# KirillHit/snn_for_object_detection

Measured on AMD Instinct MI355X. Metric: event-frames/sec (BxT) SODa-3M GEN1 304x240 fwd+bwd, higher is better.
Workload: dtype f32 (16-bit split products)

## Files before the change

include/snn_hip.h:

```cpp
#ifndef SNN_HIP_H
#define SNN_HIP_H

#include <stddef.h>
#include <stdint.h>

#ifdef __cplusplus
extern "C" {
#endif

#define SNN_ABI_VERSION 20

enum {
    SNN_NEURON_NONE = 0,
    SNN_NEURON_LIF = 1,
    SNN_NEURON_LI = 2,
    SNN_NEURON_LI_TANH = 3,
    SNN_NEURON_SLI = 4,
    SNN_NEURON_SYNAPSE = 5
};

enum { SNN_PREC_FP32 = 0, SNN_PREC_BF16X3 = 1, SNN_PREC_BF16X6 = 3, SNN_PREC_FP16X3 = 4, SNN_PREC_BF16X1 = 5,
       SNN_PREC_BF16S = 6 };

enum { SNN_SCAN_WIDE_ADDRESSING = 1,
// ... 77 lines not shown
                            int precision);
int snn_conv2d_gather_plan(int mode, int64_t N, int H, int W, int Cin, int Ho, int Wo, int Cout, int KH, int KW, int stride,
                           int pad, int64_t ld_in, int64_t ld_out, int align_bits, int has_split_image, int has_addend,
                           int has_addend2, int frames_per_step, int precision, int phase, int* out);
int snn_conv2d_wgrad_plan(int64_t N, int H, int W, int Cin, int Ho, int Wo, int Cout, int KH, int KW, int stride, int pad,
                          int64_t ldx, int64_t lddy, int align_bits, int precision, int spikes, int num_cu, int* out);
int snn_conv1x1_spikes_supported(int64_t N, int H, int W, int Cin, int Cout, int64_t ld, int fwd_precision,
                                 int bwd_precision);
int snn_conv1x1_spikes_fwd(const float* vdec, int64_t ld, float v_th, const float* w, float* y, int64_t ldy, int64_t N, int H,
                           int W, int Cin, int Cout, void* stream);
int snn_conv1x1_spikes_wgrad(const float* vdec, int64_t ld, float v_th, const float* dy, int64_t lddy, float* dw, int64_t N,
                             int H, int W, int Cin, int Cout, int accumulate, float* workspace, int splitk, void* stream);

int snn_conv2d_spikes_supported(int64_t N, int H, int W, int Cin, int Ho, int Wo, int Cout, int KH, int KW, int stride,
                                int pad, int64_t ld, int fwd_precision, int bwd_precision);
int snn_conv2d_spikes_fwd(const float* vdec, int64_t ld, float v_th, const float* w, float* y, int64_t ldy, int64_t N, int H,
                          int W, int Cin, int Ho, int Wo, int Cout, int KH, int KW, int stride, int pad, double* bn_partial,
                          int frames_per_step, int* bn_layout, void* stream);
int snn_conv2d_spikes_wgrad(const float* vdec, int64_t ld, float v_th, const float* dy, int64_t lddy, float* dw, int64_t N,
                            int H, int W, int Cin, int Ho, int Wo, int Cout, int KH, int KW, int stride, int pad,
                            int accumulate, float* workspace, int splitk, void* stream);
int snn_conv3x3_halo_spikes(const float* vdec, int64_t ld, float v_th, const void* w_image, float* y, int64_t ldy, int64_t N,
                            int H, int W, int Cin, int Cout, double* bn_partial, int frames_per_step, int* bn_layout,
                            void* stream);

int snn_conv1x1_mask_supported(int64_t N, int H, int W, int Cin, int Cout, const uint32_t* mask, int64_t ld_mask,
                               const float* w, const float* y, int64_t ldy, const float* dy, int64_t lddy, const float* dw,
                               int fwd_precision, int bwd_precision);
int snn_conv1x1_mask_fwd(const uint32_t* mask, int64_t ld_mask, const float* w, float* y, int64_t ldy, int64_t N, int H, int W,
                         int Cin, int Cout, void* stream);
int snn_conv1x1_mask_wgrad(const uint32_t* mask, int64_t ld_mask, const float* dy, int64_t lddy, float* dw, int64_t N, int H,
                           int W, int Cin, int Cout, int accumulate, float* workspace, int splitk, void* stream);

size_t snn_bn_stats_partial_size(int T, int64_t M, int C);
int snn_bn_stats(const float* y, int64_t ldy, int T, int64_t M, int C, double* partial, void* stream);
int snn_bn_stats_finalize(const double* partial, int chunks, int rows_per_chunk, int T, int64_t M, int C,
                          const float* gamma, const float* bias, float eps, float momentum,
                          float* running_mean, float* running_var, int use_running,
                          float* mean, float* invstd, float* alpha, float* beta, void* stream);

int snn_bn_stats_reduce(const double* partial, int chunks, int rows_per_chunk, int T, int64_t M, int C, double* sums,
                        void* stream);
int snn_bn_stats_from_sums(const double* sums, int T, int64_t M_total, int C,
                           const float* gamma, const float* bias, float eps, float momentum,
                           float* running_mean, float* running_var,
                           float* mean, float* invstd, float* alpha, float* beta,
                           double* var_scratch, void* stream);

int snn_affine_neuron_fwd(int neuron, const float* y, int64_t ldy,
                          const float* alpha, const float* beta,
                          const float* v0, const float* i0,
                          float* out, int64_t ldo, const float* addend, int64_t ld_addend,
                          float* vT, float* iT, float* vdec,
                          int T, int64_t M, int C, const snn_neuron_params* p, int flags, void* stream);
int snn_affine_neuron_fwd_mask(int neuron, const float* y, int64_t ldy, const float* alpha, const float* beta,
                               const float* v0, const float* i0, float* out, int64_t ldo, const float* addend,
                               int64_t ld_addend, float* vT, float* iT, float* vdec, int T, int64_t M, int C,
                               const snn_neuron_params* p, int flags, void* stream, uint32_t* mask, int64_t ld_mask);

size_t snn_affine_neuron_bwd_sums_size(int T, int64_t M, int C);
int snn_affine_neuron_bwd_sums_from_state(int neuron, int T, int64_t M, int C, int64_t ldg, const snn_neuron_params* p,
                                          int flags);
int snn_affine_neuron_bwd_plan(int neuron, int T, int64_t M, int C, int64_t ldg, int64_t ldy, int with_sums,
                               const snn_neuron_params* p, int flags, int64_t* out);
int snn_affine_neuron_bwd(int neuron, const float* g_out, int64_t ldg, const float* state,
                          const float* y, int64_t ldy, const float* g_vT, const float* g_iT,
// ... 207 lines not shown
```

snn_for_object_detection_amd/_hip.py:

```python

import ctypes
import os
from ctypes import POINTER, Structure, c_char_p, c_double, c_float, c_int, c_int32, c_int64, c_size_t, c_void_p

_HERE = os.path.dirname(os.path.abspath(__file__))
LIB_PATH = os.environ.get("SNN_HIP_LIB") or os.path.join(_HERE, "libsnn_hip.so")

NEURON_NONE, NEURON_LIF, NEURON_LI, NEURON_LI_TANH, NEURON_SLI, NEURON_SYNAPSE = 0, 1, 2, 3, 4, 5
POOL_AVG, POOL_MAX, POOL_SUM = 0, 1, 2
ACT_RELU, ACT_SILU, ACT_TANH = 0, 1, 2
ABI_VERSION = 20
PREC_FP32, PREC_BF16X3, PREC_BF16X6, PREC_FP16X3, PREC_BF16X1, PREC_BF16S = 0, 1, 3, 4, 5, 6
SCAN_WIDE_ADDRESSING, SCAN_LAST_STEP_ONLY, SCAN_BF16_STORAGE, SCAN_SPIKES_FROM_VDEC, SCAN_SUMS_FROM_STATE = 1, 2, 4, 8, 16
SCAN_STATE_LOOKBACK = 32
SCAN_SPIKE_MASK = 32
SURR_SUPER, SURR_TRIANGLE, SURR_SIGMOID, SURR_ATAN = 0, 1, 2, 3
ACTIVITY_NONZERO_F32, ACTIVITY_NONZERO_BF16, ACTIVITY_ABOVE_F32, ACTIVITY_ABOVE_BF16, ACTIVITY_MASK = 0, 1, 2, 3, 4
LOSS_CLS_MODES = {"ce": 0, "focal": 1}
LOSS_BOX_MODES = {"l1": 0, "giou": 1, "diou": 2, "ciou": 3}


class NeuronParams(Structure):
    _fields_ = [("c_mem", c_float), ("c_syn", c_float), ("v_leak", c_float), ("v_th", c_float),
                ("v_reset", c_float), ("alpha", c_float), ("v_st", c_float), ("tau_sec", c_float),
# ... 17 lines not shown
    "snn_detect_assemble": (c_int, [_P, _P, _P, _P, _P, _P, _I, _I, _I, _F, _P, _P]),
    "snn_conv2d_fwd": (c_int, [_P, _L, _P, _P, _P, _L, _L, _I, _I, _I, _I, _I, _I, _I, _I, _I, _I, _P, _L, _P, _I, _P, _I,
                               _P]),
    "snn_weight_presplit": (c_int, [_P, _P, _L, _I, _P]),
    "snn_conv2d_fwd_bn_partial_size": (c_size_t, [_L, _I, _I, _I, _I]),
    "snn_conv2d_wgrad_bn_supported": (c_int, [_L, _I, _I, _I, _I, _I, _I, _I, _I, _I, _I]),
    "snn_conv2d_wgrad_bn": (c_int, [_P, _L, _P, _L, _P, _L, _P, _I, _I, _P, _L, _I, _I, _I, _I, _I, _I, _I, _I, _I, _I, _I,
                                    _P, _I, _P]),
    "snn_conv3x3_s2_dgrad_supported": (c_int, [_L, _I, _I, _I, _I, _I, _I]),
    "snn_conv3x3_s2_dgrad_plan": (c_int, [_L, _I, _I, _I, _I, _I, _I, _P]),
    "snn_conv3x3_halo_plan": (c_int, [_L, _I, _I, _I, _I, _I, _P]),
    "snn_conv2d_wgrad_halo_plan": (c_int, [_L, _I, _I, _I, _I, _I, _I, _I, _I, _P]),
    "snn_conv_first_plan": (c_int, [_L, _I, _I, _I, _I, _I, _I, _I, _I, _I, _I, _P]),
    "snn_conv3x3_s2_dgrad": (c_int, [_P, _L, _P, _P, _L, _L, _I, _I, _I, _I, _I, _I, _P, _L, _P, _L, _I, _P]),
    "snn_conv3x3_halo_supported": (c_int, [_L, _I, _I, _I, _I]),
    "snn_conv3x3_halo_bn_chunks": (c_int64, [_I, _I, _I]),
    "snn_weight_frag_image_bytes": (c_size_t, [_I, _I]),
    "snn_weight_frag_image_batched": (c_int, [_P, _P, _P, _I, _I, _I, _I, _P]),
    "snn_conv3x3_halo": (c_int, [_P, _L, _P, _P, _L, _L, _I, _I, _I, _I, _P, _L, _P, _L, _P, _I, _P, _I, _P]),
    "snn_conv2d_dgrad": (c_int, [_P, _L, _P, _P, _P, _L, _L, _I, _I, _I, _I, _I, _I, _I, _I, _I, _I, _P, _L, _P, _L,
                                 _I, _P]),
    "snn_conv2d_wgrad": (c_int, [_P, _L, _P, _L, _P, _L, _I, _I, _I, _I, _I, _I, _I, _I, _I, _I, _I, _P, _I, _I,
                                 _P]),
    "snn_conv2d_wgrad_splitk": (c_int, [_L, _I, _I, _I, _I, _I, _I, _I, _I, _I, _I, _I]),
    "snn_conv2d_wgrad_kernel": (c_int, [_L, _I, _I, _I, _I, _I, _I, _I, _I, _I, _I, _I]),
    "snn_conv2d_gather_plan": (c_int, [_I, _L, _I, _I, _I, _I, _I, _I, _I, _I, _I, _I, _L, _L, _I, _I, _I, _I, _I, _I, _I, _P]),
    "snn_conv2d_wgrad_plan": (c_int, [_L, _I, _I, _I, _I, _I, _I, _I, _I, _I, _I, _L, _L, _I, _I, _I, _I, _P]),
    "snn_conv1x1_spikes_supported": (c_int, [_L, _I, _I, _I, _I, _L, _I, _I]),
    "snn_conv1x1_spikes_fwd": (c_int, [_P, _L, _F, _P, _P, _L, _L, _I, _I, _I, _I, _P]),
    "snn_conv1x1_spikes_wgrad": (c_int, [_P, _L, _F, _P, _L, _P, _L, _I, _I, _I, _I, _I, _P, _I, _P]),
    "snn_conv1x1_mask_supported": (c_int, [_L, _I, _I, _I, _I, _P, _L, _P, _P, _L, _P, _L, _P, _I, _I]),
    "snn_conv1x1_mask_fwd": (c_int, [_P, _L, _P, _P, _L, _L, _I, _I, _I, _I, _P]),
    "snn_conv1x1_mask_wgrad": (c_int, [_P, _L, _P, _L, _P, _L, _I, _I, _I, _I, _I, _P, _I, _P]),
    "snn_conv2d_spikes_supported": (c_int, [_L, _I, _I, _I, _I, _I, _I, _I, _I, _I, _I, _L, _I, _I]),
    "snn_conv2d_spikes_fwd": (c_int, [_P, _L, _F, _P, _P, _L, _L, _I, _I, _I, _I, _I, _I, _I, _I, _I, _I, _P, _I, _P, _P]),
    "snn_conv2d_spikes_wgrad": (c_int, [_P, _L, _F, _P, _L, _P, _L, _I, _I, _I, _I, _I, _I, _I, _I, _I, _I, _I, _P, _I, _P]),
    "snn_conv3x3_halo_spikes": (c_int, [_P, _L, _F, _P, _P, _L, _L, _I, _I, _I, _I, _P, _I, _P, _P]),
    "snn_bn_stats_partial_size": (c_size_t, [_I, _L, _I]),
    "snn_bn_stats": (c_int, [_P, _L, _I, _L, _I, _P, _P]),
    "snn_bn_stats_finalize": (c_int, [_P, _I, _I, _I, _L, _I, _P, _P, _F, _F, _P, _P, _I, _P, _P, _P, _P, _P]),
    "snn_bn_stats_reduce": (c_int, [_P, _I, _I, _I, _L, _I, _P, _P]),
    "snn_bn_stats_from_sums": (c_int, [_P, _I, _L, _I, _P, _P, _F, _F, _P, _P, _P, _P, _P, _P, _P, _P]),
    "snn_bn_bwd_reduce": (c_int, [_P, _I, _L, _I, _P, _P]),
    "snn_bn_bwd_coef": (c_int, [_P, _P, _P, _I, _L, _I, _P, _P, _P, _P, _P, _P, _P, _P, _I, _P]),
    "snn_affine_neuron_fwd": (c_int, [_I, _P, _L, _P, _P, _P, _P, _P, _L, _P, _L, _P, _P, _P, _I, _L, _I,
                                      POINTER(NeuronParams), _I, _P]),
    "snn_affine_neuron_fwd_mask": (c_int, [_I, _P, _L, _P, _P, _P, _P, _P, _L, _P, _L, _P, _P, _P, _I, _L, _I,
                                           POINTER(NeuronParams), _I, _P, _P, _L]),
    "snn_lif_ckpt_interval": (c_int, []),
    "snn_lif_fwd_ckpt": (c_int, [_P, _L, _P, _P, _P, _P, _P, _L, _P, _L, _P, _P, _P, _I, _L, _I,
                                 POINTER(NeuronParams), _P]),
    "snn_lif_bwd_ckpt": (c_int, [_P, _L, _P, _P, _L, _P, _P, _P, _P, _I, _P, _P, _P, _P, _I, _L, _I,
                                 POINTER(NeuronParams), _P]),
    "snn_affine_neuron_bwd_sums_size": (c_size_t, [_I, _L, _I]),
    "snn_affine_neuron_bwd": (c_int, [_I, _P, _L, _P, _P, _L, _P, _P, _P, _P, _I, _P, _P, _P, _P, _I, _L, _I,
                                      POINTER(NeuronParams), _I, _P]),
    "snn_bn_bwd_finalize": (c_int, [_P, _I, _L, _I, _P, _P, _P, _P, _P, _P, _P, _P, _I, _P]),
    "snn_bn_bwd_finalize_from_state": (c_int, [_P, _I, _L, _I, _P, _P, _P, _P, _P, _P, _L, _P, _P, _P, _P, _P, _I, _P]),
    "snn_bn_bwd_reduce_from_state": (c_int, [_P, _I, _L, _I, _P, _P, _P, _P, _P, _P, _L, _P, _P]),
    "snn_affine_neuron_bwd_sums_from_state": (c_int, [_I, _I, _L, _I, _L, POINTER(NeuronParams), _I]),
    "snn_affine_neuron_bwd_plan": (c_int, [_I, _I, _L, _I, _L, _L, _I, POINTER(NeuronParams), _I, _P]),
    "snn_lif_tau_param": (c_int, [_P, _P, _I, _I, _P, _P, _P]),
    "snn_lif_tau_fwd": (c_int, [_I, _P, _L, _P, _P, _P, _P, _P, _L, _P, _L, _P, _P, _P, _I, _L, _I,
                                POINTER(NeuronParams), _P, _P, _I, _P]),
    "snn_lif_tau_bwd_partial_size": (c_size_t, [_I, _L, _I, _I]),
    "snn_lif_tau_bwd_plan": (c_int, [_I, _I, _L, _I, _L, _L, _I, _I, POINTER(NeuronParams), _I, _P]),
# ... 105 lines not shown
```

snn_for_object_detection_amd/csrc/conv_common.h:

```cpp
#pragma once
#include "snn_common.h"

namespace {

constexpr int kThreads = 256;
#define SNN_CONV_MIN_WAVES 3

typedef __bf16 bf16x8 __attribute__((ext_vector_type(8)));
typedef __bf16 bf16x4 __attribute__((ext_vector_type(4)));
typedef __bf16 bf16x2 __attribute__((ext_vector_type(2)));
typedef float f32x2 __attribute__((ext_vector_type(2)));
typedef unsigned u32x4 __attribute__((ext_vector_type(4)));
typedef unsigned u32x2 __attribute__((ext_vector_type(2)));
typedef _Float16 f16x8 __attribute__((ext_vector_type(8)));
typedef _Float16 f16x2 __attribute__((ext_vector_type(2)));
constexpr float kF16WeightScale = 256.0f;
constexpr float kF16ActScale = 16.0f;
constexpr float kF16Unscale = 1.0f / (kF16WeightScale * kF16ActScale);

__device__ __forceinline__ int div_magic(int n, int d, unsigned magic) { return d == 1 ? n : (int)__umulhi((unsigned)n, magic); }

enum : unsigned {
    kAlignIn16 = 1u, kAlignIn8 = 2u, kAlignW16 = 4u, kAlignOut16 = 8u, kAlignOut8 = 16u, kAlignAdd16 = 32u, kAlignAdd8 = 64u,
    kAlignAdd2_16 = 128u, kAlignAdd2_8 = 256u, kAlignSplit16 = 512u, kAlignAll = 1023u
};

static int check_conv_shape(const char* name, int64_t N, int H, int W, int Cin, int Ho, int Wo, int Cout, int KH,
                            int KW, int stride, int pad) {
    SNN_REQUIRE(N > 0 && H > 0 && W > 0 && Cin > 0 && Cout > 0 && KH > 0 && KW > 0 && stride > 0 && pad >= 0,
                "%s: bad shape", name);
    SNN_REQUIRE(Ho == (H + 2 * pad - KH) / stride + 1 && Wo == (W + 2 * pad - KW) / stride + 1 && Ho > 0 && Wo > 0,
                "%s: output size %dx%d does not match input %dx%d k=%dx%d s=%d p=%d", name, Ho, Wo, H, W, KH, KW,
                stride, pad);
    return 0;
}

static bool spikes_shape_ok(int64_t N, int H, int W, int Cin, int Ho, int Wo, int Cout, int KH, int KW, int stride, int pad,
                            int64_t ld) {
    return N > 0 && H > 0 && W > 0 && Cin > 0 && Cout > 0 && KH >= 1 && KW >= 1 && KH <= 5 && KW <= 5 && stride >= 1 &&
           Ho == (H + 2 * pad - KH) / stride + 1 && Wo == (W + 2 * pad - KW) / stride + 1 && Ho > 0 && Wo > 0 &&
           Cin % 32 == 0 && Cout % 4 == 0 && ld % 4 == 0 && ld >= Cin && N * (int64_t)H * W < 0x7fffffffLL &&
           N * (int64_t)Ho * Wo < 0x7fffffffLL && (int64_t)H * W * ld * 16 < 0x7fffffffLL;
}

}

struct FirstGeom {
    int64_t ldx, ldy;
    int rows;
    int H, W, Ho, Wo, Cout, stride, pad;
    int group_rows, group_blocks;
    double* bn_partial;
    const float* bn_y;
    int64_t bn_ldy;
    const float* bn_coef;
    int bn_tc;
    int bn_fps;
    int rs;
};

struct FirstPlan {
    int ok;
    int rs, LW, cgs, PP;
    int blocks;
    int group_rows, group_blocks;
    int max_rows, last_stage_rows;
    size_t lds;
};
FirstPlan snn_first_layer_plan(int64_t N, int H, int W, int Ho, int Wo, int Cout, int stride, int pad,
                               int frames_per_step, bool wgrad, int num_cu);
bool snn_first_layer_shape(int Cin, int Cout, int KH, int KW);
int snn_first_layer_blocks(int64_t rows, int num_cu);
int snn_launch_first(bool wgrad, bool bnapply, bool sb, int blocks, size_t lds, const float* x, const float* w,
                     const float* dy, float* out, const FirstGeom& fg, void* stream, const char* name);

bool snn_wgrad_mask_ok(int64_t N, int H, int W, int Cin, int Cout, const uint32_t* mask, int64_t ld_mask, const float* dy,
                       int64_t lddy, const float* dw);
```

snn_for_object_detection_amd/csrc/conv_gather.hip:

```cpp
#include <stdlib.h>
#include <type_traits>
#include "conv_common.h"

#if defined(SNN_STAMP) || defined(SNN_CLOCK)
__device__ unsigned long long g_stamps[2048 * 8];
__device__ unsigned long long g_stamps2[2048 * 4];
extern "C" int snn_debug_stamps(unsigned long long* out, int n) {
    return (int)hipMemcpyFromSymbol(out, HIP_SYMBOL(g_stamps), sizeof(unsigned long long) * n);
}
extern "C" int snn_debug_stamps2(unsigned long long* out, int n) {
    return (int)hipMemcpyFromSymbol(out, HIP_SYMBOL(g_stamps2), sizeof(unsigned long long) * n);
}
#endif
#ifdef SNN_STAMP
#define STAMP(i) do { unsigned long long t_ = __builtin_readcyclecounter(); st_acc[i] += t_ - st_last; st_last = t_; } while (0)
#else
#define STAMP(i) do {} while (0)
#endif

namespace {

constexpr int BM = 128;
constexpr int BK = 32;
constexpr int LDK = BK + 4;
// ... 23 lines not shown

template <int WM, int WN, int TN>
__device__ __forceinline__ void stat_flush(double (&s)[TN], double (&q)[TN], double* red, double* __restrict__ partial,
                                           int64_t step, int64_t chunk, int64_t chunks, int n0, int OC, int tid) {
    const int lane = tid & 63, wave = tid >> 6;
#pragma unroll
    for (int j = 0; j < TN; ++j) {
        s[j] += __shfl_xor(s[j], 32, 64);
        q[j] += __shfl_xor(q[j], 32, 64);
        if (lane < 32) {
            red[((wave * TN + j) * 32 + lane) * 2 + 0] = s[j];
            red[((wave * TN + j) * 32 + lane) * 2 + 1] = q[j];
        }
    }
    __syncthreads();
    if (tid < WN * TN * 32) {
        const int wn = tid / (TN * 32), jr = tid % (TN * 32);
        double ss = 0.0, qq = 0.0;
#pragma unroll
        for (int wm = 0; wm < WM; ++wm) {
            const double* src = red + (((wm * WN + wn) * TN) * 32 + jr) * 2;
            ss += src[0];
            qq += src[1];
        }
        if (n0 + tid < OC) {
            double* dst = partial + snn_bn_partial_index(step, chunk, n0 + tid, chunks, OC);
            dst[0] = ss;
            dst[1] = qq;
        }
    }
    __syncthreads();
}

template <int BN, int WM, int WN, bool DGRAD, bool VEC, int SPLIT, bool FAST, bool PRESPLIT = false, bool SB = false,
          bool XSP = false, bool XM = false>
__global__ __launch_bounds__(kThreads, (FAST && SPLIT) ? (PRESPLIT ? 3 : (SB ? (DGRAD ? 4 : SNN_GATHER_SB_WAVES) : 2)) : SNN_CONV_MIN_WAVES) void k_conv_gather(const float* __restrict__ in, const float* __restrict__ wk,
                                                          float* __restrict__ out, ConvGeom g,
                                                          const float* __restrict__ addend, int64_t ld_add,
                                                          const float* __restrict__ addend2, int64_t ld_add2) {
    constexpr int TM = BM / WM / 32;
    constexpr int TN = BN / WN / 32;
    constexpr int BROWS = BN / 32;
    static_assert(WM * WN == 4, "4 waves");
    static_assert(!SB || (FAST && SPLIT == 5 && !PRESPLIT), "bf16 storage: the pipelined one-product kernel");
    static_assert(!XSP || (FAST && SPLIT == 4 && !DGRAD && !PRESPLIT && !SB), "spikes from potentials: fp16 x 3 forward");
    static_assert(!XM || XSP, "spike bit mask: an instance of the spikes-from-potentials kernel");
    constexpr int ES = SB ? 2 : 4;
    constexpr int NPIECE = SPLIT == 3 ? 3 : (SPLIT == 5 ? 1 : 2);
    constexpr int A_BYTES = SPLIT ? NPIECE * BM * LDB * 2 : BM * LDK * 4;
    constexpr int B_BYTES = SPLIT ? NPIECE * BN * LDB * 2 : BN * LDK * 4;
    constexpr int STAGE_BYTES = 4 * 32 * (TN * 32 + 4) * 4;
    constexpr int SMEM_BYTES = A_BYTES + B_BYTES > STAGE_BYTES ? A_BYTES + B_BYTES : STAGE_BYTES;
    __shared__ __attribute__((aligned(16))) unsigned char smem[SMEM_BYTES];
    float* As = reinterpret_cast<float*>(smem);
    float* Bs = reinterpret_cast<float*>(smem + A_BYTES);
    __bf16* Ah = reinterpret_cast<__bf16*>(smem);
    __bf16* Al = Ah + BM * LDB;
    __bf16* Am = Al + BM * LDB;
    __bf16* Bh = reinterpret_cast<__bf16*>(smem + A_BYTES);
    __bf16* Bl = Bh + BN * LDB;
    __bf16* Bm = Bl + BN * LDB;

    const int tid = threadIdx.x;
#if defined(SNN_STAMP) || defined(SNN_CLOCK)
    const unsigned long long st_kernel_begin = __builtin_amdgcn_s_memtime();
    const unsigned long long st_real_begin = __builtin_amdgcn_s_memrealtime();
#endif
    const int lane_id = tid & 63, wave = tid >> 6;
    const int wm = wave / WN, wn = wave % WN;
    const int r = lane_id & 31, h = lane_id >> 5;

    const int bid_xcd = blockIdx.x & 7, bid_q = blockIdx.x >> 3;
    const int bid_n = bid_q % g.ntiles;
    const int64_t bid_m = (int64_t)bid_xcd * g.mtiles_per_xcd + bid_q / g.ntiles;
    if (bid_m >= g.mtiles) return;
    const int64_t m0 = bid_m * BM;
    const int n0 = bid_n * BN;

    const int lrr = tid >> 3;
// ... 13 lines not shown
        const int oy = (int)(t - img * oh_);
        a_base[j] = (int)(img * (unsigned)(g.IH * g.IW));
        if (!DGRAD) {
            a_y0[j] = oy * g.stride - g.pad;
            a_x0[j] = ox * g.stride - g.pad;
        } else if (g.stride == 1) {
            a_y0[j] = oy + g.pad;
            a_x0[j] = ox + g.pad;
        } else {
            a_y0[j] = (int)((unsigned)(oy * g.stride + g.ph + g.pad - g.kh0) / (unsigned)g.stride);
            a_x0[j] = (int)((unsigned)(ox * g.stride + g.pw + g.pad - g.kw0) / (unsigned)g.stride);
        }
    }

    auto decode_k = [&](int kk, int& dy, int& dx, int& c, int& wcol) {
        int tap = div_magic(kk, g.IC, g.magic_ic);
        c = kk - tap * g.IC;
        if (!DGRAD) {
            int kh = div_magic(tap, g.KW, g.magic_kw), kw = tap - kh * g.KW;
            dy = kh;
            dx = kw;
            wcol = kk;
        } else {
            int jh = div_magic(tap, g.nkw, g.magic_kw), jw = tap - jh * g.nkw;
            dy = -jh;
            dx = -jw;
            wcol = ((g.kh0 + g.stride * jh) * g.KW + (g.kw0 + g.stride * jw)) * g.IC + c;
        }
    };

    using AReg = typename std::conditional<SB, u32x2, typename std::conditional<XM, unsigned, f32x4>::type>::type;
    AReg ra[4];
    f32x4 rb[BROWS];

    __amdgpu_buffer_rsrc_t rs_a, rs_b;
    int a_rel[4];
    unsigned a_mask[4];
    unsigned b_rel[BROWS];
    [[maybe_unused]] int xm_rel[TM];
    if constexpr (XM) {
        rs_a = __builtin_amdgcn_make_buffer_rsrc(const_cast<float*>(in), 0, (int)(g.Mtot * g.ldi * 4), 0x00020000);
        rs_b = __builtin_amdgcn_make_buffer_rsrc(const_cast<float*>(wk), 0, g.OC * g.KtotFull * 4, 0x00020000);
#pragma unroll
        for (int i = 0; i < TM; ++i) {
            const int64_t m = m0 + (wm * TM + i) * 32 + r;
            xm_rel[i] = m < g.Mtot ? (int)(m * g.ldi * 4) : -1;
        }
#pragma unroll
        for (int j = 0; j < BROWS; ++j) {
            const int n = n0 + lr + 32 * j;
            b_rel[j] = n < g.OC ? (unsigned)(n * g.KtotFull + kq) * 4u : 0x80000000u;
        }
    } else if (FAST) {
        const int ow_ = DGRAD ? g.OWc : g.OW, oh_ = DGRAD ? g.OHc : g.OH;
        const int64_t img0 = (unsigned)m0 / (unsigned)(oh_ * ow_);
        const int64_t ipix = (int64_t)g.IH * g.IW;
        const int64_t bytes = ((((int64_t)g.nimg - img0) * ipix - 1) * g.ldi + g.IC) * ES;
        rs_a = __builtin_amdgcn_make_buffer_rsrc(const_cast<char*>(reinterpret_cast<const char*>(in) + img0 * ipix * g.ldi * ES), 0,
                                                 bytes > 0xffffffffLL ? (int)0xffffffffu : (int)(unsigned)bytes,
                                                 0x00020000);
        rs_b = __builtin_amdgcn_make_buffer_rsrc(const_cast<float*>(wk), 0, g.OC * g.KtotFull * 4, 0x00020000);
        const int tw_n = DGRAD ? g.nkw : g.KW;
#pragma unroll
        for (int j = 0; j < 4; ++j) {
            const int relpix = (a_base[j] - (int)(img0 * ipix)) + a_y0[j] * g.IW + a_x0[j];
            a_rel[j] = (relpix * (int)g.ldi + kq) * ES;
            const int nth = DGRAD ? g.nkh : g.KH;
            unsigned xm = 0, mask = 0;
#pragma unroll
            for (int tw = 0; tw < 6; ++tw) {
                const int ix = DGRAD ? a_x0[j] - tw : a_x0[j] + tw;
                xm |= (tw < tw_n && (unsigned)ix < (unsigned)g.IW) ? 1u << tw : 0u;
            }
#pragma unroll
            for (int th = 0; th < 6; ++th) {
                const int iy = DGRAD ? a_y0[j] - th : a_y0[j] + th;
                mask |= (th < nth && (unsigned)iy < (unsigned)g.IH) ? xm << (th * tw_n) : 0u;
            }
            a_mask[j] = a_ok[j] ? mask : 0u;
        }
#pragma unroll
        for (int j = 0; j < BROWS; ++j) {
            const int n = n0 + lr + 32 * j;
            b_rel[j] = n < g.OC ? (unsigned)(n * g.KtotFull + kq) * 4u : 0x80000000u;
        }
    }
    const unsigned fast_tw_n = DGRAD ? g.nkw : g.KW;
    const unsigned fast_tw_one = fast_tw_n == 1 ? 1u : 0u;
    auto load_tiles_fast = [&](int k0n, AReg (&ra)[4], f32x4 (&rb)[BROWS], int which = 3) {
        const bool kin = k0n < g.Ktot;
        const int tap = (int)__umulhi((unsigned)k0n, g.magic_ic);
        const int c0 = k0n - tap * g.IC;
        const int th = (int)(__umulhi((unsigned)tap, g.magic_kw) + (unsigned)tap * fast_tw_one);
        const int tw = tap - th * (int)fast_tw_n;
        int toff, wcol0;
        if (!DGRAD) {
            toff = ((th * g.IW + tw) * (int)g.ldi + c0) * ES;
            wcol0 = k0n;
        } else {
            toff = (c0 - (th * g.IW + tw) * (int)g.ldi) * ES;
            wcol0 = ((g.kh0 + g.stride * th) * g.KW + (g.kw0 + g.stride * tw)) * g.IC + c0;
        }
        const int tbit = kin ? tap : 31;
        if constexpr (XM) {
            if (which & 1) {
#pragma unroll
                for (int i = 0; i < TM; ++i)
                    ra[i] = (unsigned)__builtin_amdgcn_raw_buffer_load_b32(rs_a, (kin && xm_rel[i] >= 0) ? xm_rel[i] + (k0n >> 5) * 4 : -1, 0, 0);
            }
        } else if (which & 1) {
#pragma unroll
            for (int j = 0; j < 4; ++j) {
                const int voff = ((a_mask[j] >> tbit) & 1u) ? a_rel[j] + toff : -1;
                if constexpr (SB) ra[j] = __builtin_bit_cast(u32x2, __builtin_amdgcn_raw_buffer_load_b64(rs_a, voff, 0, 0));
                else ra[j] = __builtin_bit_cast(f32x4, __builtin_amdgcn_raw_buffer_load_b128(rs_a, voff, 0, 0));
            }
        }
        if (which & 2) {
            const unsigned wb = (unsigned)wcol0 * 4u;
#pragma unroll
            for (int j = 0; j < BROWS; ++j)
                rb[j] = __builtin_bit_cast(f32x4, __builtin_amdgcn_raw_buffer_load_b128(rs_b, (int)(b_rel[j] + wb), 0, 0));
        }
    };

    auto load_tiles = [&](int k0) {
        if (FAST) {
            load_tiles_fast(k0, ra, rb);
            return;
        }
        if constexpr (!SB && !XM) {
        const int kk = k0 + kq;
        if (VEC) {
            const bool kin = kk < g.Ktot;
            int dy, dx, c, wcol;
            decode_k(kin ? kk : g.Ktot - 4, dy, dx, c, wcol);
            const f32x4 zero = {0.f, 0.f, 0.f, 0.f};
#pragma unroll
            for (int j = 0; j < 4; ++j) {
                const int iy = a_y0[j] + dy, ix = a_x0[j] + dx;
                const bool ok = kin & a_ok[j] & ((unsigned)iy < (unsigned)g.IH) & ((unsigned)ix < (unsigned)g.IW);
                const int iyc = min(max(iy, 0), g.IH - 1), ixc = min(max(ix, 0), g.IW - 1);
                f32x4 v = *reinterpret_cast<const f32x4*>(in + (int64_t)(a_base[j] + iyc * g.IW + ixc) * g.ldi + c);
                ra[j] = ok ? v : zero;
            }
#pragma unroll
            for (int j = 0; j < BROWS; ++j) {
                const int n = n0 + lr + 32 * j;
                const int nc = min(n, g.OC - 1);
                f32x4 v = *reinterpret_cast<const f32x4*>(wk + (int64_t)nc * g.KtotFull + wcol);
                rb[j] = (kin & (n < g.OC)) ? v : zero;
            }
        } else {
#pragma unroll
            for (int e = 0; e < 4; ++e) {
                const int ke = kk + e;
                const bool kin = ke < g.Ktot;
                int dy, dx, c, wcol;
                decode_k(kin ? ke : 0, dy, dx, c, wcol);
#pragma unroll
                for (int j = 0; j < 4; ++j) {
// ... 75 lines not shown
            if constexpr (SPLIT == 4) {
                u32x2 hi, lo;
#pragma unroll
                for (int e = 0; e < 4; e += 2) {
                    const float a = v[e] * scale, b = v[e + 1] * scale;
                    const f16x2 ph = __builtin_convertvector(f32x2{a, b}, f16x2);
                    const f16x2 pl = __builtin_convertvector(f32x2{a - (float)ph[0], b - (float)ph[1]}, f16x2);
                    hi[e >> 1] = __builtin_bit_cast(unsigned, ph);
                    lo[e >> 1] = __builtin_bit_cast(unsigned, pl);
                }
                out[0] = __builtin_bit_cast(bf16x4, hi);
                out[1] = __builtin_bit_cast(bf16x4, lo);
                return;
            }
#pragma unroll
            for (int e = 0; e < 4; e += 2) {
                f32x2 rest = {v[e], v[e + 1]};
                bf16x2 p = __builtin_convertvector(rest, bf16x2);
                unsigned bits = __builtin_bit_cast(unsigned, p);
                out[0][e] = p[0]; out[0][e + 1] = p[1];
                rest[0] -= __builtin_bit_cast(float, bits << 16);
                rest[1] -= __builtin_bit_cast(float, bits & 0xffff0000u);
                if (SPLIT == 3) {
                    p = __builtin_convertvector(rest, bf16x2);
                    bits = __builtin_bit_cast(unsigned, p);
                    out[2][e] = p[0]; out[2][e + 1] = p[1];
                    rest[0] -= __builtin_bit_cast(float, bits << 16);
                    rest[1] -= __builtin_bit_cast(float, bits & 0xffff0000u);
                }
                p = __builtin_convertvector(rest, bf16x2);
                out[1][e] = p[0]; out[1][e + 1] = p[1];
            }
        };
        auto convert_a = [&](const AReg& v, bf16x4* out) {
            if constexpr (SB) out[0] = __builtin_bit_cast(bf16x4, v);
            else if constexpr (XM) return;
            else if constexpr (XSP) {
                u32x2 hi;
#pragma unroll
                for (int e = 0; e < 4; e += 2)
                    hi[e >> 1] = (v[e] > g.x_th ? 0x4C00u : 0u) | (v[e + 1] > g.x_th ? 0x4C000000u : 0u);
                out[0] = __builtin_bit_cast(bf16x4, hi);
            } else convert(v, out, kF16ActScale);
        };
        auto convert_b = [&](const f32x4& v, bf16x4* out) {
            if constexpr (PRESPLIT) {
                static_assert(!PRESPLIT || SPLIT == 2 || SPLIT == 4, "pre-split weights: two-piece modes only");
                out[0] = __builtin_bit_cast(bf16x4, f32x2{v[0], v[1]});
                out[1] = __builtin_bit_cast(bf16x4, f32x2{v[2], v[3]});
            } else {
                convert(v, out, kF16WeightScale);
            }
        };
        [[maybe_unused]] unsigned xm_cur[TM];
        auto xm_expand = [&](unsigned word, int sel) {
            const unsigned b = (word >> (8 * sel)) & 0xffu;
            u32x4 d;
#pragma unroll
            for (int q = 0; q < 4; ++q) {
                const unsigned v = (b >> (2 * q)) & 3u;
                d[q] = ((v | (v << 15)) & 0x00010001u) * 0x4C00u;
            }
            return __builtin_bit_cast(bf16x8, d);
        };
        auto write_tiles = [&]() {
#pragma unroll
            for (int j = 0; j < (XM ? 0 : 4); ++j) {
// ... 36 lines not shown
                for (int j = 0; j < TN; ++j) {
                    if constexpr (SPLIT == 5) {
                        acc[i][j] = __builtin_amdgcn_mfma_f32_32x32x16_bf16(ah[i], bh[j], acc[i][j], 0, 0, 0);
                        continue;
                    }
                    if constexpr (SPLIT == 4 && XSP) {
                        const f16x8 xah = __builtin_bit_cast(f16x8, ah[i]);
                        const f16x8 xbh = __builtin_bit_cast(f16x8, bh[j]), xbl = __builtin_bit_cast(f16x8, bl[j]);
                        acc[i][j] = __builtin_amdgcn_mfma_f32_32x32x16_f16(xah, xbl, acc[i][j], 0, 0, 0);
                        acc[i][j] = __builtin_amdgcn_mfma_f32_32x32x16_f16(xah, xbh, acc[i][j], 0, 0, 0);
                        continue;
                    }
                    if constexpr (SPLIT == 4) {
                        const f16x8 xah = __builtin_bit_cast(f16x8, ah[i]), xal = __builtin_bit_cast(f16x8, al[i]);
                        const f16x8 xbh = __builtin_bit_cast(f16x8, bh[j]), xbl = __builtin_bit_cast(f16x8, bl[j]);
                        acc[i][j] = __builtin_amdgcn_mfma_f32_32x32x16_f16(xal, xbh, acc[i][j], 0, 0, 0);
                        acc[i][j] = __builtin_amdgcn_mfma_f32_32x32x16_f16(xah, xbl, acc[i][j], 0, 0, 0);
                        acc[i][j] = __builtin_amdgcn_mfma_f32_32x32x16_f16(xah, xbh, acc[i][j], 0, 0, 0);
                        continue;
                    }
                    acc[i][j] = __builtin_amdgcn_mfma_f32_32x32x16_bf16(al[i], bh[j], acc[i][j], 0, 0, 0);
                    acc[i][j] = __builtin_amdgcn_mfma_f32_32x32x16_bf16(ah[i], bl[j], acc[i][j], 0, 0, 0);
                    if (SPLIT == 3) {
                        acc[i][j] = __builtin_amdgcn_mfma_f32_32x32x16_bf16(am[i], bm[j], acc[i][j], 0, 0, 0);
                        acc[i][j] = __builtin_amdgcn_mfma_f32_32x32x16_bf16(am[i], bh[j], acc[i][j], 0, 0, 0);
                        acc[i][j] = __builtin_amdgcn_mfma_f32_32x32x16_bf16(ah[i], bm[j], acc[i][j], 0, 0, 0);
                    }
                    acc[i][j] = __builtin_amdgcn_mfma_f32_32x32x16_bf16(ah[i], bh[j], acc[i][j], 0, 0, 0);
                }
        };
        constexpr int NM = TM * TN * (XSP ? 2 : NPROD);
        constexpr int NREAD = XM ? TN * NP : (XSP ? TM + TN * NP : (TM + TN) * NP);
        constexpr int CONV_OPS = SPLIT == 3 ? 24 : (SPLIT == 5 ? 2 : 14);
        constexpr int VPG_A = ((XM ? TM * 18 : (XSP ? 4 * 8 : 4 * CONV_OPS)) + NM - 1) / NM;
        constexpr int VPG_B = PRESPLIT ? 1 : (BROWS * CONV_OPS + NM - 1) / NM;
        if (g.Ktot > 0) {
            AReg ra0[4];
            f32x4 rb0[BROWS];
            load_tiles_fast(0, ra0, rb0);
            load_tiles_fast(BK, ra, rb);
            if constexpr (XM) {
#pragma unroll
                for (int i = 0; i < TM; ++i) xm_cur[i] = ra0[i];
            }
#pragma unroll
            for (int j = 0; j < 4; ++j) convert_a(ra0[j], pa[j]);
#pragma unroll
            for (int j = 0; j < BROWS; ++j) convert_b(rb0[j], pb[j]);
            write_tiles();
        }
        __syncthreads();
#ifdef SNN_STAMP
        unsigned long long st_acc[8] = {0, 0, 0, 0, 0, 0, 0, 0};
        unsigned long long st_last = __builtin_readcyclecounter();
        const unsigned long long st_begin = st_last;
#endif
#pragma unroll 1
        for (int k0 = 0; k0 < g.Ktot; k0 += BK) {
            mfma_group(0);
#pragma unroll
            for (int j = 0; j < 4; ++j) convert_a(ra[j], pa[j]);
            __builtin_amdgcn_sched_group_barrier(0x100, NREAD, 0);
#pragma unroll
            for (int m = 0; m < NM; ++m) {
                __builtin_amdgcn_sched_group_barrier(0x008, 1, 0);
                __builtin_amdgcn_sched_group_barrier(0x002, VPG_A, 0);
            }
            __builtin_amdgcn_sched_barrier(0);
            STAMP(0);
            mfma_group(1);
#pragma unroll
            for (int j = 0; j < BROWS; ++j) convert_b(rb[j], pb[j]);
            __builtin_amdgcn_sched_group_barrier(0x100, NREAD, 0);
#pragma unroll
            for (int m = 0; m < NM; ++m) {
                __builtin_amdgcn_sched_group_barrier(0x008, 1, 0);
                __builtin_amdgcn_sched_group_barrier(0x002, VPG_B, 0);
            }
            __builtin_amdgcn_sched_barrier(0);
            STAMP(1);
            if constexpr (XM) {
#pragma unroll
                for (int i = 0; i < TM; ++i) xm_cur[i] = ra[i];
            }
            load_tiles_fast(k0 + 2 * BK, ra, rb);
            STAMP(2);
            __syncthreads();
            STAMP(3);
            write_tiles();
            STAMP(4);
            __syncthreads();
            STAMP(5);
        }
#ifdef SNN_STAMP
        if (tid == 0 && bid_n == 0 && blockIdx.x < 2048) {
            st_acc[6] = __builtin_readcyclecounter() - st_begin;
            st_acc[7] = st_begin;
            for (int i = 0; i < 8; ++i) g_stamps[blockIdx.x * 8 + i] = st_acc[i];
        }
#endif
    } else {
        if (g.Ktot > 0) {
            load_tiles(0);
            store_tiles();
        }
        __syncthreads();

    #pragma unroll 1
        for (int k0 = 0; k0 < g.Ktot; k0 += BK) {
            load_tiles(k0 + BK);
            __builtin_amdgcn_sched_barrier(0);
            if (SPLIT) {
    #pragma unroll
                for (int ks = 0; ks < BK / 16; ++ks) {
                    bf16x8 ah[TM], am[TM], al[TM], bh[TN], bm[TN], bl[TN];
    #pragma unroll
                    for (int i = 0; i < TM; ++i) {
                        const int off = ((wm * TM + i) * 32 + r) * LDB + ks * 16 + 8 * h;
// ... 208 lines not shown
    p.mtiles = (int)gm;
    p.mtiles_per_xcd = (int)snn_ceil_div(gm, 8);
    p.ntiles = (int)snn_ceil_div(g.OC, p.bn);
    p.blocks = (int64_t)p.mtiles_per_xcd * 8 * p.ntiles;
    if (p.blocks > 0x7fffffffLL) {
        p.why = kGatherGridTooLarge;
        return p;
    }
    p.ok = 1;
    return p;
}

static unsigned gather_align_bits(const void* in, const void* wk, const void* wk_split, const void* out, const void* addend,
                                  int64_t ld_add, const void* addend2, int64_t ld_add2) {
    unsigned a = 0;
    if (aligned(16, {in})) a |= kAlignIn16;
    if (aligned(8, {in})) a |= kAlignIn8;
    if (aligned(16, {wk})) a |= kAlignW16;
    if (aligned(16, {out})) a |= kAlignOut16;
    if (aligned(8, {out})) a |= kAlignOut8;
    if (addend && ld_add % 4 == 0 && aligned(16, {addend})) a |= kAlignAdd16;
    if (addend && ld_add % 4 == 0 && aligned(8, {addend})) a |= kAlignAdd8;
    if (addend2 && ld_add2 % 4 == 0 && aligned(16, {addend2})) a |= kAlignAdd2_16;
    if (addend2 && ld_add2 % 4 == 0 && aligned(8, {addend2})) a |= kAlignAdd2_8;
    if (wk_split && aligned(16, {wk_split})) a |= kAlignSplit16;
    return a;
}

constexpr int gather_wm(int bn) { return bn == 32 ? 4 : 2; }
constexpr int gather_wn(int bn) { return bn == 32 ? 1 : 2; }

static int launch_gather(bool dgrad, int split, bool sb, bool xsp, const float* in, const float* wk, const void* wk_split,
                         float* out, const ConvGeom& g, const float* addend, int64_t ld_add, const float* addend2,
                         int64_t ld_add2, hipStream_t st, const char* name, bool xm = false) {
    unsigned align = gather_align_bits(in, wk, wk_split, out, addend, ld_add, addend2, ld_add2);
    if (xm) align = (align & ~(kAlignIn16 | kAlignIn8)) | (aligned(4, {in}) ? kAlignIn16 : 0u);
    const GatherPlan p = gather_plan(g, dgrad, split, sb, xsp, align, wk_split != nullptr, addend != nullptr,
                                     addend2 != nullptr, xm);
    SNN_REQUIRE(p.why != kGatherTooManyPixels, "%s: too many pixels", name);
    SNN_REQUIRE(p.why != kGatherNotFastSB, "%s: bf16 storage covers the pipelined implicit GEMM only (channels a multiple of 32, pixel "
                "stride a multiple of 4, 8-byte aligned tensors): %d channels, stride %lld", name, g.IC, (long long)g.ldi);
    SNN_REQUIRE(p.why != kGatherNotFastXSP, "%s: covers the pipelined implicit GEMM only (input channels a multiple of 32, pixel stride a "
                "multiple of 4, 16-byte aligned tensors): %d channels, stride %lld", name, g.IC, (long long)g.ldi);
    SNN_REQUIRE(p.why != kGatherGridTooLarge, "%s: grid too large", name);
    ConvGeom gg = g;
    gg.out_vec = p.out_vec;
    gg.mtiles = p.mtiles;
    gg.mtiles_per_xcd = p.mtiles_per_xcd;
    gg.ntiles = p.ntiles;
    const dim3 grid((unsigned)p.blocks);
    const float* wsrc = p.loader == kLoadFastPresplit ? static_cast<const float*>(wk_split) : wk;
    dispatch(
        [&](auto BN, auto L, auto DGRAD, auto SPLIT) {
            constexpr int l = L(), s = SPLIT();
            constexpr bool vec = l != kLoadScalar, fast = l >= kLoadFast, pre = l == kLoadFastPresplit, sbl = l == kLoadSB,
                           xml = l == kLoadXM, xspl = l == kLoadXSP || xml;
            constexpr int ksplit = fast ? s : (vec ? (s == 4 ? 3 : (s == 5 ? 2 : s)) : 0);
            if constexpr ((DGRAD() ? s != 3 && s != 4 : s != 2) && (!sbl || s == 5) && (!xspl || (!DGRAD() && s == 4)) &&
                          (!pre || s == 2 || s == 4)) {
                hipLaunchKernelGGL((k_conv_gather<BN(), gather_wm(BN()), gather_wn(BN()), DGRAD(), vec, ksplit, fast, pre, sbl, xspl, xml>),
                                   grid, dim3(kThreads), 0, st, in, wsrc, out, gg, addend, ld_add, addend2, ld_add2);
                return true;
            }
            return false;
        },
        OneOf<32, 64, 128>{p.bn}, OneOf<0, 1, 2, 3, 4, 5, 6>{p.loader}, Flag{dgrad}, OneOf<0, 2, 3, 4, 5>{split});
    SNN_CHECK_LAUNCH(name);
    return 0;
}

}

namespace {
template <bool F16>
__global__ void k_weight_presplit(const f32x4* __restrict__ w, u32x4* __restrict__ out, int64_t groups) {
    for (int64_t i = (int64_t)blockIdx.x * blockDim.x + threadIdx.x; i < groups; i += (int64_t)gridDim.x * blockDim.x) {
        const f32x4 v = w[i];
        u32x4 o;
#pragma unroll
        for (int e = 0; e < 4; e += 2) {
            if (F16) {
                const float a = v[e] * kF16WeightScale, b = v[e + 1] * kF16WeightScale;
                const f16x2 ph = __builtin_convertvector(f32x2{a, b}, f16x2);
                const f16x2 pl = __builtin_convertvector(f32x2{a - (float)ph[0], b - (float)ph[1]}, f16x2);
                o[e >> 1] = __builtin_bit_cast(unsigned, ph);
                o[2 + (e >> 1)] = __builtin_bit_cast(unsigned, pl);
            } else {
                f32x2 rest = {v[e], v[e + 1]};
                const bf16x2 ph = __builtin_convertvector(rest, bf16x2);
                const unsigned bits = __builtin_bit_cast(unsigned, ph);
                rest[0] -= __builtin_bit_cast(float, bits << 16);
                rest[1] -= __builtin_bit_cast(float, bits & 0xffff0000u);
                const bf16x2 pl = __builtin_convertvector(rest, bf16x2);
                o[e >> 1] = bits;
                o[2 + (e >> 1)] = __builtin_bit_cast(unsigned, pl);
            }
        }
        out[i] = o;
    }
// ... 264 lines not shown
    if (!(N > 0 && H > 0 && W > 0 && Cin > 0 && Cout > 0 && Cin % 32 == 0 && ld_mask >= Cin / 32 && ldy >= Cout &&
          N * (int64_t)H * W < 0x7fffffffLL && (int64_t)Cin * Cin < 0xffffffffLL && mask && w && y))
        return false;
    const ConvGeom g = gather_fwd_geom(N, H, W, Cin, H, W, Cout, 1, 1, 1, 0, ld_mask, ldy);
    unsigned align = gather_align_bits(mask, w, nullptr, y, nullptr, 0, nullptr, 0) & ~(kAlignIn16 | kAlignIn8);
    if (aligned(4, {mask})) align |= kAlignIn16;
    const GatherPlan p = gather_plan(g, false, 4, false, true, align, false, false, false, true);
    return p.ok && p.loader == kLoadXM;
}
}

extern "C" int snn_conv1x1_mask_supported(int64_t N, int H, int W, int Cin, int Cout, const uint32_t* mask, int64_t ld_mask,
                                          const float* w, const float* y, int64_t ldy, const float* dy, int64_t lddy,
                                          const float* dw, int fwd_precision, int bwd_precision) {
    if (fwd_precision != SNN_PREC_FP16X3 || bwd_precision != SNN_PREC_BF16X3 || !mask) return 0;
    if (!(N > 0 && H > 0 && W > 0 && Cin > 0 && Cout > 0 && Cin % 32 == 0 && ld_mask >= Cin / 32 && aligned(4, {mask}) &&
          N * (int64_t)H * W * ld_mask * 4 < 0x7fffffffLL))
        return 0;
    if ((w || y) && !mask_fwd_ok(N, H, W, Cin, Cout, mask, ld_mask, w, y, ldy)) return 0;
    if ((dy || dw) && !snn_wgrad_mask_ok(N, H, W, Cin, Cout, mask, ld_mask, dy, lddy, dw)) return 0;
    return 1;
}

extern "C" int snn_conv1x1_mask_fwd(const uint32_t* mask, int64_t ld_mask, const float* w, float* y, int64_t ldy, int64_t N,
                                    int H, int W, int Cin, int Cout, void* stream) {
    SNN_REQUIRE(mask && w && y, "snn_conv1x1_mask_fwd: null pointer");
    if (check_conv_shape("snn_conv1x1_mask_fwd", N, H, W, Cin, H, W, Cout, 1, 1, 1, 0)) return 1;
    SNN_REQUIRE(mask_fwd_ok(N, H, W, Cin, Cout, mask, ld_mask, w, y, ldy),
                "snn_conv1x1_mask_fwd: call not covered (ask snn_conv1x1_mask_supported)");
    const ConvGeom g = gather_fwd_geom(N, H, W, Cin, H, W, Cout, 1, 1, 1, 0, ld_mask, ldy);
    return launch_gather(false, 4, false, true, reinterpret_cast<const float*>(mask), w, nullptr, y, g, nullptr, 0, nullptr, 0,
                         (hipStream_t)stream, "snn_conv1x1_mask_fwd", true);
}
```

snn_for_object_detection_amd/csrc/conv_wgrad.hip:

```cpp
#include <stdlib.h>
#include <type_traits>
#include "conv_common.h"

namespace {

constexpr int WB_K = 32;

struct WgradGeom {
    int64_t Mtot;
    int H, W, Cin, Ho, Wo, Cout, KH, KW, stride, pad;
    int64_t ldx, lddy;
    int Ktot;
    int64_t pix_per_split;
    int tiles_m, tiles_n, splitk;
    int nimg;
    float x_th;
};

template <int TM, int TN, int WM, int WN, bool VEC>
__global__ __launch_bounds__(kThreads, SNN_CONV_MIN_WAVES) void k_conv_wgrad(const float* __restrict__ x, const float* __restrict__ dy,
                                                         float* __restrict__ ws, WgradGeom g) {
    static_assert(WM * WN == 4, "4 waves");
    constexpr int BMc = 32 * TM * WM, BNk = 32 * TN * WN;
    constexpr int DG = BMc / 4, XG = BNk / 4;
    constexpr int DP = kThreads / DG, XP = kThreads / XG;
    constexpr int DJ = WB_K / DP, XJ = WB_K / XP;
    static_assert(DJ >= 1 && XJ >= 1, "tile too narrow");
    __shared__ __attribute__((aligned(16))) float Ds[WB_K * BMc];
    __shared__ __attribute__((aligned(16))) float Xs[WB_K * BNk];
    __shared__ int Pinfo[2][WB_K][4];

    const int tid = threadIdx.x;
    const int lane_id = tid & 63, wave = tid >> 6;
    const int wm = wave / WN, wn = wave % WN;
    const int r = lane_id & 31, h = lane_id >> 5;

    const int tiles = g.tiles_m * g.tiles_n;
    int L = blockIdx.x, z, tile;
    if (g.splitk % 8 == 0) {
        z = (L % 8) + 8 * (L / (8 * tiles));
        tile = (L / 8) % tiles;
    } else {
        z = L / tiles;
        tile = L % tiles;
    }
    const int co0 = (tile % g.tiles_m) * BMc;
    const int kc0 = (tile / g.tiles_m) * BNk;
    const int64_t p_lo = (int64_t)z * g.pix_per_split;
    int64_t p_hi = p_lo + g.pix_per_split;
    if (p_hi > g.Mtot) p_hi = g.Mtot;
// ... 115 lines not shown
        for (int ks = 0; ks < WB_K / 2; ++ks) {
            float a[TM], b[TN];
#pragma unroll
            for (int i = 0; i < TM; ++i) a[i] = Ds[(ks * 2 + h) * BMc + (wm * TM + i) * 32 + r];
#pragma unroll
            for (int j = 0; j < TN; ++j) b[j] = Xs[(ks * 2 + h) * BNk + (wn * TN + j) * 32 + r];
#pragma unroll
            for (int i = 0; i < TM; ++i)
#pragma unroll
                for (int j = 0; j < TN; ++j)
                    acc[i][j] = __builtin_amdgcn_mfma_f32_32x32x2f32(a[i], b[j], acc[i][j], 0, 0, 0);
        }
        __syncthreads();
        store_tiles();
        __syncthreads();
        slot ^= 1;
    }

    float* slab = ws + (int64_t)z * g.Cout * (int64_t)g.Ktot;
#pragma unroll
    for (int i = 0; i < TM; ++i)
#pragma unroll
        for (int j = 0; j < TN; ++j) {
            const int kc = kc0 + (wn * TN + j) * 32 + r;
            if (kc >= g.Ktot) continue;
#pragma unroll
            for (int e = 0; e < 16; ++e) {
                const int co = co0 + (wm * TM + i) * 32 + (e & 3) + 8 * (e >> 2) + 4 * h;
                if (co < g.Cout) slab[(int64_t)co * g.Ktot + kc] = acc[i][j][e];
            }
        }
}

template <int TM, int TN, int WM, int WN, int WBK, bool ONE, bool SB = false, bool XSP = false, bool XM = false>
__global__ __launch_bounds__(kThreads, 2) void k_conv_wgrad_pipe(const float* __restrict__ x,
                                                                 const float* __restrict__ dy,
                                                                 float* __restrict__ ws, WgradGeom g) {
    static_assert(WM * WN == 4, "4 waves");
    constexpr int BMc = 32 * TM * WM, BNk = 32 * TN * WN;
    constexpr int DG = BMc / 4, XG = BNk / 4;
    static_assert(WBK == 32 || WBK == 64, "stage length");
    static_assert(!SB || ONE, "bf16 storage: one product");
    static_assert(!XSP || (!ONE && !SB), "spikes from potentials: the bf16 x 3 kernel");
    static_assert(!XM || XSP, "spike bit mask: an instance of the spikes-from-potentials kernel");
    constexpr int XW = ((BNk / 32) * WBK + kThreads - 1) / kThreads;
    constexpr int ES = SB ? 2 : 4;
    constexpr int LDW = WBK + 8;
    constexpr int NQ = WBK / 4;
    constexpr int GPP = kThreads / NQ;
    constexpr int DQ = (DG + GPP - 1) / GPP, XQ = (XG + GPP - 1) / GPP;
    __shared__ __attribute__((aligned(16))) __bf16 Dh[BMc * LDW];
    __shared__ __attribute__((aligned(16))) __bf16 Dl[ONE ? 8 : BMc * LDW];
    __shared__ __attribute__((aligned(16))) __bf16 Xh[XM ? 8 : BNk * LDW];
    __shared__ __attribute__((aligned(16))) __bf16 Xl[(ONE || XSP) ? 8 : BNk * LDW];
    __shared__ __attribute__((aligned(16))) unsigned Xw[XM ? XW * kThreads : 4];
    __shared__ __attribute__((aligned(16))) int Pinfo[2][WBK][4];

    const int tid = threadIdx.x;
    const int lane_id = tid & 63, wave = tid >> 6;
    const int wm = wave / WN, wn = wave % WN;
    const int r = lane_id & 31, h = lane_id >> 5;

    const int tiles = g.tiles_m * g.tiles_n;
    int L = blockIdx.x, z, tile;
    if (g.splitk % 8 == 0) {
        z = (L % 8) + 8 * (L / (8 * tiles));
        tile = (L / 8) % tiles;
    } else {
        z = L / tiles;
        tile = L % tiles;
    }
    const int co0 = (tile % g.tiles_m) * BMc;
    const int kc0 = (tile / g.tiles_m) * BNk;
    const unsigned p_lo = (unsigned)((int64_t)z * g.pix_per_split);
    unsigned p_hi = p_lo + (unsigned)g.pix_per_split;
    if (p_hi > (unsigned)g.Mtot) p_hi = (unsigned)g.Mtot;
    if (p_lo >= p_hi) p_hi = p_lo;
// ... 2 lines not shown
    const unsigned img_lo = p_lo / opix;
    __amdgpu_buffer_rsrc_t rs_d, rs_x;
    {
        const int64_t dbytes = p_hi > p_lo ? (((int64_t)(p_hi - p_lo) - 1) * g.lddy + g.Cout) * ES : 0;
        rs_d = __builtin_amdgcn_make_buffer_rsrc(
            const_cast<char*>(reinterpret_cast<const char*>(dy) + (int64_t)p_lo * g.lddy * ES), 0, (int)dbytes, 0x00020000);
        const int64_t xbytes = ((((int64_t)g.nimg - img_lo) * ipix - 1) * g.ldx + g.Cin) * ES;
        rs_x = __builtin_amdgcn_make_buffer_rsrc(
            const_cast<char*>(reinterpret_cast<const char*>(x) + (int64_t)img_lo * ipix * g.ldx * ES), 0,
                                                 xbytes > 0x7fffffffLL ? 0x7fffffff : (xbytes < 0 ? 0 : (int)xbytes), 0x00020000);
    }

    const int quad = (tid >> 2) % NQ, grp0 = (tid & 3) + 4 * (tid / (4 * NQ));
    int d_off[DQ];
    int x_tapoff[XQ];
    int x_kh[XQ], x_kw[XQ], x_cq[XQ], d_cq[DQ];
    bool x_ok[XQ];
#pragma unroll
    for (int q = 0; q < DQ; ++q) {
        d_cq[q] = (grp0 + GPP * q) * 4;
        const bool ok = (grp0 + GPP * q) < DG && (co0 + d_cq[q]) < g.Cout;
        d_off[q] = ok ? ((quad * 4) * (int)g.lddy + co0 + d_cq[q]) * ES : -1;
    }
#pragma unroll
    for (int q = 0; q < XQ; ++q) {
        x_cq[q] = (grp0 + GPP * q) * 4;
        const int kc = kc0 + x_cq[q];
        x_ok[q] = (grp0 + GPP * q) < XG && kc < g.Ktot;
        const int kcc = x_ok[q] ? kc : 0;
        const int tap = kcc / g.Cin, ci = kcc - tap * g.Cin;
        x_kh[q] = tap / g.KW;
        x_kw[q] = tap - x_kh[q] * g.KW;
        x_tapoff[q] = ((x_kh[q] * g.W + x_kw[q]) * (int)g.ldx + ci) * ES;
    }

    int d_img = 0, d_oy = 0, d_ox = 0;
    unsigned d_p = p_lo + tid;
    if (tid < WBK) {
        const unsigned pp = d_p < (unsigned)g.Mtot ? d_p : 0u;
        const unsigned t = pp / (unsigned)g.Wo;
        d_ox = (int)(pp - t * (unsigned)g.Wo);
        const unsigned im = t / (unsigned)g.Ho;
        d_oy = (int)(t - im * (unsigned)g.Ho);
        d_img = (int)(im - img_lo);
    }
    auto decode = [&](int slot) {
        if constexpr (XM) return;
        if (tid < WBK) {
            const int y0 = d_oy * g.stride - g.pad, x0 = d_ox * g.stride - g.pad;
            int4 info;
            info.x = ((d_img * (int)ipix + y0 * g.W + x0) * (int)g.ldx) * ES;
            info.y = y0;
            info.z = x0;
            info.w = d_p < p_hi ? 1 : 0;
            *reinterpret_cast<int4*>(&Pinfo[slot][tid][0]) = info;
            d_p += WBK;
            d_ox += WBK;
            while (d_ox >= g.Wo) {
                d_ox -= g.Wo;
                if (++d_oy == g.Ho) {
                    d_oy = 0;
                    ++d_img;
                }
            }
        }
    };

    using OReg = typename std::conditional<SB, u32x2, f32x4>::type;
    OReg rd[DQ][4], rx[XQ][4];
    [[maybe_unused]] unsigned rxw[XW] = {}, pxw[XW] = {};
    [[maybe_unused]] const int xm_pl = tid % WBK;
    [[maybe_unused]] const int xm_word = kc0 / 32 + tid / WBK;
    [[maybe_unused]] bool xm_ok[XW];
#pragma unroll
    for (int k = 0; k < XW; ++k)
        xm_ok[k] = tid / WBK + k * (kThreads / WBK) < BNk / 32 && (xm_word + k * (kThreads / WBK)) * 32 < g.Cin;
    if constexpr (XM)
        rs_x = __builtin_amdgcn_make_buffer_rsrc(const_cast<float*>(x), 0, (int)(g.Mtot * g.ldx * 4), 0x00020000);
    auto load_tiles = [&](unsigned p0, int slot) {
        const int dstage = (int)(p0 - p_lo) * (int)g.lddy * ES;
        auto fetch = [&](__amdgpu_buffer_rsrc_t rs, int voff) -> OReg {
            if constexpr (SB) return __builtin_bit_cast(u32x2, __builtin_amdgcn_raw_buffer_load_b64(rs, voff, 0, 0));
            else return __builtin_bit_cast(f32x4, __builtin_amdgcn_raw_buffer_load_b128(rs, voff, 0, 0));
        };
        if constexpr (XM) {
            const unsigned p = p0 + (unsigned)xm_pl;
#pragma unroll
            for (int k = 0; k < XW; ++k)
                rxw[k] = (unsigned)__builtin_amdgcn_raw_buffer_load_b32(
                    rs_x, (xm_ok[k] && p < p_hi) ? (int)((p * (unsigned)g.ldx + (unsigned)(xm_word + k * (kThreads / WBK))) * 4u) : -1, 0, 0);
        }
#pragma unroll
        for (int e = 0; e < 4; ++e) {
            const int4 info = XM ? int4{0, 0, 0, 0} : *reinterpret_cast<const int4*>(&Pinfo[slot][quad * 4 + e][0]);
#pragma unroll
            for (int q = 0; q < DQ; ++q) {
                const int voff = d_off[q] < 0 ? -1 : d_off[q] + e * (int)g.lddy * ES + dstage;
                rd[q][e] = fetch(rs_d, voff);
            }
#pragma unroll
            for (int q = 0; q < (XM ? 0 : XQ); ++q) {
                const int iy = info.y + x_kh[q], ix = info.z + x_kw[q];
                const bool ok = (info.w != 0) & x_ok[q] & ((unsigned)iy < (unsigned)g.H) & ((unsigned)ix < (unsigned)g.W);
                const int voff = ok ? info.x + x_tapoff[q] : -1;
                rx[q][e] = fetch(rs_x, voff);
            }
        }
    };
    bf16x4 pd[DQ][4][2], px[XQ][4][2];
    auto convert_quad = [&](const OReg (&v)[4], bf16x4 (&out)[4][2]) {
        if constexpr (SB) {
#pragma unroll
            for (int c = 0; c < 4; ++c) {
                const unsigned a0 = v[0][c >> 1], a1 = v[1][c >> 1], a2 = v[2][c >> 1], a3 = v[3][c >> 1];
                u32x2 o;
                if (c & 1) o = u32x2{(a0 >> 16) | (a1 & 0xffff0000u), (a2 >> 16) | (a3 & 0xffff0000u)};
                else o = u32x2{(a0 & 0xffffu) | (a1 << 16), (a2 & 0xffffu) | (a3 << 16)};
                out[c][0] = __builtin_bit_cast(bf16x4, o);
            }
        } else {
#pragma unroll
        for (int c = 0; c < 4; ++c)
#pragma unroll
            for (int e = 0; e < 4; e += 2) {
                f32x2 rest = {v[e][c], v[e + 1][c]};
                bf16x2 pp = __builtin_convertvector(rest, bf16x2);
                const unsigned bits = __builtin_bit_cast(unsigned, pp);
                out[c][0][e] = pp[0]; out[c][0][e + 1] = pp[1];
                if constexpr (!ONE) {
                    rest[0] -= __builtin_bit_cast(float, bits << 16);
                    rest[1] -= __builtin_bit_cast(float, bits & 0xffff0000u);
                    pp = __builtin_convertvector(rest, bf16x2);
                    out[c][1][e] = pp[0]; out[c][1][e + 1] = pp[1];
                }
            }
        }
    };
    auto convert_spikes = [&](const OReg (&v)[4], bf16x4 (&out)[4][2]) {
        if constexpr (XSP) {
#pragma unroll
            for (int c = 0; c < 4; ++c) {
                u32x2 o;
// ... 46 lines not shown
            if constexpr (!ONE) al[i] = *reinterpret_cast<const bf16x8*>(&Dl[off]);
        }
#pragma unroll
        for (int j = 0; j < TN; ++j) {
            if constexpr (XM) {
                const u32x4 w0 = *reinterpret_cast<const u32x4*>(&Xw[(wn * TN + j) * WBK + ks * 16 + 8 * h]);
                const u32x4 w1 = *reinterpret_cast<const u32x4*>(&Xw[(wn * TN + j) * WBK + ks * 16 + 8 * h + 4]);
                u32x4 d;
                d[0] = (((w0[0] >> r) & 1u) | (((w0[1] >> r) & 1u) << 16)) * 0x3F80u;
                d[1] = (((w0[2] >> r) & 1u) | (((w0[3] >> r) & 1u) << 16)) * 0x3F80u;
                d[2] = (((w1[0] >> r) & 1u) | (((w1[1] >> r) & 1u) << 16)) * 0x3F80u;
                d[3] = (((w1[2] >> r) & 1u) | (((w1[3] >> r) & 1u) << 16)) * 0x3F80u;
                bh[j] = __builtin_bit_cast(bf16x8, d);
                continue;
            }
            const int off = ((wn * TN + j) * 32 + r) * LDW + ks * 16 + 8 * h;
            bh[j] = *reinterpret_cast<const bf16x8*>(&Xh[off]);
            if constexpr (!ONE && !XSP) bl[j] = *reinterpret_cast<const bf16x8*>(&Xl[off]);
        }
#pragma unroll
        for (int i = 0; i < TM; ++i)
#pragma unroll
            for (int j = 0; j < TN; ++j) {
                if constexpr (!ONE) {
                    acc[i][j] = __builtin_amdgcn_mfma_f32_32x32x16_bf16(al[i], bh[j], acc[i][j], 0, 0, 0);
                    if constexpr (!XSP) acc[i][j] = __builtin_amdgcn_mfma_f32_32x32x16_bf16(ah[i], bl[j], acc[i][j], 0, 0, 0);
                }
                acc[i][j] = __builtin_amdgcn_mfma_f32_32x32x16_bf16(ah[i], bh[j], acc[i][j], 0, 0, 0);
            }
    };
    constexpr int NM = TM * TN * (ONE ? 1 : (XSP ? 2 : 3));
    constexpr int NREAD = XM ? 2 * TM + 2 * TN : (XSP ? 2 * TM + TN : (TM + TN) * (ONE ? 1 : 2));
    constexpr int CQ_OPS = SB ? 12 : 56;
    constexpr int VPG_D = (DQ * CQ_OPS + NM - 1) / NM, VPG_X = XM ? (TN * 20 + NM - 1) / NM : (XQ * (XSP ? 24 : CQ_OPS) + NM - 1) / NM;

    decode(0);
    __syncthreads();
    load_tiles(p_lo, 0);
    decode(1);
    __syncthreads();
#pragma unroll
    for (int q = 0; q < DQ; ++q) convert_quad(rd[q], pd[q]);
#pragma unroll
    for (int k = 0; k < XW; ++k) pxw[k] = rxw[k];
#pragma unroll
    for (int q = 0; q < XQ; ++q) {
        if constexpr (XM) continue;
        else if constexpr (XSP) convert_spikes(rx[q], px[q]);
        else convert_quad(rx[q], px[q]);
    }
    write_tiles();
    load_tiles(p_lo + WBK, 1);
    decode(0);
    __syncthreads();

    int slot = 0;
#pragma unroll 1
    for (unsigned p0 = p_lo; p0 < p_hi; p0 += WBK) {
        mfma_group(0);
#pragma unroll
        for (int q = 0; q < DQ; ++q) convert_quad(rd[q], pd[q]);
        __builtin_amdgcn_sched_group_barrier(0x100, NREAD, 0);
#pragma unroll
        for (int m = 0; m < NM; ++m) {
            __builtin_amdgcn_sched_group_barrier(0x008, 1, 0);
            __builtin_amdgcn_sched_group_barrier(0x002, VPG_D, 0);
        }
        __builtin_amdgcn_sched_barrier(0);
        mfma_group(1);
#pragma unroll
        for (int k = 0; k < XW; ++k) pxw[k] = rxw[k];
#pragma unroll
        for (int q = 0; q < XQ; ++q) {
            if constexpr (XM) continue;
            else if constexpr (XSP) convert_spikes(rx[q], px[q]);
            else convert_quad(rx[q], px[q]);
        }
        __builtin_amdgcn_sched_group_barrier(0x100, NREAD, 0);
#pragma unroll
        for (int m = 0; m < NM; ++m) {
            __builtin_amdgcn_sched_group_barrier(0x008, 1, 0);
            __builtin_amdgcn_sched_group_barrier(0x002, VPG_X, 0);
        }
        __builtin_amdgcn_sched_barrier(0);
#pragma unroll
        for (int ks = 2; ks < WBK / 16; ++ks) mfma_group(ks);
        load_tiles(p0 + 2 * WBK, slot);
        __syncthreads();
        write_tiles();
        decode(slot ^ 1);
        __syncthreads();
        slot ^= 1;
    }

    float* slab = ws + (int64_t)z * g.Cout * (int64_t)g.Ktot;
#pragma unroll
    for (int i = 0; i < TM; ++i)
#pragma unroll
        for (int j = 0; j < TN; ++j) {
            const int kcol = kc0 + (wn * TN + j) * 32 + r;
            if (kcol >= g.Ktot) continue;
#pragma unroll
            for (int e = 0; e < 16; ++e) {
                const int co = co0 + (wm * TM + i) * 32 + (e & 3) + 8 * (e >> 2) + 4 * h;
                if (co < g.Cout) slab[(int64_t)co * g.Ktot + kcol] = acc[i][j][e];
            }
        }
}

// ... 306 lines not shown
    p.pix_per_split = snn_ceil_div(snn_ceil_div(M, p.splitk), p.wbk) * p.wbk;
    const int64_t span_pix = p.pix_per_split * (int64_t)stride * stride + 3 * (int64_t)H * W;
    static const bool no_pipe = snn_tuning_env("SNN_WGRAD_NO_PIPE") != nullptr;
    const bool pipe = vec && bwd_split && !no_pipe && M < 0x7fffffffLL && span_pix * ldx * 4 < 0x7fffffffLL &&
                      p.pix_per_split * lddy * 4 < 0x7fffffffLL && (int64_t)H * W * ldx * 4 < 0x7fffffffLL &&
                      (!xm || (Cin % 32 == 0 && ldx * 32 >= Cin && M * ldx * 4 < 0x7fffffffLL));
    p.one = precision == SNN_PREC_BF16X1 || sbf;
    p.kernel = pipe ? kWgradPipe : (vec ? kWgradVec : kWgradScalar);
    if (sbf && !pipe) {
        p.why = kWgradNotPipeSB;
        return p;
    }
    if (xsp && !(pipe && !p.one)) {
        p.why = kWgradNotPipeXSP;
        return p;
    }
    p.tiles_m = (int)snn_ceil_div(Cout, p.t.bm);
    p.tiles_n = (int)snn_ceil_div(Ktot, p.t.bn);
    if ((int64_t)p.tiles_m * p.tiles_n * p.splitk > 0x7fffffff) {
        p.why = kWgradGridTooLarge;
        return p;
    }
    const int64_t owners = snn_ceil_div(M, p.pix_per_split);
    p.last_pix = M - (owners - 1) * p.pix_per_split;
    p.empty_splits = (int)(p.splitk - owners);
    p.ok = 1;
    return p;
}
}

static int wgrad_common(const float* x, int64_t ldx, const float* dy, int64_t lddy, float* dw, int64_t N,
                        int H, int W, int Cin, int Ho, int Wo, int Cout, int KH, int KW, int stride, int pad,
                        int accumulate, float* workspace, int splitk, int precision, void* stream, bool xsp, float x_th,
                        bool xm = false) {
    SNN_REQUIRE(x && dy && dw && workspace, "snn_conv2d_wgrad: null pointer");
    SNN_REQUIRE(precision == SNN_PREC_FP32 || precision == SNN_PREC_BF16X3 || precision == SNN_PREC_BF16X1 ||
                    precision == SNN_PREC_BF16S,
                "snn_conv2d_wgrad: precision must be SNN_PREC_FP32, _BF16X3, _BF16X1 or _BF16S (got %d)", precision);
    const bool sbf = precision == SNN_PREC_BF16S;
    if (check_conv_shape("snn_conv2d_wgrad", N, H, W, Cin, Ho, Wo, Cout, KH, KW, stride, pad)) return 1;
    SNN_REQUIRE((xm || ldx >= Cin) && lddy >= Cout, "snn_conv2d_wgrad: pixel stride smaller than channel count");
    SNN_REQUIRE(splitk >= 1 && splitk <= 32768, "snn_conv2d_wgrad: bad splitk %d", splitk);
    SNN_REQUIRE(N * (int64_t)H * W < 0x7fffffffLL, "snn_conv2d_wgrad: more than 2^31 input pixels");
    WgradGeom g;
    g.Mtot = N * Ho * (int64_t)Wo;
    g.H = H; g.W = W; g.Cin = Cin; g.Ho = Ho; g.Wo = Wo; g.Cout = Cout;
    g.KH = KH; g.KW = KW; g.stride = stride; g.pad = pad;
    g.ldx = ldx; g.lddy = lddy;
    g.Ktot = KH * KW * Cin;
    g.x_th = x_th;
    unsigned align = wgrad_align_bits(x, dy) | (aligned(16, {dw, workspace}) ? kAlignDw16 : 0u);
    if (xm) align = (align & ~(kAlignIn16 | kAlignIn8)) | (aligned(4, {x}) ? kAlignIn16 : 0u);
    WgradPlan p = wgrad_plan(N, H, W, Cin, Ho, Wo, Cout, KH, KW, stride, pad, ldx, lddy, align, precision, xsp, 0, splitk, !xm, xm);
    if (p.kernel == kWgradFirst) {
        const FirstPlan& fp = p.fp;
        FirstGeom fg = {ldx, lddy, (int)(N * Ho), H, W, Ho, Wo, Cout, stride, pad, fp.group_rows, splitk, nullptr,
                        nullptr, 0, nullptr, 0, 1, fp.rs};
        if (const int rc = snn_launch_first(true, false, sbf, splitk, fp.lds, x, nullptr, dy, workspace, fg, stream, "snn_conv2d_wgrad"))
            return rc;
        return wgrad_reduce_slabs(workspace, dw, (int64_t)Cout * g.Ktot, splitk, accumulate, (hipStream_t)stream);
    }
    if (p.kernel == kWgradHalo) {
        const SnnWgradHaloPlan& hp = p.hp;
        SNN_REQUIRE(p.why != kWgradHaloSplitk, "snn_conv2d_wgrad: splitk %d, expected %d (snn_conv2d_wgrad_splitk)", splitk,
                    hp.slabs);
        const int rc = snn_wgrad_halo_launch(hp, x, ldx, dy, lddy, workspace, N, H, W, Cin, Ho, Wo, Cout, stride,
                                             xsp ? 2 : ((precision == SNN_PREC_BF16X1 || sbf) ? 1 : 3), sbf,
                                             (hipStream_t)stream, x_th);
        if (rc == 0)
            return wgrad_reduce_slabs(workspace, dw, (int64_t)Cout * g.Ktot, hp.slabs, accumulate, (hipStream_t)stream);
        if (rc > 0) return rc;
        p = wgrad_plan(N, H, W, Cin, Ho, Wo, Cout, KH, KW, stride, pad, ldx, lddy, align, precision, xsp, 0, splitk, false);
    }
    SNN_REQUIRE(p.why != kWgradNotPipeSB, "snn_conv2d_wgrad: bf16 storage covers the event-frame layer and the pipelined kernels only "
                "(channels and strides multiples of 4, 8-byte aligned tensors, < 2 GiB per pixel split)");
    SNN_REQUIRE(p.why != kWgradNotPipeXSP, "snn_conv1x1_spikes_wgrad: covers the pipelined bf16 x 3 kernel only (channels and "
                "strides multiples of 4, 16-byte aligned tensors, < 2 GiB per pixel split)");
    SNN_REQUIRE(p.why != kWgradGridTooLarge, "snn_conv2d_wgrad: grid too large");
    g.pix_per_split = p.pix_per_split;
    g.nimg = (int)N;
    g.tiles_m = p.tiles_m;
    g.tiles_n = p.tiles_n;
    g.splitk = splitk;
    dim3 grid((unsigned)((int64_t)g.tiles_m * g.tiles_n * splitk));
    hipStream_t st = (hipStream_t)stream;
    dispatch(
        [&](auto ID, auto KERNEL, auto WBK, auto ONE, auto SB, auto XSP, auto XM) {
            constexpr WgradShape t = kWgradShapes[ID()];
            if constexpr (KERNEL() != kWgradPipe) {
                hipLaunchKernelGGL((k_conv_wgrad<t.tm, t.tn, t.wm, t.wn, KERNEL() == kWgradVec>), grid, dim3(kThreads), 0, st, x, dy,
                                   workspace, g);
            } else if constexpr ((!SB() || ONE()) && (!XSP() || (!ONE() && !SB())) && (!XM() || XSP())) {
                hipLaunchKernelGGL((k_conv_wgrad_pipe<t.tm, t.tn, t.wm, t.wn, WBK(), ONE(), SB(), XSP(), XM()>), grid, dim3(kThreads), 0,
                                   st, x, dy, workspace, g);
            }
            return true;
        },
        OneOf<0, 1, 2, 3, 4, 5>{p.t.id}, OneOf<0, 1, 2>{p.kernel}, OneOf<32, 64>{p.wbk}, Flag{p.one}, Flag{sbf}, Flag{xsp}, Flag{xm});
    SNN_CHECK_LAUNCH("snn_conv2d_wgrad");
    return wgrad_reduce_slabs(workspace, dw, (int64_t)Cout * g.Ktot, splitk, accumulate, st);
}

extern "C" int snn_conv2d_wgrad_splitk(int64_t N, int H, int W, int Cin, int Ho, int Wo, int Cout, int KH, int KW,
                                       int stride, int pad, int precision) {
    if (N <= 0 || Ho <= 0 || Wo <= 0 || Cin <= 0 || Cout <= 0 || KH <= 0 || KW <= 0) return 1;
    return wgrad_plan(N, H, W, Cin, Ho, Wo, Cout, KH, KW, stride, pad, Cin, Cout, kAlignAll, precision, false, 0, 0).splitk;
}

extern "C" int snn_conv2d_wgrad_kernel(int64_t N, int H, int W, int Cin, int Ho, int Wo, int Cout, int KH, int KW, int stride,
                                       int pad, int precision) {
    if (N <= 0 || Ho <= 0 || Wo <= 0 || Cin <= 0 || Cout <= 0 || KH <= 0 || KW <= 0) return 0;
    if (snn_first_layer_shape(Cin, Cout, KH, KW)) return 2;
    const int k = wgrad_plan(N, H, W, Cin, Ho, Wo, Cout, KH, KW, stride, pad, Cin, Cout, kAlignAll, precision, false, 0, 0).kernel;
    return k == kWgradHalo ? 1 : (k == kWgradFirst ? 2 : 0);
}

extern "C" int snn_conv2d_wgrad_bn_supported(int64_t N, int H, int W, int Cin, int Ho, int Wo, int Cout, int KH, int KW,
                                             int stride, int pad) {
    if (Cin != 2 || KH != 3 || KW != 3) return 0;
    return snn_first_layer_plan(N, H, W, Ho, Wo, Cout, stride, pad, 0, true, 0).ok;
}

extern "C" int snn_conv2d_wgrad_bn(const float* x, int64_t ldx, const float* gx, int64_t ldgx, const float* y, int64_t ldy,
                                   const float* coef, int T, int frames_per_step, float* dw, int64_t N, int H, int W,
                                   int Cin, int Ho, int Wo, int Cout, int KH, int KW, int stride, int pad, int accumulate,
                                   float* workspace, int splitk, void* stream) {
    SNN_REQUIRE(x && gx && y && coef && dw && workspace, "snn_conv2d_wgrad_bn: null pointer");
    if (check_conv_shape("snn_conv2d_wgrad_bn", N, H, W, Cin, Ho, Wo, Cout, KH, KW, stride, pad)) return 1;
    SNN_REQUIRE(frames_per_step > 0 && T > 0 && (int64_t)T * frames_per_step == N,
                "snn_conv2d_wgrad_bn: %lld frames are not %d timesteps of %d", (long long)N, T, frames_per_step);
    SNN_REQUIRE(ldx >= Cin && ldgx >= Cout && ldy >= Cout, "snn_conv2d_wgrad_bn: pixel stride smaller than channel count");
// ... 48 lines not shown
                        SNN_PREC_BF16X3, stream, true, v_th);
}

extern "C" int snn_conv1x1_spikes_wgrad(const float* vdec, int64_t ld, float v_th, const float* dy, int64_t lddy, float* dw,
                                        int64_t N, int H, int W, int Cin, int Cout, int accumulate, float* workspace,
                                        int splitk, void* stream) {
    return snn_conv2d_spikes_wgrad(vdec, ld, v_th, dy, lddy, dw, N, H, W, Cin, H, W, Cout, 1, 1, 1, 0, accumulate, workspace,
                                   splitk, stream);
}

bool snn_wgrad_mask_ok(int64_t N, int H, int W, int Cin, int Cout, const uint32_t* mask, int64_t ld_mask, const float* dy,
                       int64_t lddy, const float* dw) {
    if (!(N > 0 && H > 0 && W > 0 && Cin > 0 && Cout > 0 && mask && dy && dw && Cin % 32 == 0 && Cout % 4 == 0 &&
          ld_mask >= Cin / 32 && lddy >= Cout && lddy % 4 == 0 && aligned(4, {mask, dw}) && aligned(16, {dy}) &&
          (int64_t)Cin * Cout < (1LL << 26)))
        return false;
    const int64_t M = N * H * (int64_t)W;
    if (!(M < 0x7fffffffLL - 64 && (M + 64 + 3 * (int64_t)H * W) * ld_mask * 4 < 0x7fffffffLL && (M + 64) * lddy * 4 < 0x7fffffffLL))
        return false;
    const unsigned align = kAlignIn16 | kAlignDy16 | kAlignDy8 | (aligned(16, {dw}) ? kAlignDw16 : 0u);
    const WgradPlan p = wgrad_plan(N, H, W, Cin, H, W, Cout, 1, 1, 1, 0, ld_mask, lddy, align, SNN_PREC_BF16X3, true, 0, 0, false, true);
    return p.ok && p.kernel == kWgradPipe;
}

extern "C" int snn_conv1x1_mask_wgrad(const uint32_t* mask, int64_t ld_mask, const float* dy, int64_t lddy, float* dw, int64_t N,
                                      int H, int W, int Cin, int Cout, int accumulate, float* workspace, int splitk,
                                      void* stream) {
    SNN_REQUIRE(mask && dy && dw && workspace, "snn_conv1x1_mask_wgrad: null pointer");
    SNN_REQUIRE(snn_wgrad_mask_ok(N, H, W, Cin, Cout, mask, ld_mask, dy, lddy, dw),
                "snn_conv1x1_mask_wgrad: call not covered (ask snn_conv1x1_mask_supported)");
    return wgrad_common(reinterpret_cast<const float*>(mask), ld_mask, dy, lddy, dw, N, H, W, Cin, H, W, Cout, 1, 1, 1, 0,
                        accumulate, workspace, splitk, SNN_PREC_BF16X3, stream, true, 0.0f, true);
}
```

snn_for_object_detection_amd/functional.py:

```python

import collections
import ctypes
import os
from typing import List, NamedTuple, Optional, Sequence, Tuple

import torch
from torch.autograd import Function

from . import _hip
from ._hip import NeuronParams

_F32 = torch.float32
DEFAULT_DT = 0.001


SURROGATES = {"super": _hip.SURR_SUPER, "triangle": _hip.SURR_TRIANGLE, "sigmoid": _hip.SURR_SIGMOID,
              "atan": _hip.SURR_ATAN}


def _surrogate_code(surrogate: str) -> int:
    if surrogate not in SURROGATES:
        raise ValueError(f"unknown surrogate {surrogate!r}: one of {sorted(SURROGATES)}")
    return SURROGATES[surrogate]

# ... 509 lines not shown
        self.buf = buf
        self.written = False

    def claim(self) -> int:
        acc = 1 if self.written else 0
        self.written = True
        return acc


_NBT_BATCH = None


def begin_counter_batch() -> None:
    global _NBT_BATCH
    _NBT_BATCH = []


def flush_counter_batch() -> None:
    global _NBT_BATCH
    pending, _NBT_BATCH = _NBT_BATCH, None
    if pending:
        by_inc = {}
        for t, inc in pending:
            by_inc.setdefault(inc, []).append(t)
        for inc, tensors in by_inc.items():
            torch._foreach_add_(tensors, inc)


FUSE_OUTER_ADDEND = not os.environ.get("SNN_NO_OUTER_ADDEND")
USE_SIBLING_FUSION = not os.environ.get("SNN_NO_SIBLING_FUSION")
USE_SPIKES_FROM_VDEC = not os.environ.get("SNN_NO_SPIKES_FROM_VDEC")
USE_SPIKE_MASK = not os.environ.get("SNN_NO_SPIKE_MASK")
SPIKE_MASK_MIN_BYTES = 4 << 20


class GradAccumulator:

    __slots__ = ("deposits", "result", "fused", "outer", "exclusive", "grad_in_slot")

    def __init__(self):
        self.deposits = {}
        self.result = None
        self.fused = {}
        self.outer = None
        self.exclusive = set()
        self.grad_in_slot = False

    def deposit(self, key, g: torch.Tensor, exclusive: bool = False) -> None:
        if self.result is None and g is not None:
            self.deposits[key] = g
            if exclusive:
                self.exclusive.add(key)

    def set_result(self, dx: torch.Tensor) -> None:
        self.result = dx


def _acc_of(x):
    return getattr(x, "_snn_acc", None)


def _same_tensor(a: torch.Tensor, b: torch.Tensor) -> bool:
    return (a.data_ptr() == b.data_ptr() and tuple(a.shape) == tuple(b.shape) and a.stride() == b.stride())


def _slot_of(param) -> Optional[GradSlot]:
# ... 119 lines not shown
class PendingBnApply(NamedTuple):
    gx: torch.Tensor
    y: torch.Tensor
    coef: torch.Tensor
    dims: Tuple[int, int, int, int, int]


_PENDING_APPLY = {}
USE_DEFERRED_BN_APPLY = not os.environ.get("SNN_NO_DEFERRED_BN_APPLY")


def reset_backward_state() -> None:
    _PENDING_APPLY.clear()


def _apply_pending(pend: PendingBnApply) -> None:
    T, B, C, H, W = pend.dims
    _hip.call("snn_bn_bwd_apply_bf16" if pend.gx.dtype == _BF16 else "snn_bn_bwd_apply", pend.gx.data_ptr(), pend.y.data_ptr(), cl_stride(pend.y), pend.coef[0].data_ptr(),
              pend.coef[1].data_ptr(), pend.coef[2].data_ptr(), pend.gx.data_ptr(), C, T, B * H * W, C, 0, _stream())


def _wgrad_bn_ok(x: torch.Tensor, weight: torch.Tensor, stride: int, pad: int) -> bool:
    if not (USE_DEFERRED_BN_APPLY and weight.requires_grad and x.dim() == 5) or x.requires_grad:
        return False
    T, B, Cin, H, W = x.shape
    Cout, _, KH, KW = weight.shape
    Ho, Wo = (H + 2 * pad - KH) // stride + 1, (W + 2 * pad - KW) // stride + 1
    return bool(_hip.query("snn_conv2d_wgrad_bn_supported", T * B, H, W, Cin, Ho, Wo, Cout, KH, KW, stride, pad))


class _Conv2d(Function):

    @staticmethod
    def forward(ctx, x, weight, stride: int, pad: int, slot=None, dest=None, acc=None, prec=None, bn_out=None, x_th=None):
        _require_device(x, "conv2d input", bf16_ok=True)
        _require_device(weight, "conv2d weight")
        T, B, Cin, H, W = _dims5(x)
        Cout, Cin_w, KH, KW = weight.shape
        sb = x.dtype == _BF16 or (_activation_storage == "bf16" and Cin == 2 and (KH, KW) == (3, 3))
        fwd_prec, bwd_prec = _conv_precs(prec, sb)
        if Cin_w != Cin:
            raise RuntimeError(f"conv2d: input has {Cin} channels, weight expects {Cin_w}")
        Ho = (H + 2 * pad - KH) // stride + 1
        Wo = (W + 2 * pad - KW) // stride + 1
        x = _raw_to_cl(x)
        w = weight.detach()
        w_ohwi = w if is_channels_last(w) else _raw_dense_cl(w)
        x, x_th = _spikes_fwd_operand(x, x_th, lambda: not sb and _spikes_fwd_ok(
            _hip.query("snn_conv2d_spikes_supported", T * B, H, W, Cin, Ho, Wo, Cout, KH, KW, stride, pad, cl_stride(x),
                       fwd_prec, bwd_prec),
            _halo_ok(T * B, H, W, Cin, Cout, KH, KW, stride, pad), x.data_ptr(), w_ohwi.data_ptr()))
        if _ACTIVITY is not None:
            _ACTIVITY.count_conv((weight,), x, x_th, None, Cout, KH, KW, stride)
        y = _out_tensor(dest, T, B, Cout, Ho, Wo, x, _BF16 if sb else None)
        partial = layout = None
        if bn_out is not None:
            n_part = _hip.query("snn_conv2d_fwd_bn_partial_size", T * B, B, Ho, Wo, Cout)
            partial = torch.empty((n_part,), device=x.device, dtype=torch.float64)
            layout = (ctypes.c_int * 2)()
        w16 = None
        if fwd_prec == _hip.PREC_FP16X3 and USE_PRESPLIT_WEIGHTS and w_ohwi is w:
            w16 = _ptr(_kept_view(weight, "_snn_w16"))
        halo = (_halo_ok(T * B, H, W, Cin, Cout, KH, KW, stride, pad)
                and _halo_operand_ok(x.data_ptr(), cl_stride(x), x.dtype == _BF16))
        if halo and fwd_prec in (_hip.PREC_FP16X3, _hip.PREC_BF16S):
            img_prec = _hip.PREC_BF16X3 if sb else _hip.PREC_FP16X3
            img = _kept_view(weight, "_snn_wfrag", img_prec) if w_ohwi is w else None
            if img is None:
                img = _frag_image(w_ohwi, Cout, Cin, 0, img_prec)
            if x_th is not None:
                _hip.call("snn_conv3x3_halo_spikes", x.data_ptr(), cl_stride(x), x_th, img.data_ptr(), y.data_ptr(),
                          cl_stride(y), T * B, H, W, Cin, Cout, _ptr(partial), B, layout, _stream())
            else:
                _hip.call("snn_conv3x3_halo", x.data_ptr(), cl_stride(x), img.data_ptr(), y.data_ptr(), cl_stride(y), T * B,
                          H, W, Cin, Cout, None, 0, None, 0, _ptr(partial), B, layout, fwd_prec, _stream())
        elif x_th is not None:
            _hip.call("snn_conv2d_spikes_fwd", x.data_ptr(), cl_stride(x), x_th, w_ohwi.data_ptr(), y.data_ptr(), cl_stride(y),
                      T * B, H, W, Cin, Ho, Wo, Cout, KH, KW, stride, pad, _ptr(partial), B, layout, _stream())
        else:
            _hip.call("snn_conv2d_fwd", x.data_ptr(), cl_stride(x), w_ohwi.data_ptr(), w16, y.data_ptr(), cl_stride(y),
                      T * B, H, W, Cin, Ho, Wo, Cout, KH, KW, stride, pad, None, 0, _ptr(partial), B, layout, fwd_prec,
                      _stream())
        if layout is not None and layout[0] > 0:
            bn_out.append(BnPartial(partial, int(layout[0]), int(layout[1]), y.data_ptr(), (T, B * Ho * Wo, Cout)))
        ctx.prec = bwd_prec
        ctx.x_th = x_th
        ctx.save_for_backward(x, w_ohwi)
        ctx.weight = weight
        ctx.geom = (T, B, Cin, H, W, Cout, KH, KW, Ho, Wo, stride, pad)
        ctx.slot = slot
        ctx.acc = acc
        return y

    @staticmethod
    def backward(ctx, gy):
        x, w_ohwi = ctx.saved_tensors
        T, B, Cin, H, W, Cout, KH, KW, Ho, Wo, stride, pad = ctx.geom
        gy = _raw_to_cl(gy)
        ldg, ldx = cl_stride(gy), cl_stride(x)
        st = _stream()
        dx = dw = None
        pend = _PENDING_APPLY.pop(gy.data_ptr(), None)
        if pend is not None:
            fused = (not ctx.needs_input_grad[0] and ctx.needs_input_grad[1] and ctx.slot is not None
                     and pend.gx.dtype == _F32 and pend.dims == (T, B, Cout, Ho, Wo) and cl_stride(pend.y) % 4 == 0
                     and _hip.query("snn_conv2d_wgrad_bn_supported", T * B, H, W, Cin, Ho, Wo, Cout, KH, KW, stride, pad))
            if fused:
                splitk = _hip.query("snn_conv2d_wgrad_splitk", T * B, H, W, Cin, Ho, Wo, Cout, KH, KW, stride, pad, ctx.prec)
                with _WgradLaunch(x.device, True, splitk, Cout, KH * KW * Cin,
                                   hold=(x, pend.gx, pend.y, pend.coef)) as (stream, ws, _):
                    _hip.call("snn_conv2d_wgrad_bn", x.data_ptr(), ldx, pend.gx.data_ptr(), Cout, pend.y.data_ptr(),
                              cl_stride(pend.y), pend.coef.data_ptr(), T, B, ctx.slot.buf.data_ptr(), T * B, H, W, Cin, Ho,
                              Wo, Cout, KH, KW, stride, pad, ctx.slot.claim(), ws.data_ptr(), splitk, stream)
                return None, None, None, None, None, None, None, None, None, None
            _apply_pending(pend)
        if ctx.needs_input_grad[0]:
            wt = _kept_view(ctx.weight, "_snn_wt")
            wt16 = wt_img = None
            if wt is not None:
                wt_img = _kept_view(ctx.weight, "_snn_wtfrag")
                if ctx.prec == _hip.PREC_BF16X3 and USE_PRESPLIT_WEIGHTS and USE_PRESPLIT_DGRAD:
                    wt16 = _ptr(_kept_view(ctx.weight, "_snn_wt16"))
            else:
                wt = torch.empty((Cin, KH, KW, Cout), device=x.device, dtype=_F32)
                _hip.call("snn_weight_transpose", w_ohwi.data_ptr(), wt.data_ptr(), Cout, KH, KW, Cin, st)
            dx = _dgrad_accumulate(ctx.acc, gy, ldg, wt, x, ctx.geom, st, ctx.prec, wt_split=wt16, wt_image=wt_img)
        if ctx.needs_input_grad[1]:
            splitk = _hip.query("snn_conv2d_wgrad_splitk", T * B, H, W, Cin, Ho, Wo, Cout, KH, KW, stride, pad, ctx.prec)
            xw, ldxw, x_th = _spikes_wgrad_operand(x, ldx, ctx.x_th, gy, ldg)
            slot = ctx.slot
            with _WgradLaunch(x.device, slot is not None, splitk, Cout, KH * KW * Cin,
                              hold=(x, xw, gy)) as (stream, ws, _):
                if slot is not None:
                    dst, accumulate = slot.buf, slot.claim()
                else:
                    dst, accumulate = torch.empty((Cout, KH, KW, Cin), device=x.device, dtype=_F32), 0
                if x_th is not None:
                    _hip.call("snn_conv2d_spikes_wgrad", xw.data_ptr(), ldxw, x_th, gy.data_ptr(), ldg, dst.data_ptr(),
                              T * B, H, W, Cin, Ho, Wo, Cout, KH, KW, stride, pad, accumulate, ws.data_ptr(), splitk,
                              stream)
                else:
                    _hip.call("snn_conv2d_wgrad", xw.data_ptr(), ldxw, gy.data_ptr(), ldg, dst.data_ptr(), T * B, H, W,
                              Cin, Ho, Wo, Cout, KH, KW, stride, pad, accumulate, ws.data_ptr(), splitk, ctx.prec,
                              stream)
            if slot is None:
                dw = dst.permute(0, 3, 1, 2)
        return dx, dw, None, None, None, None, None, None, None, None


def _small_gemm(a: torch.Tensor, trans_a: bool, b: torch.Tensor, trans_b: bool, c: torch.Tensor, accumulate: int,
                ct: Optional[torch.Tensor] = None, ct_col: int = 0) -> None:
    m, n = c.shape
    k = a.shape[0] if trans_a else a.shape[1]
    ct_ptr, ldct = (None, 0) if ct is None else (ct.data_ptr() + 4 * ct_col, ct.shape[1])
    _hip.call("snn_small_gemm", a.data_ptr(), a.shape[1], int(trans_a), b.data_ptr(), b.shape[1], int(trans_b),
              c.data_ptr(), n, m, n, k, int(accumulate), ct_ptr, ldct, _stream())


class _SplitChannels(Function):

    @staticmethod
    def forward(ctx, x, widths):
        T, B, C, H, W = _dims5(x)
        if sum(widths) != C:
            raise RuntimeError(f"split_channels: widths {widths} do not add up to {C} channels")
        ctx.widths, ctx.like = tuple(widths), (T, B, H, W)
        ld, outs, off = cl_stride(x), [], 0
        for c in widths:
            t = _alias(x, x.storage_offset() + off, T, B, c, H, W, ld)
            t._snn_grad_in_slot = True
            outs.append(t)
            off += c
        return tuple(outs)

    @staticmethod
    def backward(ctx, *gs):
        T, B, H, W = ctx.like
        live = [g for g in gs if g is not None]
        if not live:
            return None, None
# ... 178 lines not shown
def sibling_conv1x1(x: torch.Tensor, w1: Optional[torch.Tensor], w2s: Sequence[torch.Tensor], dest: Optional[Dest] = None,
                    forward_precision: Optional[str] = None, backward_precision: Optional[str] = None) -> torch.Tensor:
    return _SiblingConv1x1.apply(x, w1, dest, _acc_of(x), _prec_codes(forward_precision, backward_precision),
                                 _slot_of(w1), tuple(_slot_of(w) for w in w2s), getattr(x, "_snn_spike_threshold", None),
                                 getattr(x, "_snn_spike_mask", None), *w2s)


def composed_conv1x1(x: torch.Tensor, w1: torch.Tensor, w2: torch.Tensor, dest: Optional[Dest] = None,
                     forward_precision: Optional[str] = None, backward_precision: Optional[str] = None) -> torch.Tensor:
    if x.dtype == _BF16 and (w1.shape[1] % 32 or w2.shape[0] % 32):
        y = to_bfloat16(composed_conv1x1(to_float32(x), w1, w2, None, forward_precision, backward_precision))
        return place(y, dest) if dest is not None else y
    seq, single = as_sequence(x)
    y = _SiblingConv1x1.apply(seq, w1, dest, _acc_of(seq), _prec_codes(forward_precision, backward_precision),
                              _slot_of(w1), (_slot_of(w2),), None, None, w2)
    return y[0] if single else y


class BnPartial(NamedTuple):
    partial: torch.Tensor
    chunks: int
    rows_per_chunk: int
    data_ptr: int
    dims: Tuple[int, int, int]


def conv2d(x: torch.Tensor, weight: torch.Tensor, stride: int = 1, padding: int = 0, dest: Optional[Dest] = None,
           forward_precision: Optional[str] = None, backward_precision: Optional[str] = None,
           bn_stats: bool = False) -> torch.Tensor:
    if x.dtype == _BF16 and (weight.shape[1] % 32 or weight.shape[0] % 32):
        y = to_bfloat16(conv2d(to_float32(x), weight, stride, padding, None, forward_precision, backward_precision, False))
        return place(y, dest) if dest is not None else y
    x_th = getattr(x, "_snn_spike_threshold", None)
    seq, single = as_sequence(x)
    bn_out = [] if bn_stats else None
    y = _Conv2d.apply(seq, weight, int(stride), int(padding), _slot_of(weight), dest, _acc_of(seq),
                      _prec_codes(forward_precision, backward_precision), bn_out, x_th)
    y = y[0] if single else y
    if bn_out:
        y._snn_bn_partial = bn_out[0]
    if bn_stats and not single and _slot_of(weight) is not None and _wgrad_bn_ok(seq, weight, int(stride), int(padding)):
        y._snn_defer_apply = True
    return y


class NeuronState(NamedTuple):
    v: torch.Tensor
    i: torch.Tensor


class SynapseState(NamedTuple):
    p: torch.Tensor


_SAVES_STEP = (_hip.NEURON_LIF, _hip.NEURON_SLI, _hip.NEURON_SYNAPSE)
SCAN_SEGMENT_T = 32
USE_CONV_BN_STATS = not os.environ.get("SNN_NO_CONV_BN_STATS")
USE_PRESPLIT_WEIGHTS = not os.environ.get("SNN_NO_PRESPLIT_WEIGHTS")
USE_PRESPLIT_DGRAD = bool(os.environ.get("SNN_PRESPLIT_DGRAD"))
SCAN_FLAGS = 0
USE_SUMS_FROM_STATE = not os.environ.get("SNN_NO_SUMS_FROM_STATE")

LIF_CHECKPOINT_BYTES: Optional[int] = None


def _bn_coefficients(y, ldy, dims, gamma, bias, use_running, eps, momentum, running_mean, running_var, sync_group,
                     bn_hint, st):
    T, M, C = dims
    dev = y.device
    mean, invstd, alpha, beta = (torch.empty((T, C), device=dev, dtype=_F32) for _ in range(4))
# ... 43 lines not shown
    else:
        _hip.call("snn_bn_bwd_reduce", sums.data_ptr(), T, M, C, raw_local.data_ptr(), st)
    raw = raw_local.clone()
    dist.all_reduce(raw, op=dist.ReduceOp.SUM, group=sync_group[0])
    param_sums = torch.empty((T, C, 2), device=y.device, dtype=torch.float64)
    _hip.call("snn_bn_bwd_coef", raw.data_ptr(), raw_local.data_ptr(), param_sums.data_ptr(), T, M * world,
              C, _ptr(gamma), mean.data_ptr(), invstd.data_ptr(), coef[0].data_ptr(), coef[1].data_ptr(),
              coef[2].data_ptr(), dg_ptr, db_ptr, acc_flag, st)


def _ptr_at(t: Optional[torch.Tensor], offset: int) -> Optional[int]:
    return None if t is None else t.data_ptr() + offset


class _NeuronCfg(NamedTuple):
    neuron: int
    has_bn: bool
    training: bool
    eps: float
    momentum: float
    running_mean: Optional[torch.Tensor]
    running_var: Optional[torch.Tensor]
    params: NeuronParams
    g_slot: Optional[GradSlot]
    b_slot: Optional[GradSlot]
    dest: Optional[Dest]
    sync_group: object
    bn_hint: object
    last_only: bool
    defer_apply: bool
    spikes_out: Optional[list]
    tau_slots: Tuple[Optional[GradSlot], Optional[GradSlot]]
    spike_mask: bool = False


def _bf16_scan_covers(neuron: int, channels: int) -> bool:
    return neuron in (_hip.NEURON_NONE, _hip.NEURON_LIF, _hip.NEURON_LI, _hip.NEURON_LI_TANH) and channels % 4 == 0


def _takes_checkpointed_pair(neuron: int, nbytes: int, params: NeuronParams, last_only: bool, sb: bool, tau: bool) -> bool:
    return (neuron == _hip.NEURON_LIF and LIF_CHECKPOINT_BYTES is not None and not last_only and not sb
            and nbytes >= LIF_CHECKPOINT_BYTES and default_gradient_rule(params) and not tau)


def _grad_pair(slots, needed, n: int, dev):
    if not any(needed):
        return None, None, 0, None, None
    if all(s_ is not None or not need for s_, need in zip(slots, needed)):
        acc = 1 if (slots[0] or slots[1]).written else 0
        for s_ in slots:
            if s_ is not None:
                s_.claim()
        pa, pb = (s_.buf.data_ptr() if (s_ is not None and need) else None for s_, need in zip(slots, needed))
        return pa, pb, acc, None, None
    fa, fb = (torch.empty((n,), device=dev, dtype=_F32) if need else None for need in needed)
    return _ptr(fa), _ptr(fb), 0, fa, fb


class _AffineNeuron(Function):

    @staticmethod
    def forward(ctx, y, gamma, bias, v0, i0, addend, cfg, w_mem=None, w_syn=None):
        neuron, has_bn, params, dest, sync_group, last_only = (cfg.neuron, cfg.has_bn, cfg.params, cfg.dest, cfg.sync_group,
                                                               cfg.last_only)
        _require_device(y, "norm/neuron input", bf16_ok=True)
        sb = y.dtype == _BF16
        tau = w_mem is not None
        if tau:
            _tau_refusal(neuron, sb)
            if last_only and (ctx.needs_input_grad[7] or ctx.needs_input_grad[8]):
                raise RuntimeError("last_only is not built for a LIF layer whose time constants are learned (tau=...)")
        if sb and not _bf16_scan_covers(neuron, y.shape[-3]):
            raise RuntimeError("bf16 storage: Norm + none / LIF / LI / LI+Tanh with a multiple of 4 channels only")
        if not default_gradient_rule(params):
            name = next((k for k, v in SURROGATES.items() if v == params.surrogate), params.surrogate)
            rule = f"surrogate={name!r}, detach_reset={bool(params.reset_detached)}"
            if neuron != _hip.NEURON_LIF:
                raise RuntimeError(f"a non-default gradient rule ({rule}) belongs to LIF layers")
            if sb:
                raise RuntimeError(f"bf16 storage has the default LIF gradient rule only, not ({rule}): keep this layer's "
                                   "tensors fp32 or its rule at surrogate='super', detach_reset=False")
        sb_flag = _hip.SCAN_BF16_STORAGE if sb else 0
        ctx.set_materialize_grads(False)
        y = _raw_to_cl(y)
        ldy = cl_stride(y)
        T, B, C, H, W = _dims5(y)
        if (C % 4 == 0 and (y.data_ptr() % (8 if sb else 16) or ldy % 4)
                and (has_bn or neuron in (_hip.NEURON_SLI, _hip.NEURON_SYNAPSE))):
            y = _raw_dense_cl(y)
            ldy = C
        M = B * H * W
        st = _stream()
        dev = y.device
        use_running = has_bn and not cfg.training
        if tau:
            learn = ctx.needs_input_grad[7] or ctx.needs_input_grad[8]
            nig = ctx.needs_input_grad
            sums_wanted = has_bn and ((nig[0] and not use_running) or (gamma is not None and nig[1]) or nig[2])
            if learn and sums_wanted and sync_group is None and SCAN_SEGMENT_T and T > SCAN_SEGMENT_T:
                raise RuntimeError(f"learnable time constants (tau=...): a Norm -> LIF sequence of {T} steps is longer than one "
                                   f"scan segment (SCAN_SEGMENT_T = {SCAN_SEGMENT_T}) and the segment look-back of the two "
                                   "gradient sums is not built")
        mean = invstd = alpha = beta = None
        if has_bn:
            mean, invstd, alpha, beta = _bn_coefficients(y, ldy, (T, M, C), gamma, bias, use_running, cfg.eps, cfg.momentum,
                                                         cfg.running_mean, cfg.running_var, sync_group, cfg.bn_hint, st)
        need_grad = any(ctx.needs_input_grad[:5]) or (tau and (ctx.needs_input_grad[7] or ctx.needs_input_grad[8]))
        c_mem = c_syn = None
        if tau:
            c_mem, c_syn = lif_time_constants(w_mem, w_syn, C)
        ckpt_pair = _takes_checkpointed_pair(neuron, T * M * C * 4, params, last_only, sb, tau)
        spikes_out = cfg.spikes_out
        no_out = (spikes_out is not None and USE_SPIKES_FROM_VDEC and neuron == _hip.NEURON_LIF and need_grad and has_bn
                  and addend is None and dest is None and not last_only and not sb and C % 4 == 0 and ldy % 4 == 0
                  and params.v_th >= 0.0 and not ckpt_pair)
        if last_only:
            if (neuron not in (_hip.NEURON_LIF, _hip.NEURON_LI, _hip.NEURON_LI_TANH) or addend is not None
                    or dest is not None):
                raise RuntimeError("last_only is for LIF / LI / LI+Tanh without shortcut or concat destination")
            out = _new_cl((B,), C, H, W, y)
        elif no_out:
            out = None
        else:
            out = _out_tensor(dest, T, B, C, H, W, y)
        has_state = neuron != _hip.NEURON_NONE
        vT = _new_cl((B,), C, H, W, y, _F32) if has_state else torch.empty(0, device=dev)
        iT = _new_cl((B,), C, H, W, y, _F32) if has_state else torch.empty(0, device=dev)
        vdec = None
        ckpt = False
        if neuron in _SAVES_STEP and need_grad:
            ckpt = ckpt_pair
            if ckpt:
                k = _hip.query("snn_lif_ckpt_interval")
                vdec = torch.empty(((T + k - 1) // k, 2, B, H, W, C), device=dev, dtype=_F32)
            else:
                vdec = torch.empty((T, B, H, W, C), device=dev, dtype=y.dtype)
        count_only = False
        if _ACTIVITY is not None and neuron == _hip.NEURON_LIF and (addend is not None or last_only):
            if ckpt:
                raise RuntimeError("activity.record: a LIF layer on the checkpointed scan (LIF_CHECKPOINT_BYTES) with a fused "
                                   "shortcut keeps neither spikes nor potentials to count")
            if vdec is None:
                vdec = torch.empty((T, B, H, W, C), device=dev, dtype=y.dtype)
                count_only = True
        if v0 is not None:
            v0 = _expand_state(v0, (B, C, H, W), dev)
        if i0 is not None:
            i0 = _expand_state(i0, (B, C, H, W), dev)
        ctx.addend_acc = None
        ad_ptr, ld_ad = None, 0
        if addend is not None:
            if neuron == _hip.NEURON_LI_TANH:
                raise RuntimeError("a fused shortcut is not supported after LI+Tanh (its backward reads the output)")
            ctx.addend_acc = _acc_of(addend)
            addend = _raw_to_cl(addend)
            if tuple(addend.shape) != (T, B, C, H, W):
                raise RuntimeError("Residual merge: branch outputs differ in shape")
            if addend.dtype != y.dtype:
                raise RuntimeError("Residual merge: shortcut and branch are stored in different types (fp32 / bf16)")
            ad_ptr, ld_ad = addend.data_ptr(), cl_stride(addend)
        mask = None
        if ckpt:
            _hip.call("snn_lif_fwd_ckpt", y.data_ptr(), ldy, _ptr(alpha), _ptr(beta), _ptr(v0), _ptr(i0),
                      out.data_ptr(), cl_stride(out), ad_ptr, ld_ad, _ptr(vT), _ptr(iT), vdec.data_ptr(), T, M, C,
                      params, st)
        else:
            head = (neuron, y.data_ptr(), ldy, _ptr(alpha), _ptr(beta), _ptr(v0), _ptr(i0),
                    _ptr(out), C if out is None else cl_stride(out), ad_ptr, ld_ad, _ptr(vT) if has_state else None,
                    _ptr(iT) if has_state else None, _ptr(vdec), T, M, C, params)
            fwd_flags = ((_hip.SCAN_LAST_STEP_ONLY if last_only else 0) | sb_flag
                         | (_hip.SCAN_SPIKES_FROM_VDEC if no_out else 0))
            if no_out and cfg.spike_mask and USE_SPIKE_MASK and not tau and C % 32 == 0 and T * M * C * 4 >= SPIKE_MASK_MIN_BYTES and all(
                    t is None or t.data_ptr() % 16 == 0 for t in (y, alpha, beta, v0, i0, vT, iT, vdec)):
                mask = torch.empty((T, B, H, W, C // 32), device=dev, dtype=torch.int32)
            if tau:
                _hip.call("snn_lif_tau_fwd", *head, c_mem.data_ptr(), c_syn.data_ptr(), fwd_flags, st)
            elif mask is not None:
                _hip.call("snn_affine_neuron_fwd_mask", *head, fwd_flags | _hip.SCAN_SPIKE_MASK, st, mask.data_ptr(), C // 32)
            else:
                _hip.call("snn_affine_neuron_fwd", *head, fwd_flags, st)
            if no_out:
                out = _alias(vdec, vdec.storage_offset(), T, B, C, H, W, C)
                spikes_out.append(float(params.v_th))
                if mask is not None:
                    spikes_out.append(mask)
        if _ACTIVITY is not None and neuron == _hip.NEURON_LIF:
            spikes = None if (no_out or addend is not None or last_only) else out
            _ACTIVITY.count_lif(params, mask, spikes, None if ckpt else vdec, float(params.v_th), (T, B, C, H, W))
            if count_only:
                vdec = None
        ctx.ckpt = ckpt
        ctx.sb = sb
        ctx.defer_apply = cfg.defer_apply
        ctx.last_only = last_only
        ctx.cfg = (neuron, has_bn, use_running, NeuronParams.from_buffer_copy(params), (T, B, C, H, W))
# ... 155 lines not shown

def affine_neuron_bwd_plan(neuron: int, T: int, M: int, C: int, ldg: int, ldy: int, with_sums: bool, flags: int = 0,
                           params: Optional[NeuronParams] = None) -> BwdPlan:
    out = (ctypes.c_int64 * 10)()
    _hip.call("snn_affine_neuron_bwd_plan", neuron, T, M, C, ldg, ldy, int(bool(with_sums)), params or neuron_params(),
              flags, ctypes.addressof(out))
    return BwdPlan(*out)


class TauBwdPlan(NamedTuple):
    scan: BwdPlan
    ordered: int
    lds_bytes: int


def lif_tau_bwd_plan(T: int, M: int, C: int, ldg: int, ldy: int, with_sums: bool, with_tau_sums: bool = True, flags: int = 0,
                     params: Optional[NeuronParams] = None, neuron: int = _hip.NEURON_LIF) -> TauBwdPlan:
    out = (ctypes.c_int64 * 12)()
    _hip.call("snn_lif_tau_bwd_plan", neuron, T, M, C, ldg, ldy, int(bool(with_sums)), int(bool(with_tau_sums)),
              params or neuron_params(), flags, ctypes.addressof(out))
    return TauBwdPlan(BwdPlan(*out[:10]), int(out[10]), int(out[11]))


def _expand_state(s: torch.Tensor, shape, dev) -> torch.Tensor:
    s = s.detach()
    if s.dim() == 0 or tuple(s.shape) != tuple(shape):
        s = s.to(device=dev, dtype=_F32).expand(shape)
    return _raw_dense_cl(s)


def affine_neuron(y: torch.Tensor, neuron: int, state: Optional[NeuronState] = None, bn=None,
                  params: Optional[NeuronParams] = None, dest: Optional[Dest] = None,
                  addend: Optional[torch.Tensor] = None, last_only: bool = False, spikes_ok: bool = False,
                  tau: Optional[Tuple[torch.Tensor, torch.Tensor]] = None, spike_mask_ok: bool = False):
    if y.dtype == _BF16 and not _bf16_scan_covers(neuron, y.shape[-3]):
        if tau is not None:
            _tau_refusal(neuron, True)
        out, new_state = affine_neuron(to_float32(y), neuron, state, bn, params, None,
                                       None if addend is None else to_float32(addend), last_only, False)
        out = out if (last_only and y.dim() == 5) else to_bfloat16(out)
        return (place(out, dest) if dest is not None else out), new_state
    bn_hint = getattr(y, "_snn_bn_partial", None)
    defer_apply = bool(getattr(y, "_snn_defer_apply", False))
    seq, single = as_sequence(y)
    if addend is not None:
        acc = _acc_of(addend)
        addend, _ = as_sequence(addend)
        if acc is not None:
            addend._snn_acc = acc
    params = params or neuron_params()
    has_bn = bn is not None
    gamma = bias = rm = rv = None
    training, eps, momentum = False, 1e-5, 0.1
    if has_bn:
        gamma, bias = bn.weight, bn.bias
        training = bn.training or (bn.running_mean is None and bn.running_var is None)
        rm, rv = bn.running_mean, bn.running_var
        eps = bn.eps
        if bn.momentum is None:
            raise RuntimeError("cumulative-average BatchNorm (momentum=None) is not supported")
        momentum = bn.momentum
        if training and seq.shape[1] * seq.shape[3] * seq.shape[4] <= 1:
            raise ValueError("Expected more than 1 value per channel when training, got input size "
                             f"{torch.Size((seq.shape[1], seq.shape[2], seq.shape[3], seq.shape[4]))}")
        if training and bn.num_batches_tracked is not None:
            if _NBT_BATCH is not None:
                _NBT_BATCH.append((bn.num_batches_tracked, int(seq.shape[0])))
            else:
                bn.num_batches_tracked.add_(seq.shape[0])
    v0 = i0 = None
    if state is not None:
        if neuron == _hip.NEURON_SYNAPSE:
            (v0,) = state
        else:
            v0, i0 = state
    sync_group = getattr(bn, "_snn_sync_group", None) if has_bn else None
    spikes_out = [] if (spikes_ok and not single and dest is None and addend is None) else None
    w_mem, w_syn = tau if tau is not None else (None, None)
    cfg = _NeuronCfg(neuron=neuron, has_bn=has_bn, training=training, eps=float(eps), momentum=float(momentum),
                     running_mean=rm, running_var=rv, params=params, g_slot=_slot_of(gamma), b_slot=_slot_of(bias), dest=dest,
                     sync_group=sync_group, bn_hint=bn_hint, last_only=bool(last_only) and not single,
                     defer_apply=defer_apply, spikes_out=spikes_out, tau_slots=(_slot_of(w_mem), _slot_of(w_syn)),
                     spike_mask=bool(spike_mask_ok))
    out, vT, iT = _AffineNeuron.apply(seq, gamma, bias, v0, i0, addend, cfg, w_mem, w_syn)
    if spikes_out:
        out._snn_spike_threshold = spikes_out[0]
        if len(spikes_out) > 1:
            out._snn_spike_mask = spikes_out[1]
    if neuron == _hip.NEURON_NONE:
        new_state = None
    elif neuron == _hip.NEURON_SYNAPSE:
        new_state = SynapseState(vT)
    else:
        new_state = NeuronState(vT, iT)
    if last_only and not single:
        return out, new_state
    return (out[0] if single else out), new_state


def _copy_cl(src: torch.Tensor, dst: torch.Tensor) -> None:
    if src.dtype != dst.dtype:
        raise RuntimeError("merge: operands are stored in different types (fp32 / bf16 storage mixed)")
    T, B, C, H, W = _dims5(src)
    _hip.call("snn_copy_channels_bf16" if src.dtype == _BF16 else "snn_copy_channels", src.data_ptr(), cl_stride(src),
              dst.data_ptr(), cl_stride(dst), T * B * H * W, C, _stream())


def _add_cl(a: torch.Tensor, b: torch.Tensor, dst: torch.Tensor) -> None:
    if not (a.dtype == b.dtype == dst.dtype):
        raise RuntimeError("merge: operands are stored in different types (fp32 / bf16 storage mixed)")
    T, B, C, H, W = _dims5(a)
    _hip.call("snn_add_bf16" if a.dtype == _BF16 else "snn_add", a.data_ptr(), cl_stride(a), b.data_ptr(), cl_stride(b),
              dst.data_ptr(), cl_stride(dst), T * B * H * W, C, _stream())


class _Concat(Function):

# ... 138 lines not shown
class _Place(Function):

    @staticmethod
    def forward(ctx, x, dest):
        ctx.acc = _acc_of(x)
        x = _raw_to_cl(x)
        T, B, C, H, W = _dims5(x)
        out = dest.tensor(T, B, C, H, W, x)
        _copy_cl(x, out)
        return out

    @staticmethod
    def backward(ctx, g):
        if ctx.acc is not None:
            ctx.acc[0].deposit(ctx.acc[1], g)
        return g, None


def place(x: torch.Tensor, dest: Dest) -> torch.Tensor:
    if dest.holds(x):
        return x
    return _Place.apply(x, dest)


def concat_channels(xs: List[torch.Tensor], dest: Optional[Dest] = None) -> torch.Tensor:
    if len(xs) == 1 and dest is None:
        return xs[0]
    seqs = [as_sequence(x) for x in xs]
    out = _Concat.apply(dest, *[s for s, _ in seqs])
    return out[0] if seqs[0][1] else out


def assemble_channels(promise: ConcatPromise, xs: List[torch.Tensor]) -> torch.Tensor:
    return _ConcatAssemble.apply(promise.buf, *xs)


def sum_tensors(xs: List[torch.Tensor], dest: Optional[Dest] = None) -> torch.Tensor:
    if len(xs) == 1:
        return xs[0] if dest is None else place(as_sequence(xs[0])[0], dest)
    seqs = [as_sequence(x) for x in xs]
    out = _Sum.apply(dest, *[s for s, _ in seqs])
    return out[0] if seqs[0][1] else out


class _GradReady(Function):

    @staticmethod
    def forward(ctx, x, fn):
        ctx.fn = fn
        acc = _acc_of(x)
        out = torch.empty(0, device=x.device, dtype=x.dtype)
        out.set_(x.untyped_storage(), x.storage_offset(), x.size(), x.stride())
        if acc is not None:
            out._snn_acc = acc
        return out

    @staticmethod
    def backward(ctx, g):
        ctx.fn()
        return g, None


def grad_ready_hook(x: torch.Tensor, fn) -> torch.Tensor:
    if fn is None or not x.requires_grad:
        return x
    return _GradReady.apply(x, fn)

# ... 560 lines not shown
```

snn_for_object_detection_amd/generator.py:

```python

import inspect
import os
from typing import Any, List, Optional, Tuple, Union

import torch
from torch import nn

from . import _hip
from . import functional as HF
from .anchors import AnchorGenerator
from .layer_gen import *
from .layer_gen import (ConvLSTM, Dense, HipBatchNorm2d, HipConv2d, HipReLU, HipSiLU, HipTanh, LayerGen,
                        LICell, LIFCell, Residual, Return, SLICell, StateStorage, Storage, SumPool2d, SynapseCell)

ListGen = List[Union[LayerGen, "ListGen"]]
ListState = List[Union[torch.Tensor, None, "ListState"]]


def _is_module_stateful(m: nn.Module) -> bool:
    return "state" in inspect.signature(m.forward).parameters


def _neuron_cell(layer: nn.Module) -> Optional[nn.Module]:
    cell = layer.module if isinstance(layer, StateStorage) else layer
# ... 136 lines not shown

    def _run_siblings(self, X: torch.Tensor, promise, pre_conv):
        specs = self._siblings
        convs = [branch[0] for branch in self.net]
        pendings = []
        for b, (_, _, nested) in enumerate(specs):
            if nested is None:
                pendings.append(None)
            else:
                nxt = self.net[b][nested]
                pendings.append(HF.ConcatPromise(nxt.out_channels,
                                                 parent=HF.Dest(promise, self._offsets[b], self._branch_channels[b])))
        first = convs[0]
        fp = (pre_conv.forward_precision if pre_conv is not None else None) or first.forward_precision
        bp = (pre_conv.backward_precision if pre_conv is not None else None) or first.backward_precision
        dest = HF.Dest(promise, specs[0][0], sum(c for _, c, _ in specs))
        whole = HF.sibling_conv1x1(X, pre_conv.weight if pre_conv is not None else None, [c.weight for c in convs],
                                   dest=dest, forward_precision=fp, backward_precision=bp)
        T, B, _, H, W = whole.shape
        for p in pendings:
            if p is not None:
                p.get(T, B, H, W, whole)
        return HF.split_channels(whole, [c for _, c, _ in specs]), pendings

    def _opens_with_1x1(self, in_channels: int) -> bool:
        if self.in_channels != in_channels or not len(self.net):
            return False
        for branch, plan in zip(self.net, self._plan):
            if not plan or plan[0] != ("layer", 0, 1) or not _is_plain_1x1(branch[0]):
                return False
        return True

    def forward(self, X: torch.Tensor, state: Optional[ListState] = None, dest=None, promise=None, pre_conv=None,
                last_only: bool = False):
        out = []
        out_state = []
        state = [None] * len(self.net) if state is None else state
        zero_copy = X.dim() == 5
        if not zero_copy:
            dest = promise = None
        if self.merge == "dense" and zero_copy and promise is None:
            promise = HF.ConcatPromise(self.out_channels, parent=dest)
        siblings = None
        spike_coded = getattr(X, "_snn_spike_threshold", None) is not None
        if (self._siblings is not None and zero_copy and HF.USE_SIBLING_FUSION and X.is_cuda
                and (X.dtype != torch.bfloat16 or all(c % 32 == 0 for c in (self.in_channels, *(s[1] for s in self._siblings))))):
            inputs, siblings = self._run_siblings(X, promise, pre_conv)
        elif spike_coded:
            raise RuntimeError("internal error: a tensor of saved potentials (spikes never written) reached a block that does "
                               "not open with the fused sibling convolution")
        else:
            inputs = HF.fanout(X, len(self.net))
        for b, (branch, flags, plan, branch_state) in enumerate(zip(self.net, self.branch_state, self._plan, state)):
            branch_state = [None] * len(branch) if branch_state is None else branch_state
            if self.merge == "dense":
                branch_dest = HF.Dest(promise, self._offsets[b], self._branch_channels[b]) if zero_copy else None
            elif self.merge == "forward":
                branch_dest = dest
            else:
                branch_dest = None
            fuse_here = self._fused_shortcut is not None and self._fused_shortcut[0] == b
            Y = inputs[b]
            pending = None
            if siblings is not None:
                pending = siblings[b]
            for k, (kind, idx, span) in enumerate(plan):
                if siblings is not None and k == 0:
                    continue
                last = k == len(plan) - 1
                step_dest = branch_dest if last else None
                step_promise, pending = pending, None
                if zero_copy and not last:
                    nkind, nidx, _ = plan[k + 1]
                    nxt = branch[nidx]
                    if nkind == "layer" and isinstance(nxt, BlockGen) and nxt._pass_offset is not None:
                        parent = branch_dest if (k + 1 == len(plan) - 1) else None
                        pending = HF.ConcatPromise(nxt.out_channels, parent=parent)
                        step_dest = HF.Dest(pending, nxt._pass_offset, nxt.in_channels)
                layer = branch[idx]
                if kind == "norm_neuron":
                    holder = branch[idx + 1]
                    cell = _neuron_cell(holder)
                    neuron = cell.kind
                    if span == 3:
                        neuron = _hip.NEURON_LI_TANH
                    old = branch_state[idx + 1]
                    direct = step_dest if neuron != _hip.NEURON_LI_TANH else None
                    shortcut = None
                    if fuse_here and last:
                        direct, shortcut = dest, inputs[self._fused_shortcut[1]]
                    only_last = (last_only and last and zero_copy and len(self.net) == 1 and direct is None
                                 and shortcut is None
                                 and neuron in (_hip.NEURON_LIF, _hip.NEURON_LI, _hip.NEURON_LI_TANH)
                                 and not (getattr(cell, "tau", None) is not None and torch.is_grad_enabled()
                                          and any(w.requires_grad for w in cell.tau))
                                 and not (isinstance(holder, StateStorage) and not self.training))
                    nxt_l = branch[plan[k + 1][1]] if (not last and plan[k + 1][0] == "layer") else None
                    to_siblings = (not last and plan[k + 1][0] == "conv_block"
                                   and branch[plan[k + 1][1] + 1]._siblings is not None and HF.USE_SIBLING_FUSION)
                    spikes_ok = (zero_copy and not last and self.training and neuron == _hip.NEURON_LIF
                                 and direct is None and shortcut is None and not isinstance(holder, StateStorage)
                                 and HF.USE_SPIKES_FROM_VDEC
                                 and (to_siblings
                                      or (isinstance(nxt_l, HipConv2d) and nxt_l.in_channels % 32 == 0
                                          and nxt_l.out_channels % 4 == 0 and nxt_l.kernel_size[0] <= 5
                                          and nxt_l.forward_precision is None and nxt_l.backward_precision is None)))
                    Y, new = HF.affine_neuron(Y, neuron, old, bn=layer, params=cell.params, dest=direct,
                                              addend=shortcut, last_only=only_last, spikes_ok=spikes_ok,
                                              tau=getattr(cell, "tau", None), spike_mask_ok=spikes_ok and to_siblings)
                    if isinstance(holder, StateStorage):
                        holder.record(old, Y, new)
                    branch_state[idx + 1] = new
                elif kind == "conv_block":
                    blk = branch[idx + 1]
                    Y, branch_state[idx + 1] = blk(Y, branch_state[idx + 1], dest=step_dest, promise=step_promise,
                                                   pre_conv=layer)
                elif isinstance(layer, BlockGen):
                    Y, branch_state[idx] = layer(Y, branch_state[idx], dest=step_dest, promise=step_promise,
                                                 last_only=last_only and last and len(self.net) == 1)
                elif isinstance(layer, HipConv2d) and pre_conv is not None and k == 0:
                    Y = HF.composed_conv1x1(Y, pre_conv.weight, layer.weight, dest=step_dest,
                                            forward_precision=pre_conv.forward_precision or layer.forward_precision,
                                            backward_precision=(pre_conv.backward_precision
                                                                or layer.backward_precision))
                elif isinstance(layer, HipConv2d):
                    feeds_bn = False
                    if not last and plan[k + 1][0] == "norm_neuron" and Y.is_cuda:
                        bn = branch[plan[k + 1][1]]
                        feeds_bn = bn.training or (bn.running_mean is None and bn.running_var is None)
                    Y = layer(Y, dest=step_dest, bn_stats=feeds_bn)
                elif isinstance(layer, (LIFCell, LICell, SLICell, SynapseCell)):
                    Y, branch_state[idx] = layer(Y, branch_state[idx], dest=step_dest)
                elif flags[idx]:
                    Y, branch_state[idx] = layer(Y, branch_state[idx])
                else:
                    Y = layer(Y)
                if step_dest is not None:
                    Y = HF.place(Y, step_dest)
            if branch_dest is not None and not plan:
                Y = HF.place(Y, branch_dest)
            out.append(Y)
            out_state.append(branch_state)
        if self.merge == "residual" and self._fused_shortcut is not None:
            merged = out[self._fused_shortcut[0]]
        elif self.merge == "residual":
            merged = HF.sum_tensors(out, dest=dest)
        elif self.merge == "dense":
            merged = HF.assemble_channels(promise, out) if zero_copy else HF.concat_channels(out)
        else:
            merged = out[0]
        return merged, out_state

# ... 176 lines not shown
```

snn_for_object_detection_amd/profiler.py:

```python

from collections import defaultdict
from typing import Dict

import torch


WGRAD_LABELS = ("k_conv_wgrad_pipe", "k_conv_wgrad_halo", "k_conv_first<wgrad>")


def _wgrad_label(n, h, w, cin, ho, wo, cout, kh, kw, stride, pad, prec) -> str:
    from . import _hip
    return WGRAD_LABELS[int(_hip.query("snn_conv2d_wgrad_kernel", n, h, w, cin, ho, wo, cout, kh, kw, stride, pad, prec))]


def _conv_label(name: str, a) -> str:
    if name == "snn_conv2d_wgrad":
        return _wgrad_label(a[5], a[6], a[7], a[8], a[9], a[10], a[11], a[12], a[13], a[14], a[15], a[19])
    dgrad = name == "snn_conv2d_dgrad"
    cin, cout = a[8], a[11]
    oc, ic = (cin, cout) if dgrad else (cout, cin)
    if not dgrad and cin == 2 and a[12] == 3 and a[13] == 3 and cout % 4 == 0 and (cout // 4) & (cout // 4 - 1) == 0 \
            and cout <= 256 and a[16] is None:
        return "k_conv_first<2, 3, false>"
    if oc <= 32:
# ... 13 lines not shown
        a = tuple(a[:3]) + tuple(a[4:])
        n, h, w, cin, ho, wo, cout, kh, kw = a[5], a[6], a[7], a[8], a[9], a[10], a[11], a[12], a[13]
        sb = a[21 if name == "snn_conv2d_fwd" else 20] == PREC_BF16S
        es = 2.0 if sb else 4.0
        es_in = 4.0 if (cin == 2 and name == "snn_conv2d_fwd") else es
        flops = 2.0 * n * ho * wo * cout * kh * kw * cin
        byts = es_in * n * h * w * cin + es * n * ho * wo * cout + 4.0 * cout * kh * kw * cin
        return _conv_label(name, a) + (", bf16s" if sb else ""), flops, byts
    if name == "snn_conv2d_wgrad":
        n, h, w, cin, ho, wo, cout, kh, kw = a[5], a[6], a[7], a[8], a[9], a[10], a[11], a[12], a[13]
        sb = a[19] == PREC_BF16S
        es = 2.0 if sb else 4.0
        flops = 2.0 * n * ho * wo * cout * kh * kw * cin
        byts = (4.0 if cin == 2 else es) * n * h * w * cin + es * n * ho * wo * cout + 4.0 * cout * kh * kw * cin
        return _conv_label(name, a) + (", bf16s" if sb else ""), flops, byts
    if name in ("snn_conv1x1_spikes_fwd", "snn_conv1x1_spikes_wgrad"):
        fwd = name.endswith("_fwd")
        n, h, w, cin, cout = (a[6], a[7], a[8], a[9], a[10])
        flops = 2.0 * n * h * w * cout * cin
        byts = 4.0 * (n * h * w * cin + n * h * w * cout + cout * cin)
        if not fwd:
            return WGRAD_LABELS[0], flops, byts
        tile = "32, 4, 1" if cout <= 32 else ("64, 2, 2" if cout <= 64 else "128, 2, 2")
        return f"k_conv_gather<{tile}, false, true>", flops, byts
    if name in ("snn_conv1x1_mask_fwd", "snn_conv1x1_mask_wgrad"):
        fwd = name.endswith("_fwd")
        n, h, w, cin, cout = (a[5], a[6], a[7], a[8], a[9])
        flops = 2.0 * n * h * w * cout * cin
        byts = n * h * w * cin / 8.0 + 4.0 * (n * h * w * cout + cout * cin)
        if not fwd:
            return WGRAD_LABELS[0] + ", mask, spikes", flops, byts
        tile = "32, 4, 1" if cout <= 32 else ("64, 2, 2" if cout <= 64 else "128, 2, 2")
        return f"k_conv_gather<{tile}, false, true>, mask, spikes", flops, byts
    if name in ("snn_conv2d_spikes_fwd", "snn_conv2d_spikes_wgrad"):
        fwd = name.endswith("_fwd")
        n, h, w, cin, ho, wo, cout, kh, kw, stride, pad = a[6:17]
        flops = 2.0 * n * ho * wo * cout * kh * kw * cin
        byts = 4.0 * (n * h * w * cin + n * ho * wo * cout + cout * kh * kw * cin)
        if not fwd:
            return _wgrad_label(n, h, w, cin, ho, wo, cout, kh, kw, stride, pad, 1) + ", spikes", flops, byts
        tile = "32, 4, 1" if cout <= 32 else ("64, 2, 2" if cout <= 64 else "128, 2, 2")
        return f"k_conv_gather<{tile}, false, true>", flops, byts
    if name == "snn_conv3x3_halo_spikes":
        n, h, w, cin, cout = a[6], a[7], a[8], a[9], a[10]
        flops = 2.0 * n * h * w * cout * 9 * cin
        byts = 4.0 * (n * h * w * cin + n * h * w * cout) + 4.0 * cout * 9 * cin
        return f"k_conv_halo3<{128 if cout % 128 == 0 else (64 if cout % 64 == 0 else 32)}, fwd, spikes>", flops, byts
    if name == "snn_conv3x3_halo":
        n, h, w, cin, cout, prec = a[5], a[6], a[7], a[8], a[9], a[17]
        es = 2.0 if prec == PREC_BF16S else 4.0
        flops = 2.0 * n * h * w * cout * 9 * cin
        byts = es * (n * h * w * cin + n * h * w * cout) + 4.0 * cout * 9 * cin
        kind = "fwd" if prec == 4 else ("dgrad" if prec == 1 else "bf16s")
        return f"k_conv_halo3<{128 if cout % 128 == 0 else (64 if cout % 64 == 0 else 32)}, {kind}>", flops, byts
    if name == "snn_conv3x3_s2_dgrad":
        n, h, w, cin, ho, wo, cout = a[5], a[6], a[7], a[8], a[9], a[10], a[11]
        sb = a[16] == PREC_BF16S
        flops = 2.0 * n * ho * wo * cout * 9 * cin
        byts = (2.0 if sb else 4.0) * (n * h * w * cin + n * ho * wo * cout) + 4.0 * cout * 9 * cin
        return "k_conv_s2dgrad3<dgrad>" + (", bf16s" if sb else ""), flops, byts
    if name == "snn_conv2d_wgrad_bn":
        n, h, w, cin, ho, wo, cout, kh, kw = a[10], a[11], a[12], a[13], a[14], a[15], a[16], a[17], a[18]
        flops = 2.0 * n * ho * wo * cout * kh * kw * cin
        byts = 4.0 * (n * h * w * cin + 2 * n * ho * wo * cout + cout * kh * kw * cin)
        return WGRAD_LABELS[2], flops, byts
    if name in ("snn_affine_neuron_fwd", "snn_affine_neuron_fwd_mask"):
# ... 105 lines not shown
```

Before: 7405.

## Fuse residual-chain spike masks into 1x1 conv gather instead of materializing sums

Adds a residual-chain path for 1x1 convolutions. Instead of materializing the residual-sum activations, the layer stores the base tensor plus per-layer spike bit masks. The gather kernel adds the mask bits to the base values while loading the A operand, and a matching wgrad path is added. This cuts the memory writes and reads of the full fp32 sum tensors between blocks, at the cost of extra mask loads, more register pressure (lower launch-bounds occupancy for XC>1) and fairly complex Python plumbing.

```diff
diff --git a/include/snn_hip.h b/include/snn_hip.h
--- a/include/snn_hip.h
+++ b/include/snn_hip.h
@@ -133,6 +133,18 @@
 int snn_conv1x1_mask_wgrad(const uint32_t* mask, int64_t ld_mask, const float* dy, int64_t lddy, float* dw, int64_t N, int H,
                            int W, int Cin, int Cout, int accumulate, float* workspace, int splitk, void* stream);
 
+int snn_conv1x1_chain_supported(int64_t N, int H, int W, int Cin, int Cout, const float* x, int64_t ldx, const int* groups,
+                                const uint32_t* const* masks, const int64_t* ld_masks, int n_masks, const float* w,
+                                const void* w_split, const float* y, int64_t ldy, const float* dy, int64_t lddy,
+                                const float* dw, int fwd_precision, int bwd_precision);
+int snn_conv1x1_chain_fwd(const float* x, int64_t ldx, const int* groups, const uint32_t* const* masks,
+                          const int64_t* ld_masks, int n_masks, const float* w, const void* w_split, float* y, int64_t ldy,
+                          int64_t N, int H, int W, int Cin, int Cout, double* bn_partial, int frames_per_step, int* bn_layout,
+                          void* stream);
+int snn_conv1x1_chain_wgrad(const float* x, int64_t ldx, const int* groups, const uint32_t* const* masks,
+                            const int64_t* ld_masks, int n_masks, const float* dy, int64_t lddy, float* dw, int64_t N, int H,
+                            int W, int Cin, int Cout, int accumulate, float* workspace, int splitk, void* stream);
+
 size_t snn_bn_stats_partial_size(int T, int64_t M, int C);
 int snn_bn_stats(const float* y, int64_t ldy, int T, int64_t M, int C, double* partial, void* stream);
 int snn_bn_stats_finalize(const double* partial, int chunks, int rows_per_chunk, int T, int64_t M, int C,
diff --git a/snn_for_object_detection_amd/_hip.py b/snn_for_object_detection_amd/_hip.py
--- a/snn_for_object_detection_amd/_hip.py
+++ b/snn_for_object_detection_amd/_hip.py
@@ -73,6 +73,9 @@
     "snn_conv1x1_mask_supported": (c_int, [_L, _I, _I, _I, _I, _P, _L, _P, _P, _L, _P, _L, _P, _I, _I]),
     "snn_conv1x1_mask_fwd": (c_int, [_P, _L, _P, _P, _L, _L, _I, _I, _I, _I, _P]),
     "snn_conv1x1_mask_wgrad": (c_int, [_P, _L, _P, _L, _P, _L, _I, _I, _I, _I, _I, _P, _I, _P]),
+    "snn_conv1x1_chain_supported": (c_int, [_L, _I, _I, _I, _I, _P, _L, _P, _P, _P, _I, _P, _P, _P, _L, _P, _L, _P, _I, _I]),
+    "snn_conv1x1_chain_fwd": (c_int, [_P, _L, _P, _P, _P, _I, _P, _P, _P, _L, _L, _I, _I, _I, _I, _P, _I, _P, _P]),
+    "snn_conv1x1_chain_wgrad": (c_int, [_P, _L, _P, _P, _P, _I, _P, _L, _P, _L, _I, _I, _I, _I, _I, _P, _I, _P]),
     "snn_conv2d_spikes_supported": (c_int, [_L, _I, _I, _I, _I, _I, _I, _I, _I, _I, _I, _L, _I, _I]),
     "snn_conv2d_spikes_fwd": (c_int, [_P, _L, _F, _P, _P, _L, _L, _I, _I, _I, _I, _I, _I, _I, _I, _I, _I, _P, _I, _P, _P]),
     "snn_conv2d_spikes_wgrad": (c_int, [_P, _L, _F, _P, _L, _P, _L, _I, _I, _I, _I, _I, _I, _I, _I, _I, _I, _I, _P, _I, _P]),
diff --git a/snn_for_object_detection_amd/csrc/conv_common.h b/snn_for_object_detection_amd/csrc/conv_common.h
--- a/snn_for_object_detection_amd/csrc/conv_common.h
+++ b/snn_for_object_detection_amd/csrc/conv_common.h
@@ -43,7 +43,50 @@
            N * (int64_t)Ho * Wo < 0x7fffffffLL && (int64_t)H * W * ld * 16 < 0x7fffffffLL;
 }
 
+constexpr int kChainMaxGroups = 32;
+constexpr int kChainMaxMasks = 4;
+constexpr int kChainMaxDepth = 4;
+struct GatherChain {
+    const uint32_t* mask[kChainMaxMasks];
+    int ld_mask[kChainMaxMasks];
+    unsigned grp[kChainMaxGroups];
+};
+
+static int chain_build(GatherChain& ch, int64_t pixels, int Cin, const int* groups, const uint32_t* const* masks,
+                       const int64_t* ld_masks, int n_masks) {
+    if (!(groups && masks && ld_masks && Cin > 0 && Cin % 32 == 0 && Cin / 32 <= kChainMaxGroups && n_masks >= 1 &&
+          n_masks <= kChainMaxMasks && pixels > 0))
+        return -1;
+    ch = GatherChain{};
+    for (int m = 0; m < n_masks; ++m) {
+        if (!(masks[m] && aligned(4, {masks[m]}) && ld_masks[m] >= 1 && pixels * ld_masks[m] * 4 < 0x7fffffffLL)) return -1;
+        ch.mask[m] = masks[m];
+        ch.ld_mask[m] = (int)ld_masks[m];
+    }
+    for (int m = n_masks; m < kChainMaxMasks; ++m) ch.mask[m] = masks[0];
+    int depth = 0;
+    for (int k = 0; k < Cin / 32; ++k) {
+        const int base = groups[4 * k], first = groups[4 * k + 1], count = groups[4 * k + 2], word = groups[4 * k + 3];
+        if (!(base >= 0 && base % 4 == 0 && base + 32 <= Cin && count >= 0 && count <= kChainMaxDepth)) return -1;
+        if (count == 0) {
+            if (base != 32 * k) return -1;
+            ch.grp[k] = (unsigned)base;
+            continue;
+        }
+        if (!(first >= 0 && first + count <= n_masks && word >= 0 && word < 64)) return -1;
+        for (int m = first; m < first + count; ++m)
+            if (word >= ld_masks[m]) return -1;
+        ch.grp[k] = (unsigned)base | ((unsigned)first << 16) | ((unsigned)count << 20) | ((unsigned)word << 23);
+        if (count > depth) depth = count;
+    }
+    return depth > 0 ? depth : -1;
 }
+
+}
+
+bool snn_wgrad_chain_ok(int64_t N, int H, int W, int Cin, int Cout, const float* x, int64_t ldx, const int* groups,
+                        const uint32_t* const* masks, const int64_t* ld_masks, int n_masks, const float* dy, int64_t lddy,
+                        const float* dw);
 
 struct FirstGeom {
     int64_t ldx, ldy;
diff --git a/snn_for_object_detection_amd/csrc/conv_gather.hip b/snn_for_object_detection_amd/csrc/conv_gather.hip
--- a/snn_for_object_detection_amd/csrc/conv_gather.hip
+++ b/snn_for_object_detection_amd/csrc/conv_gather.hip
@@ -79,12 +79,15 @@
     __syncthreads();
 }
 
+struct GatherNoChain {};
+
 template <int BN, int WM, int WN, bool DGRAD, bool VEC, int SPLIT, bool FAST, bool PRESPLIT = false, bool SB = false,
-          bool XSP = false, bool XM = false>
-__global__ __launch_bounds__(kThreads, (FAST && SPLIT) ? (PRESPLIT ? 3 : (SB ? (DGRAD ? 4 : SNN_GATHER_SB_WAVES) : 2)) : SNN_CONV_MIN_WAVES) void k_conv_gather(const float* __restrict__ in, const float* __restrict__ wk,
+          bool XSP = false, bool XM = false, int XC = 0>
+__global__ __launch_bounds__(kThreads, (FAST && SPLIT) ? (PRESPLIT ? (XC > 1 ? 2 : 3) : (SB ? (DGRAD ? 4 : SNN_GATHER_SB_WAVES) : 2)) : SNN_CONV_MIN_WAVES) void k_conv_gather(const float* __restrict__ in, const float* __restrict__ wk,
                                                           float* __restrict__ out, ConvGeom g,
                                                           const float* __restrict__ addend, int64_t ld_add,
-                                                          const float* __restrict__ addend2, int64_t ld_add2) {
+                                                          const float* __restrict__ addend2, int64_t ld_add2,
+                                                          typename std::conditional<(XC > 0), GatherChain, GatherNoChain>::type ch) {
     constexpr int TM = BM / WM / 32;
     constexpr int TN = BN / WN / 32;
     constexpr int BROWS = BN / 32;
@@ -92,6 +95,8 @@
     static_assert(!SB || (FAST && SPLIT == 5 && !PRESPLIT), "bf16 storage: the pipelined one-product kernel");
     static_assert(!XSP || (FAST && SPLIT == 4 && !DGRAD && !PRESPLIT && !SB), "spikes from potentials: fp16 x 3 forward");
     static_assert(!XM || XSP, "spike bit mask: an instance of the spikes-from-potentials kernel");
+    static_assert(XC == 0 || ((XC == 1 || XC == kChainMaxDepth) && FAST && SPLIT == 4 && !DGRAD && !SB && !XSP),
+                  "residual-chain K groups: the pipelined fp16 x 3 forward");
     constexpr int ES = SB ? 2 : 4;
     constexpr int NPIECE = SPLIT == 3 ? 3 : (SPLIT == 5 ? 1 : 2);
     constexpr int A_BYTES = SPLIT ? NPIECE * BM * LDB * 2 : BM * LDK * 4;
@@ -171,6 +176,8 @@
     using AReg = typename std::conditional<SB, u32x2, typename std::conditional<XM, unsigned, f32x4>::type>::type;
     AReg ra[4];
     f32x4 rb[BROWS];
+    struct ChainWords { unsigned w[4][XC > 0 ? XC : 1]; };
+    [[maybe_unused]] ChainWords rm;
 
     __amdgpu_buffer_rsrc_t rs_a, rs_b;
     int a_rel[4];
@@ -226,7 +233,7 @@
     }
     const unsigned fast_tw_n = DGRAD ? g.nkw : g.KW;
     const unsigned fast_tw_one = fast_tw_n == 1 ? 1u : 0u;
-    auto load_tiles_fast = [&](int k0n, AReg (&ra)[4], f32x4 (&rb)[BROWS], int which = 3) {
+    auto load_tiles_fast = [&](int k0n, AReg (&ra)[4], f32x4 (&rb)[BROWS], [[maybe_unused]] ChainWords& rm, int which = 3) {
         const bool kin = k0n < g.Ktot;
         const int tap = (int)__umulhi((unsigned)k0n, g.magic_ic);
         const int c0 = k0n - tap * g.IC;
@@ -241,6 +248,24 @@
             wcol0 = ((g.kh0 + g.stride * th) * g.KW + (g.kw0 + g.stride * tw)) * g.IC + c0;
         }
         const int tbit = kin ? tap : 31;
+        if constexpr (XC > 0) {
+            const unsigned d = ch.grp[kin ? (k0n >> 5) : 0];
+            const int cnt = kin ? (int)((d >> 20) & 7u) : 0, first = (int)((d >> 16) & 15u), word = (int)((d >> 23) & 63u);
+            toff = (int)(d & 0xffffu) * ES;
+            if (which & 1) {
+#pragma unroll
+                for (int q = 0; q < XC; ++q) {
+                    const int mi = first + q < kChainMaxMasks ? first + q : kChainMaxMasks - 1;
+                    const int ldm = ch.ld_mask[mi];
+                    const __amdgpu_buffer_rsrc_t rs_m = __builtin_amdgcn_make_buffer_rsrc(
+                        const_cast<uint32_t*>(ch.mask[mi]), 0, q < cnt ? (int)(g.Mtot * ldm * 4) : 0, 0x00020000);
+#pragma unroll
+                    for (int j = 0; j < 4; ++j)
+                        rm.w[j][q] = (unsigned)__builtin_amdgcn_raw_buffer_load_b32(
+                            rs_m, a_ok[j] ? (int)(((unsigned)m0 + lr + 32 * j) * (unsigned)ldm + (unsigned)word) * 4 : -1, 0, 0);
+                }
+            }
+        }
         if constexpr (XM) {
             if (which & 1) {
 #pragma unroll
@@ -265,7 +290,7 @@
 
     auto load_tiles = [&](int k0) {
         if (FAST) {
-            load_tiles_fast(k0, ra, rb);
+            load_tiles_fast(k0, ra, rb, rm);
             return;
         }
         if constexpr (!SB && !XM) {
@@ -407,7 +432,15 @@
                 out[1][e] = p[0]; out[1][e + 1] = p[1];
             }
         };
-        auto convert_a = [&](const AReg& v, bf16x4* out) {
+        auto convert_a = [&](const AReg& v, bf16x4* out, [[maybe_unused]] const unsigned* words = nullptr) {
+            if constexpr (XC > 0) {
+                f32x4 s = v;
+#pragma unroll
+                for (int q = 0; q < XC; ++q)
+#pragma unroll
+                    for (int e = 0; e < 4; ++e) s[e] += (float)((words[q] >> (kq + e)) & 1u);
+                convert(s, out, kF16ActScale);
+            } else
             if constexpr (SB) out[0] = __builtin_bit_cast(bf16x4, v);
             else if constexpr (XM) return;
             else if constexpr (XSP) {
@@ -510,19 +543,23 @@
         constexpr int NM = TM * TN * (XSP ? 2 : NPROD);
         constexpr int NREAD = XM ? TN * NP : (XSP ? TM + TN * NP : (TM + TN) * NP);
         constexpr int CONV_OPS = SPLIT == 3 ? 24 : (SPLIT == 5 ? 2 : 14);
-        constexpr int VPG_A = ((XM ? TM * 18 : (XSP ? 4 * 8 : 4 * CONV_OPS)) + NM - 1) / NM;
+        constexpr int VPG_A = ((XM ? TM * 18 : (XSP ? 4 * 8 : 4 * (CONV_OPS + 12 * XC))) + NM - 1) / NM;
         constexpr int VPG_B = PRESPLIT ? 1 : (BROWS * CONV_OPS + NM - 1) / NM;
         if (g.Ktot > 0) {
             AReg ra0[4];
             f32x4 rb0[BROWS];
-            load_tiles_fast(0, ra0, rb0);
-            load_tiles_fast(BK, ra, rb);
+            [[maybe_unused]] ChainWords rm0;
+            load_tiles_fast(0, ra0, rb0, rm0);
+            load_tiles_fast(BK, ra, rb, rm);
             if constexpr (XM) {
 #pragma unroll
                 for (int i = 0; i < TM; ++i) xm_cur[i] = ra0[i];
             }
 #pragma unroll
-            for (int j = 0; j < 4; ++j) convert_a(ra0[j], pa[j]);
+            for (int j = 0; j < 4; ++j) {
+                if constexpr (XC > 0) convert_a(ra0[j], pa[j], rm0.w[j]);
+                else convert_a(ra0[j], pa[j]);
+            }
 #pragma unroll
             for (int j = 0; j < BROWS; ++j) convert_b(rb0[j], pb[j]);
             write_tiles();
@@ -537,7 +574,10 @@
         for (int k0 = 0; k0 < g.Ktot; k0 += BK) {
             mfma_group(0);
 #pragma unroll
-            for (int j = 0; j < 4; ++j) convert_a(ra[j], pa[j]);
+            for (int j = 0; j < 4; ++j) {
+                if constexpr (XC > 0) convert_a(ra[j], pa[j], rm.w[j]);
+                else convert_a(ra[j], pa[j]);
+            }
             __builtin_amdgcn_sched_group_barrier(0x100, NREAD, 0);
 #pragma unroll
             for (int m = 0; m < NM; ++m) {
@@ -561,7 +601,7 @@
 #pragma unroll
                 for (int i = 0; i < TM; ++i) xm_cur[i] = ra[i];
             }
-            load_tiles_fast(k0 + 2 * BK, ra, rb);
+            load_tiles_fast(k0 + 2 * BK, ra, rb, rm);
             STAMP(2);
             __syncthreads();
             STAMP(3);
@@ -836,7 +876,8 @@
 
 static int launch_gather(bool dgrad, int split, bool sb, bool xsp, const float* in, const float* wk, const void* wk_split,
                          float* out, const ConvGeom& g, const float* addend, int64_t ld_add, const float* addend2,
-                         int64_t ld_add2, hipStream_t st, const char* name, bool xm = false) {
+                         int64_t ld_add2, hipStream_t st, const char* name, bool xm = false, const GatherChain* chain = nullptr,
+                         int xc = 0) {
     unsigned align = gather_align_bits(in, wk, wk_split, out, addend, ld_add, addend2, ld_add2);
     if (xm) align = (align & ~(kAlignIn16 | kAlignIn8)) | (aligned(4, {in}) ? kAlignIn16 : 0u);
     const GatherPlan p = gather_plan(g, dgrad, split, sb, xsp, align, wk_split != nullptr, addend != nullptr,
@@ -854,21 +895,33 @@
     gg.ntiles = p.ntiles;
     const dim3 grid((unsigned)p.blocks);
     const float* wsrc = p.loader == kLoadFastPresplit ? static_cast<const float*>(wk_split) : wk;
-    dispatch(
-        [&](auto BN, auto L, auto DGRAD, auto SPLIT) {
+    SNN_REQUIRE(!chain || ((p.loader == kLoadFast || p.loader == kLoadFastPresplit) && !dgrad && split == 4 && g.KtotFull == g.IC &&
+                           g.stride == 1 && g.pad == 0 && (xc == 1 || xc == kChainMaxDepth)),
+                "%s: residual-chain groups take the pipelined fp16 x 3 forward of a 1x1 convolution only", name);
+    const bool launched = dispatch(
+        [&](auto BN, auto L, auto DGRAD, auto SPLIT, auto XC) {
             constexpr int l = L(), s = SPLIT();
             constexpr bool vec = l != kLoadScalar, fast = l >= kLoadFast, pre = l == kLoadFastPresplit, sbl = l == kLoadSB,
                            xml = l == kLoadXM, xspl = l == kLoadXSP || xml;
             constexpr int ksplit = fast ? s : (vec ? (s == 4 ? 3 : (s == 5 ? 2 : s)) : 0);
-            if constexpr ((DGRAD() ? s != 3 && s != 4 : s != 2) && (!sbl || s == 5) && (!xspl || (!DGRAD() && s == 4)) &&
+            if constexpr (XC() > 0) {
+                if constexpr ((l == kLoadFast || l == kLoadFastPresplit) && !DGRAD() && s == 4) {
+                    hipLaunchKernelGGL((k_conv_gather<BN(), gather_wm(BN()), gather_wn(BN()), false, true, 4, true, pre, false, false, false, XC()>),
+                                       grid, dim3(kThreads), 0, st, in, wsrc, out, gg, addend, ld_add, addend2, ld_add2, *chain);
+                    return true;
+                }
+                return false;
+            } else if constexpr ((DGRAD() ? s != 3 && s != 4 : s != 2) && (!sbl || s == 5) && (!xspl || (!DGRAD() && s == 4)) &&
                           (!pre || s == 2 || s == 4)) {
                 hipLaunchKernelGGL((k_conv_gather<BN(), gather_wm(BN()), gather_wn(BN()), DGRAD(), vec, ksplit, fast, pre, sbl, xspl, xml>),
-                                   grid, dim3(kThreads), 0, st, in, wsrc, out, gg, addend, ld_add, addend2, ld_add2);
+                                   grid, dim3(kThreads), 0, st, in, wsrc, out, gg, addend, ld_add, addend2, ld_add2, GatherNoChain{});
                 return true;
             }
             return false;
         },
-        OneOf<32, 64, 128>{p.bn}, OneOf<0, 1, 2, 3, 4, 5, 6>{p.loader}, Flag{dgrad}, OneOf<0, 2, 3, 4, 5>{split});
+        OneOf<32, 64, 128>{p.bn}, OneOf<0, 1, 2, 3, 4, 5, 6>{p.loader}, Flag{dgrad}, OneOf<0, 2, 3, 4, 5>{split},
+        OneOf<0, 1, kChainMaxDepth>{chain ? xc : 0});
+    SNN_REQUIRE(launched || !chain, "%s: no kernel instance for these residual-chain groups", name);
     SNN_CHECK_LAUNCH(name);
     return 0;
 }
@@ -1199,3 +1252,62 @@
     return launch_gather(false, 4, false, true, reinterpret_cast<const float*>(mask), w, nullptr, y, g, nullptr, 0, nullptr, 0,
                          (hipStream_t)stream, "snn_conv1x1_mask_fwd", true);
 }
+
+namespace {
+static bool chain_fwd_ok(int64_t N, int H, int W, int Cin, int Cout, const float* x, int64_t ldx, const int* groups,
+                         const uint32_t* const* masks, const int64_t* ld_masks, int n_masks, const float* w,
+                         const void* w_split, const float* y, int64_t ldy, GatherChain* out_chain, int* out_depth) {
+    if (!(N > 0 && H > 0 && W > 0 && Cin > 0 && Cout > 0 && x && w && ldx >= Cin && ldy >= Cout &&
+          N * (int64_t)H * W < 0x7fffffffLL && (int64_t)Cin * Cin < 0xffffffffLL))
+        return false;
+    GatherChain ch;
+    const int depth = chain_build(ch, N * (int64_t)H * W, Cin, groups, masks, ld_masks, n_masks);
+    if (depth < 1) return false;
+    const ConvGeom g = gather_fwd_geom(N, H, W, Cin, H, W, Cout, 1, 1, 1, 0, ldx, ldy);
+    const unsigned align = gather_align_bits(x, w, w_split, y ? y : x, nullptr, 0, nullptr, 0);
+    const GatherPlan p = gather_plan(g, false, 4, false, false, align, w_split != nullptr, false, false);
+    if (!(p.ok && (p.loader == kLoadFast || p.loader == kLoadFastPresplit))) return false;
+    if (out_chain) *out_chain = ch;
+    if (out_depth) *out_depth = depth;
+    return true;
+}
+}
+
+extern "C" int snn_conv1x1_chain_supported(int64_t N, int H, int W, int Cin, int Cout, const float* x, int64_t ldx,
+                                           const int* groups, const uint32_t* const* masks, const int64_t* ld_masks,
+                                           int n_masks, const float* w, const void* w_split, const float* y, int64_t ldy,
+                                           const float* dy, int64_t lddy, const float* dw, int fwd_precision,
+                                           int bwd_precision) {
+    if (fwd_precision != SNN_PREC_FP16X3 || bwd_precision != SNN_PREC_BF16X3 || !x) return 0;
+    if (w && !chain_fwd_ok(N, H, W, Cin, Cout, x, ldx, groups, masks, ld_masks, n_masks, w, w_split, y, y ? ldy : Cout, nullptr,
+                           nullptr))
+        return 0;
+    if (!snn_wgrad_chain_ok(N, H, W, Cin, Cout, x, ldx, groups, masks, ld_masks, n_masks, dy, dy ? lddy : Cout, dw)) return 0;
+    return 1;
+}
+
+extern "C" int snn_conv1x1_chain_fwd(const float* x, int64_t ldx, const int* groups, const uint32_t* const* masks,
+                                     const int64_t* ld_masks, int n_masks, const float* w, const void* w_split, float* y,
+                                     int64_t ldy, int64_t N, int H, int W, int Cin, int Cout, double* bn_partial,
+                                     int frames_per_step, int* bn_layout, void* stream) {
+    SNN_REQUIRE(x && w && y, "snn_conv1x1_chain_fwd: null pointer");
+    if (check_conv_shape("snn_conv1x1_chain_fwd", N, H, W, Cin, H, W, Cout, 1, 1, 1, 0)) return 1;
+    GatherChain ch;
+    int depth = 0;
+    SNN_REQUIRE(chain_fwd_ok(N, H, W, Cin, Cout, x, ldx, groups, masks, ld_masks, n_masks, w, w_split, y, ldy, &ch, &depth),
+                "snn_conv1x1_chain_fwd: call not covered (ask snn_conv1x1_chain_supported)");
+    SNN_REQUIRE(!bn_partial || (bn_layout && frames_per_step > 0 && N % frames_per_step == 0),
+                "snn_conv1x1_chain_fwd: statistics need bn_layout and a frames_per_step that divides N");
+    if (bn_layout) bn_layout[0] = bn_layout[1] = 0;
+    ConvGeom g = gather_fwd_geom(N, H, W, Cin, H, W, Cout, 1, 1, 1, 0, ldx, ldy);
+    const int64_t step_rows = bn_partial ? (int64_t)frames_per_step * H * W : 0;
+    if (const int chunks = gather_bn_plan(bn_partial != nullptr, step_rows)) {
+        g.bn_partial = bn_partial;
+        g.bn_rows = step_rows;
+        g.bn_chunks = chunks;
+        bn_layout[0] = g.bn_chunks;
+        bn_layout[1] = BM;
+    }
+    return launch_gather(false, 4, false, false, x, w, w_split, y, g, nullptr, 0, nullptr, 0, (hipStream_t)stream,
+                         "snn_conv1x1_chain_fwd", false, &ch, depth == 1 ? 1 : kChainMaxDepth);
+}
diff --git a/snn_for_object_detection_amd/csrc/conv_wgrad.hip b/snn_for_object_detection_amd/csrc/conv_wgrad.hip
--- a/snn_for_object_detection_amd/csrc/conv_wgrad.hip
+++ b/snn_for_object_detection_amd/csrc/conv_wgrad.hip
@@ -16,6 +16,8 @@
     int nimg;
     float x_th;
 };
+
+struct WgradNoChain {};
 
 template <int TM, int TN, int WM, int WN, bool VEC>
 __global__ __launch_bounds__(kThreads, SNN_CONV_MIN_WAVES) void k_conv_wgrad(const float* __restrict__ x, const float* __restrict__ dy,
@@ -197,10 +199,11 @@
         }
 }
 
-template <int TM, int TN, int WM, int WN, int WBK, bool ONE, bool SB = false, bool XSP = false, bool XM = false>
-__global__ __launch_bounds__(kThreads, 2) void k_conv_wgrad_pipe(const float* __restrict__ x,
+template <int TM, int TN, int WM, int WN, int WBK, bool ONE, bool SB = false, bool XSP = false, bool XM = false, int XC = 0>
+__global__ __launch_bounds__(kThreads, (XC > 1 && TN * WN == 8) ? 1 : 2) void k_conv_wgrad_pipe(const float* __restrict__ x,
                                                                  const float* __restrict__ dy,
-                                                                 float* __restrict__ ws, WgradGeom g) {
+                                                                 float* __restrict__ ws, WgradGeom g,
+                                                                 typename std::conditional<(XC > 0), GatherChain, WgradNoChain>::type ch) {
     static_assert(WM * WN == 4, "4 waves");
     constexpr int BMc = 32 * TM * WM, BNk = 32 * TN * WN;
     constexpr int DG = BMc / 4, XG = BNk / 4;
@@ -208,6 +211,7 @@
     static_assert(!SB || ONE, "bf16 storage: one product");
     static_assert(!XSP || (!ONE && !SB), "spikes from potentials: the bf16 x 3 kernel");
     static_assert(!XM || XSP, "spike bit mask: an instance of the spikes-from-potentials kernel");
+    static_assert(XC == 0 || ((XC == 1 || XC == kChainMaxMasks) && !ONE && !SB && !XSP), "residual-chain K groups: the bf16 x 3 kernel");
     constexpr int XW = ((BNk / 32) * WBK + kThreads - 1) / kThreads;
     constexpr int ES = SB ? 2 : 4;
     constexpr int LDW = WBK + 8;
@@ -276,6 +280,26 @@
         x_kh[q] = tap / g.KW;
         x_kw[q] = tap - x_kh[q] * g.KW;
         x_tapoff[q] = ((x_kh[q] * g.W + x_kw[q]) * (int)g.ldx + ci) * ES;
+    }
+    [[maybe_unused]] unsigned xc_use[XQ];
+    [[maybe_unused]] int xc_word[XQ], xc_sh[XQ];
+    if constexpr (XC > 0) {
+#pragma unroll
+        for (int q = 0; q < XQ; ++q) {
+            const int kc = kc0 + x_cq[q];
+            unsigned d = 0;
+#pragma unroll
+            for (int gi = 0; gi < BNk / 32; ++gi) {
+                const int gk = kc0 / 32 + gi;
+                const unsigned dg = ch.grp[gk < kChainMaxGroups ? gk : kChainMaxGroups - 1];
+                if ((x_cq[q] >> 5) == gi) d = dg;
+            }
+            const unsigned first = (d >> 16) & 15u, count = x_ok[q] ? (d >> 20) & 7u : 0u;
+            xc_use[q] = ((1u << count) - 1u) << first;
+            xc_word[q] = (int)((d >> 23) & 63u);
+            xc_sh[q] = kc & 31;
+            if (x_ok[q]) x_tapoff[q] = ((int)(d & 0xffffu) + (kc & 31)) * ES;
+        }
     }
 
     int d_img = 0, d_oy = 0, d_ox = 0;
@@ -312,6 +336,7 @@
 
     using OReg = typename std::conditional<SB, u32x2, f32x4>::type;
     OReg rd[DQ][4], rx[XQ][4];
+    [[maybe_unused]] unsigned rxm[XQ][4][XC > 0 ? XC : 1];
     [[maybe_unused]] unsigned rxw[XW] = {}, pxw[XW] = {};
     [[maybe_unused]] const int xm_pl = tid % WBK;
     [[maybe_unused]] const int xm_word = kc0 / 32 + tid / WBK;
@@ -348,10 +373,29 @@
                 const bool ok = (info.w != 0) & x_ok[q] & ((unsigned)iy < (unsigned)g.H) & ((unsigned)ix < (unsigned)g.W);
                 const int voff = ok ? info.x + x_tapoff[q] : -1;
                 rx[q][e] = fetch(rs_x, voff);
+                if constexpr (XC > 0) {
+                    const unsigned pix = ok ? p0 + (unsigned)(quad * 4 + e) : 0u;
+#pragma unroll
+                    for (int m = 0; m < XC; ++m) {
+                        const bool use = ok && ((xc_use[q] >> m) & 1u) != 0u;
+                        const unsigned wv = ch.mask[m][use ? (int64_t)pix * ch.ld_mask[m] + xc_word[q] : 0];
+                        rxm[q][e][m] = use ? wv : 0u;
+                    }
+                }
             }
         }
     };
     bf16x4 pd[DQ][4][2], px[XQ][4][2];
+    auto chain_quad = [&](OReg (&v)[4], const unsigned (&words)[4][XC > 0 ? XC : 1], int sh) {
+        if constexpr (XC > 0) {
+#pragma unroll
+            for (int e = 0; e < 4; ++e)
+#pragma unroll
+                for (int m = 0; m < XC; ++m)
+#pragma unroll
+                    for (int c = 0; c < 4; ++c) v[e][c] += (float)((words[e][m] >> (sh + c)) & 1u);
+        }
+    };
     auto convert_quad = [&](const OReg (&v)[4], bf16x4 (&out)[4][2]) {
         if constexpr (SB) {
 #pragma unroll
@@ -464,7 +508,7 @@
     constexpr int NM = TM * TN * (ONE ? 1 : (XSP ? 2 : 3));
     constexpr int NREAD = XM ? 2 * TM + 2 * TN : (XSP ? 2 * TM + TN : (TM + TN) * (ONE ? 1 : 2));
     constexpr int CQ_OPS = SB ? 12 : 56;
-    constexpr int VPG_D = (DQ * CQ_OPS + NM - 1) / NM, VPG_X = XM ? (TN * 20 + NM - 1) / NM : (XQ * (XSP ? 24 : CQ_OPS) + NM - 1) / NM;
+    constexpr int VPG_D = (DQ * CQ_OPS + NM - 1) / NM, VPG_X = XM ? (TN * 20 + NM - 1) / NM : (XQ * (XSP ? 24 : CQ_OPS + 48 * XC) + NM - 1) / NM;
 
     decode(0);
     __syncthreads();
@@ -479,7 +523,10 @@
     for (int q = 0; q < XQ; ++q) {
         if constexpr (XM) continue;
         else if constexpr (XSP) convert_spikes(rx[q], px[q]);
-        else convert_quad(rx[q], px[q]);
+        else {
+            chain_quad(rx[q], rxm[q], xc_sh[q]);
+            convert_quad(rx[q], px[q]);
+        }
     }
     write_tiles();
     load_tiles(p_lo + WBK, 1);
@@ -506,7 +553,10 @@
         for (int q = 0; q < XQ; ++q) {
             if constexpr (XM) continue;
             else if constexpr (XSP) convert_spikes(rx[q], px[q]);
-            else convert_quad(rx[q], px[q]);
+            else {
+                chain_quad(rx[q], rxm[q], xc_sh[q]);
+                convert_quad(rx[q], px[q]);
+            }
         }
         __builtin_amdgcn_sched_group_barrier(0x100, NREAD, 0);
 #pragma unroll
@@ -879,7 +929,7 @@
 static int wgrad_common(const float* x, int64_t ldx, const float* dy, int64_t lddy, float* dw, int64_t N,
                         int H, int W, int Cin, int Ho, int Wo, int Cout, int KH, int KW, int stride, int pad,
                         int accumulate, float* workspace, int splitk, int precision, void* stream, bool xsp, float x_th,
-                        bool xm = false) {
+                        bool xm = false, const GatherChain* chain = nullptr, int xc = 0) {
     SNN_REQUIRE(x && dy && dw && workspace, "snn_conv2d_wgrad: null pointer");
     SNN_REQUIRE(precision == SNN_PREC_FP32 || precision == SNN_PREC_BF16X3 || precision == SNN_PREC_BF16X1 ||
                     precision == SNN_PREC_BF16S,
@@ -924,6 +974,10 @@
     SNN_REQUIRE(p.why != kWgradNotPipeXSP, "snn_conv1x1_spikes_wgrad: covers the pipelined bf16 x 3 kernel only (channels and "
                 "strides multiples of 4, 16-byte aligned tensors, < 2 GiB per pixel split)");
     SNN_REQUIRE(p.why != kWgradGridTooLarge, "snn_conv2d_wgrad: grid too large");
+    SNN_REQUIRE(!chain || (p.kernel == kWgradPipe && !p.one && !sbf && !xsp && KH == 1 && KW == 1 && stride == 1 && pad == 0 &&
+                           p.wbk == (p.t.id >= 4 ? 64 : 32) &&
+                           (xc == 1 || xc == kChainMaxMasks)),
+                "snn_conv1x1_chain_wgrad: residual-chain groups take the pipelined bf16 x 3 kernel of a 1x1 convolution only");
     g.pix_per_split = p.pix_per_split;
     g.nimg = (int)N;
     g.tiles_m = p.tiles_m;
@@ -932,18 +986,23 @@
     dim3 grid((unsigned)((int64_t)g.tiles_m * g.tiles_n * splitk));
     hipStream_t st = (hipStream_t)stream;
     dispatch(
-        [&](auto ID, auto KERNEL, auto WBK, auto ONE, auto SB, auto XSP, auto XM) {
+        [&](auto ID, auto KERNEL, auto WBK, auto ONE, auto SB, auto XSP, auto XM, auto XC) {
             constexpr WgradShape t = kWgradShapes[ID()];
-            if constexpr (KERNEL() != kWgradPipe) {
+            if constexpr (XC() > 0) {
+                if constexpr (KERNEL() == kWgradPipe && !ONE() && !SB() && !XSP() && !XM() && (WBK() == 64) == (ID() >= 4))
+                    hipLaunchKernelGGL((k_conv_wgrad_pipe<t.tm, t.tn, t.wm, t.wn, WBK(), false, false, false, false, XC()>), grid,
+                                       dim3(kThreads), 0, st, x, dy, workspace, g, *chain);
+            } else if constexpr (KERNEL() != kWgradPipe) {
                 hipLaunchKernelGGL((k_conv_wgrad<t.tm, t.tn, t.wm, t.wn, KERNEL() == kWgradVec>), grid, dim3(kThreads), 0, st, x, dy,
                                    workspace, g);
             } else if constexpr ((!SB() || ONE()) && (!XSP() || (!ONE() && !SB())) && (!XM() || XSP())) {
                 hipLaunchKernelGGL((k_conv_wgrad_pipe<t.tm, t.tn, t.wm, t.wn, WBK(), ONE(), SB(), XSP(), XM()>), grid, dim3(kThreads), 0,
-                                   st, x, dy, workspace, g);
+                                   st, x, dy, workspace, g, WgradNoChain{});
             }
             return true;
         },
-        OneOf<0, 1, 2, 3, 4, 5>{p.t.id}, OneOf<0, 1, 2>{p.kernel}, OneOf<32, 64>{p.wbk}, Flag{p.one}, Flag{sbf}, Flag{xsp}, Flag{xm});
+        OneOf<0, 1, 2, 3, 4, 5>{p.t.id}, OneOf<0, 1, 2>{p.kernel}, OneOf<32, 64>{p.wbk}, Flag{p.one}, Flag{sbf}, Flag{xsp}, Flag{xm},
+        OneOf<0, 1, kChainMaxMasks>{chain ? xc : 0});
     SNN_CHECK_LAUNCH("snn_conv2d_wgrad");
     return wgrad_reduce_slabs(workspace, dw, (int64_t)Cout * g.Ktot, splitk, accumulate, st);
 }
@@ -1058,3 +1117,33 @@
     return wgrad_common(reinterpret_cast<const float*>(mask), ld_mask, dy, lddy, dw, N, H, W, Cin, H, W, Cout, 1, 1, 1, 0,
                         accumulate, workspace, splitk, SNN_PREC_BF16X3, stream, true, 0.0f, true);
 }
+
+bool snn_wgrad_chain_ok(int64_t N, int H, int W, int Cin, int Cout, const float* x, int64_t ldx, const int* groups,
+                        const uint32_t* const* masks, const int64_t* ld_masks, int n_masks, const float* dy, int64_t lddy,
+                        const float* dw) {
+    if (!(N > 0 && H > 0 && W > 0 && Cin > 0 && Cout > 0 && x && Cin % 32 == 0 && Cout % 4 == 0 && ldx >= Cin && ldx % 4 == 0 &&
+          lddy >= Cout && lddy % 4 == 0 && aligned(16, {x}) && (!dy || aligned(16, {dy})) && (!dw || aligned(4, {dw})) &&
+          (int64_t)Cin * Cout < (1LL << 26)))
+        return false;
+    const int64_t M = N * H * (int64_t)W;
+    if (!(M < 0x7fffffffLL - 64 && (M + 64 + 3 * (int64_t)H * W) * ldx * 4 < 0x7fffffffLL && (M + 64) * lddy * 4 < 0x7fffffffLL))
+        return false;
+    GatherChain ch;
+    if (chain_build(ch, M, Cin, groups, masks, ld_masks, n_masks) < 1) return false;
+    const unsigned align = kAlignIn16 | kAlignIn8 | kAlignDy16 | kAlignDy8 | ((!dw || aligned(16, {dw})) ? kAlignDw16 : 0u);
+    const WgradPlan p = wgrad_plan(N, H, W, Cin, H, W, Cout, 1, 1, 1, 0, ldx, lddy, align, SNN_PREC_BF16X3, false, 0, 0, false);
+    return p.ok && p.kernel == kWgradPipe && !p.one && p.wbk == (p.t.id >= 4 ? 64 : 32);
+}
+
+extern "C" int snn_conv1x1_chain_wgrad(const float* x, int64_t ldx, const int* groups, const uint32_t* const* masks,
+                                       const int64_t* ld_masks, int n_masks, const float* dy, int64_t lddy, float* dw, int64_t N,
+                                       int H, int W, int Cin, int Cout, int accumulate, float* workspace, int splitk,
+                                       void* stream) {
+    SNN_REQUIRE(x && dy && dw && workspace, "snn_conv1x1_chain_wgrad: null pointer");
+    SNN_REQUIRE(snn_wgrad_chain_ok(N, H, W, Cin, Cout, x, ldx, groups, masks, ld_masks, n_masks, dy, lddy, dw),
+                "snn_conv1x1_chain_wgrad: call not covered (ask snn_conv1x1_chain_supported)");
+    GatherChain ch;
+    chain_build(ch, N * (int64_t)H * W, Cin, groups, masks, ld_masks, n_masks);
+    return wgrad_common(x, ldx, dy, lddy, dw, N, H, W, Cin, H, W, Cout, 1, 1, 1, 0, accumulate, workspace, splitk, SNN_PREC_BF16X3,
+                        stream, false, 0.0f, false, &ch, n_masks == 1 ? 1 : kChainMaxMasks);
+}
diff --git a/snn_for_object_detection_amd/functional.py b/snn_for_object_detection_amd/functional.py
--- a/snn_for_object_detection_amd/functional.py
+++ b/snn_for_object_detection_amd/functional.py
@@ -565,6 +565,81 @@
 USE_SPIKES_FROM_VDEC = not os.environ.get("SNN_NO_SPIKES_FROM_VDEC")
 USE_SPIKE_MASK = not os.environ.get("SNN_NO_SPIKE_MASK")
 SPIKE_MASK_MIN_BYTES = 4 << 20
+USE_RESIDUAL_CHAIN = not os.environ.get("SNN_NO_RESIDUAL_CHAIN")
+RESIDUAL_CHAIN_MAX_DEPTH = 4
+RESIDUAL_CHAIN_MIN_BYTES = SPIKE_MASK_MIN_BYTES
+RESIDUAL_CHAIN_MAX_CIN = 128
+
+
+class ChainConsumer(NamedTuple):
+    weight: torch.Tensor
+    default_precision: bool
+    training: bool
+
+
+class ResidualChain(NamedTuple):
+    base: torch.Tensor
+    masks: Tuple[torch.Tensor, ...]
+
+
+def residual_chain_refusal(*, enabled: bool, train: bool, sequence: bool, fp32: bool, learnable_tau: bool, state_holder: bool,
+                           channels: int, nbytes: int, aligned: bool, recorded: bool, base_depth: int,
+                           consumers_ok: bool) -> Optional[str]:
+    if not enabled:
+        return "SNN_NO_RESIDUAL_CHAIN"
+    if not train:
+        return "eval mode"
+    if not sequence:
+        return "time-outer call (one timestep)"
+    if not fp32:
+        return "bf16 storage"
+    if learnable_tau:
+        return "learnable time constants"
+    if state_holder:
+        return "StateStorage holder"
+    if recorded:
+        return "the activity monitor reads the tensor"
+    if channels % 32 != 0:
+        return "channels not a multiple of 32"
+    if nbytes < RESIDUAL_CHAIN_MIN_BYTES or not aligned:
+        return "below RESIDUAL_CHAIN_MIN_BYTES or unaligned"
+    if base_depth + 1 > RESIDUAL_CHAIN_MAX_DEPTH:
+        return "chain depth cap"
+    if not consumers_ok:
+        return "a consumer has no chain-capable kernel for this shape"
+    return None
+
+
+def _chain_tables(x: torch.Tensor, chains):
+    Cin, ld = x.shape[2], cl_stride(x)
+    if Cin % 32 or ld is None:
+        return None
+    masks: List[torch.Tensor] = []
+    table = [[32 * k, 0, 0, 0] for k in range(Cin // 32)]
+    for off, ch in chains:
+        C = ch.base.shape[2]
+        delta = ch.base.data_ptr() - x.data_ptr()
+        if (ch.base.dtype != _F32 or delta % 4 or not 0 <= delta // 4 <= Cin - C or cl_stride(ch.base) != ld or off % 32
+                or C % 32 or off + C > Cin or tuple(ch.base.shape) != (x.shape[0], x.shape[1], C, x.shape[3], x.shape[4])):
+            return None
+        first = None
+        for k, m in enumerate(ch.masks):
+            idx = next((i for i, t in enumerate(masks) if t is m), None)
+            if idx is None:
+                masks.append(m)
+                idx = len(masks) - 1
+            if first is None:
+                first = idx
+            elif idx != first + k:
+                return None
+        for i in range(C // 32):
+            table[off // 32 + i] = [delta // 4 + 32 * i, first, len(ch.masks), i]
+    if not masks:
+        return None
+    groups = (ctypes.c_int * (4 * len(table)))(*[v for row in table for v in row])
+    ptrs = (ctypes.c_void_p * len(masks))(*[m.data_ptr() for m in masks])
+    lds = (ctypes.c_int64 * len(masks))(*[m.shape[-1] for m in masks])
+    return groups, ptrs, lds, len(masks), tuple(masks)
 
 
 class GradAccumulator:
@@ -750,7 +825,8 @@
 class _Conv2d(Function):
 
     @staticmethod
-    def forward(ctx, x, weight, stride: int, pad: int, slot=None, dest=None, acc=None, prec=None, bn_out=None, x_th=None):
+    def forward(ctx, x, weight, stride: int, pad: int, slot=None, dest=None, acc=None, prec=None, bn_out=None, x_th=None,
+                chain=None):
         _require_device(x, "conv2d input", bf16_ok=True)
         _require_device(weight, "conv2d weight")
         T, B, Cin, H, W = _dims5(x)
@@ -768,6 +844,14 @@
             _hip.query("snn_conv2d_spikes_supported", T * B, H, W, Cin, Ho, Wo, Cout, KH, KW, stride, pad, cl_stride(x),
                        fwd_prec, bwd_prec),
             _halo_ok(T * B, H, W, Cin, Cout, KH, KW, stride, pad), x.data_ptr(), w_ohwi.data_ptr()))
+        tables = None
+        if chain:
+            ok = ((KH, KW, stride, pad) == (1, 1, 1, 0) and x_th is None and not sb and _ACTIVITY is None
+                  and fwd_prec == _hip.PREC_FP16X3 and bwd_prec == _hip.PREC_BF16X3)
+            tables = _chain_tables(x, chain) if ok else None
+            if tables is None:
+                raise RuntimeError("conv2d: the input holds residual-chain channels (never written) and this call cannot "
+                                   "rebuild them: a plain 1x1 convolution in the default arithmetic only")
         if _ACTIVITY is not None:
             _ACTIVITY.count_conv((weight,), x, x_th, None, Cout, KH, KW, stride)
         y = _out_tensor(dest, T, B, Cout, Ho, Wo, x, _BF16 if sb else None)
@@ -795,6 +879,15 @@
         elif x_th is not None:
             _hip.call("snn_conv2d_spikes_fwd", x.data_ptr(), cl_stride(x), x_th, w_ohwi.data_ptr(), y.data_ptr(), cl_stride(y),
                       T * B, H, W, Cin, Ho, Wo, Cout, KH, KW, stride, pad, _ptr(partial), B, layout, _stream())
+        elif tables is not None:
+            groups, mptrs, mlds, n_masks, _ = tables
+            if not _hip.query("snn_conv1x1_chain_supported", T * B, H, W, Cin, Cout, x.data_ptr(), cl_stride(x), groups, mptrs,
+                              mlds, n_masks, w_ohwi.data_ptr(), w16, y.data_ptr(), cl_stride(y), None, 0, None, fwd_prec,
+                              bwd_prec):
+                raise RuntimeError("conv2d: snn_conv1x1_chain_fwd does not cover this call, and the chain channels of its "
+                                   "input were never written")
+            _hip.call("snn_conv1x1_chain_fwd", x.data_ptr(), cl_stride(x), groups, mptrs, mlds, n_masks, w_ohwi.data_ptr(), w16,
+                      y.data_ptr(), cl_stride(y), T * B, H, W, Cin, Cout, _ptr(partial), B, layout, _stream())
         else:
             _hip.call("snn_conv2d_fwd", x.data_ptr(), cl_stride(x), w_ohwi.data_ptr(), w16, y.data_ptr(), cl_stride(y),
                       T * B, H, W, Cin, Ho, Wo, Cout, KH, KW, stride, pad, None, 0, _ptr(partial), B, layout, fwd_prec,
@@ -803,6 +896,7 @@
             bn_out.append(BnPartial(partial, int(layout[0]), int(layout[1]), y.data_ptr(), (T, B * Ho * Wo, Cout)))
         ctx.prec = bwd_prec
         ctx.x_th = x_th
+        ctx.chain = tables
         ctx.save_for_backward(x, w_ohwi)
         ctx.weight = weight
         ctx.geom = (T, B, Cin, H, W, Cout, KH, KW, Ho, Wo, stride, pad)
@@ -830,7 +924,7 @@
                     _hip.call("snn_conv2d_wgrad_bn", x.data_ptr(), ldx, pend.gx.data_ptr(), Cout, pend.y.data_ptr(),
                               cl_stride(pend.y), pend.coef.data_ptr(), T, B, ctx.slot.buf.data_ptr(), T * B, H, W, Cin, Ho,
                               Wo, Cout, KH, KW, stride, pad, ctx.slot.claim(), ws.data_ptr(), splitk, stream)
-                return None, None, None, None, None, None, None, None, None, None
+                return None, None, None, None, None, None, None, None, None, None, None
             _apply_pending(pend)
         if ctx.needs_input_grad[0]:
             wt = _kept_view(ctx.weight, "_snn_wt")
@@ -848,12 +942,21 @@
             xw, ldxw, x_th = _spikes_wgrad_operand(x, ldx, ctx.x_th, gy, ldg)
             slot = ctx.slot
             with _WgradLaunch(x.device, slot is not None, splitk, Cout, KH * KW * Cin,
-                              hold=(x, xw, gy)) as (stream, ws, _):
+                              hold=(x, xw, gy) + (ctx.chain[4] if ctx.chain else ())) as (stream, ws, _):
                 if slot is not None:
                     dst, accumulate = slot.buf, slot.claim()
                 else:
                     dst, accumulate = torch.empty((Cout, KH, KW, Cin), device=x.device, dtype=_F32), 0
-                if x_th is not None:
+                if ctx.chain is not None:
+                    groups, mptrs, mlds, n_masks, _ = ctx.chain
+                    if not _hip.query("snn_conv1x1_chain_supported", T * B, H, W, Cin, Cout, x.data_ptr(), ldx, groups, mptrs, mlds,
+                                      n_masks, None, None, None, 0, gy.data_ptr(), ldg, dst.data_ptr(), _hip.PREC_FP16X3,
+                                      ctx.prec):
+                        raise RuntimeError("conv2d backward: snn_conv1x1_chain_wgrad does not cover this call, and the chain "
+                                           "channels of its input were never written")
+                    _hip.call("snn_conv1x1_chain_wgrad", x.data_ptr(), ldx, groups, mptrs, mlds, n_masks, gy.data_ptr(), ldg,
+                              dst.data_ptr(), T * B, H, W, Cin, Cout, accumulate, ws.data_ptr(), splitk, stream)
+                elif x_th is not None:
                     _hip.call("snn_conv2d_spikes_wgrad", xw.data_ptr(), ldxw, x_th, gy.data_ptr(), ldg, dst.data_ptr(),
                               T * B, H, W, Cin, Ho, Wo, Cout, KH, KW, stride, pad, accumulate, ws.data_ptr(), splitk,
                               stream)
@@ -863,7 +966,7 @@
                               stream)
             if slot is None:
                 dw = dst.permute(0, 3, 1, 2)
-        return dx, dw, None, None, None, None, None, None, None, None
+        return dx, dw, None, None, None, None, None, None, None, None, None
 
 
 def _small_gemm(a: torch.Tensor, trans_a: bool, b: torch.Tensor, trans_b: bool, c: torch.Tensor, accumulate: int,
@@ -1108,10 +1211,11 @@
         y = to_bfloat16(conv2d(to_float32(x), weight, stride, padding, None, forward_precision, backward_precision, False))
         return place(y, dest) if dest is not None else y
     x_th = getattr(x, "_snn_spike_threshold", None)
+    chain = getattr(x, "_snn_chain", None)
     seq, single = as_sequence(x)
     bn_out = [] if bn_stats else None
     y = _Conv2d.apply(seq, weight, int(stride), int(padding), _slot_of(weight), dest, _acc_of(seq),
-                      _prec_codes(forward_precision, backward_precision), bn_out, x_th)
+                      _prec_codes(forward_precision, backward_precision), bn_out, x_th, chain)
     y = y[0] if single else y
     if bn_out:
         y._snn_bn_partial = bn_out[0]
@@ -1221,6 +1325,8 @@
     spikes_out: Optional[list]
     tau_slots: Tuple[Optional[GradSlot], Optional[GradSlot]]
     spike_mask: bool = False
+    chain: Optional[ChainConsumer] = None
+    chain_out: Optional[list] = None
 
 
 def _bf16_scan_covers(neuron: int, channels: int) -> bool:
@@ -1244,6 +1350,46 @@
         return pa, pb, acc, None, None
     fa, fb = (torch.empty((n,), device=dev, dtype=_F32) if need else None for need in needed)
     return _ptr(fa), _ptr(fb), 0, fa, fb
+
+
+def _chain_root(dest: Dest) -> Tuple[ConcatPromise, int]:
+    promise, off = dest.promise, dest.off
+    while promise.parent is not None:
+        off += promise.parent.off
+        promise = promise.parent.promise
+    return promise, off
+
+
+def _chain_form(cfg: "_NeuronCfg", addend: torch.Tensor, y: torch.Tensor, ldy: int, dims, dest: Dest, scan_ok: bool, sb: bool,
+                tau: bool, state) -> Optional[torch.Tensor]:
+    T, B, C, H, W = dims
+    base = _raw_to_cl(addend)
+    root, off = _chain_root(dest)
+    buf = root.buf
+    consumer = cfg.chain
+    w = consumer.weight
+    aligned = all(t is None or t.data_ptr() % 16 == 0 for t in (y, base, *state)) and ldy % 4 == 0
+    consumers_ok = False
+    if (scan_ok and buf is not None and cfg.chain_out is not None and consumer.default_precision and tuple(w.shape[1:]) == (buf.shape[2], 1, 1)
+            and w.dtype == _F32 and C % 32 == 0 and tuple(base.shape) == (T, B, C, H, W)):
+        delta = base.data_ptr() - buf.data_ptr()
+        Cin = buf.shape[2]
+        if (delta % 4 == 0 and 0 <= delta // 4 <= Cin - C and cl_stride(base) == cl_stride(buf) and off % 32 == 0 and Cin % 32 == 0
+                and Cin <= RESIDUAL_CHAIN_MAX_CIN):
+            table = [[32 * k, 0, 0, 0] for k in range(Cin // 32)]
+            for i in range(C // 32):
+                table[off // 32 + i] = [delta // 4 + 32 * i, 0, 1, i]
+            groups = (ctypes.c_int * (4 * len(table)))(*[v for row in table for v in row])
+            mptrs = (ctypes.c_void_p * 1)(base.data_ptr())
+            mlds = (ctypes.c_int64 * 1)(C // 32)
+            fwd_prec, bwd_prec = _conv_precs(None, False)
+            wp = w.data_ptr() if is_channels_last(w.detach()) else buf.data_ptr()
+            consumers_ok = bool(_hip.query("snn_conv1x1_chain_supported", T * B, H, W, Cin, w.shape[0], buf.data_ptr(), cl_stride(buf),
+                                           groups, mptrs, mlds, 1, wp, None, None, 0, None, 0, None, fwd_prec, bwd_prec))
+    why = residual_chain_refusal(enabled=USE_RESIDUAL_CHAIN and USE_SPIKE_MASK and USE_SPIKES_FROM_VDEC, train=consumer.training, sequence=True, fp32=not sb, learnable_tau=tau,
+                                 state_holder=False, channels=C, nbytes=T * B * H * W * C * 4, aligned=aligned,
+                                 recorded=_ACTIVITY is not None, base_depth=0, consumers_ok=consumers_ok)
+    return base if why is None else None
 
 
 class _AffineNeuron(Function):
@@ -1303,6 +1449,10 @@
         no_out = (spikes_out is not None and USE_SPIKES_FROM_VDEC and neuron == _hip.NEURON_LIF and need_grad and has_bn
                   and addend is None and dest is None and not last_only and not sb and C % 4 == 0 and ldy % 4 == 0
                   and params.v_th >= 0.0 and not ckpt_pair)
+        chain_form = None
+        if addend is not None and cfg.chain is not None and dest is not None:
+            chain_form = _chain_form(cfg, addend, y, ldy, (T, B, C, H, W), dest, neuron == _hip.NEURON_LIF and need_grad
+                                     and has_bn and not last_only and params.v_th >= 0.0 and not ckpt_pair, sb, tau, (v0, i0))
         if last_only:
             if (neuron not in (_hip.NEURON_LIF, _hip.NEURON_LI, _hip.NEURON_LI_TANH) or addend is not None
                     or dest is not None):
@@ -1338,6 +1488,8 @@
             i0 = _expand_state(i0, (B, C, H, W), dev)
         ctx.addend_acc = None
         ad_ptr, ld_ad = None, 0
+        if addend is not None and getattr(addend, "_snn_chain", None):
+            raise RuntimeError("internal error: a residual-chain tensor (never written) reached a LIF layer as its shortcut")
         if addend is not None:
             if neuron == _hip.NEURON_LI_TANH:
                 raise RuntimeError("a fused shortcut is not supported after LI+Tanh (its backward reads the output)")
@@ -1349,7 +1501,13 @@
                 raise RuntimeError("Residual merge: shortcut and branch are stored in different types (fp32 / bf16)")
             ad_ptr, ld_ad = addend.data_ptr(), cl_stride(addend)
         mask = None
-        if ckpt:
+        if chain_form is not None:
+            mask = torch.empty((T, B, H, W, C // 32), device=dev, dtype=torch.int32)
+            _hip.call("snn_affine_neuron_fwd_mask", neuron, y.data_ptr(), ldy, _ptr(alpha), _ptr(beta), _ptr(v0), _ptr(i0), None, C,
+                      None, 0, _ptr(vT), _ptr(iT), _ptr(vdec), T, M, C, params,
+                      sb_flag | _hip.SCAN_SPIKES_FROM_VDEC | _hip.SCAN_SPIKE_MASK, st, mask.data_ptr(), C // 32)
+            cfg.chain_out.append(ResidualChain(chain_form, (mask,)))
+        elif ckpt:
             _hip.call("snn_lif_fwd_ckpt", y.data_ptr(), ldy, _ptr(alpha), _ptr(beta), _ptr(v0), _ptr(i0),
                       out.data_ptr(), cl_stride(out), ad_ptr, ld_ad, _ptr(vT), _ptr(iT), vdec.data_ptr(), T, M, C,
                       params, st)
@@ -1571,7 +1729,8 @@
 def affine_neuron(y: torch.Tensor, neuron: int, state: Optional[NeuronState] = None, bn=None,
                   params: Optional[NeuronParams] = None, dest: Optional[Dest] = None,
                   addend: Optional[torch.Tensor] = None, last_only: bool = False, spikes_ok: bool = False,
-                  tau: Optional[Tuple[torch.Tensor, torch.Tensor]] = None, spike_mask_ok: bool = False):
+                  tau: Optional[Tuple[torch.Tensor, torch.Tensor]] = None, spike_mask_ok: bool = False,
+                  chain: Optional[ChainConsumer] = None):
     if y.dtype == _BF16 and not _bf16_scan_covers(neuron, y.shape[-3]):
         if tau is not None:
             _tau_refusal(neuron, True)
@@ -1616,12 +1775,15 @@
     sync_group = getattr(bn, "_snn_sync_group", None) if has_bn else None
     spikes_out = [] if (spikes_ok and not single and dest is None and addend is None) else None
     w_mem, w_syn = tau if tau is not None else (None, None)
+    chain_out = [] if (chain is not None and not single and dest is not None and addend is not None) else None
     cfg = _NeuronCfg(neuron=neuron, has_bn=has_bn, training=training, eps=float(eps), momentum=float(momentum),
                      running_mean=rm, running_var=rv, params=params, g_slot=_slot_of(gamma), b_slot=_slot_of(bias), dest=dest,
                      sync_group=sync_group, bn_hint=bn_hint, last_only=bool(last_only) and not single,
                      defer_apply=defer_apply, spikes_out=spikes_out, tau_slots=(_slot_of(w_mem), _slot_of(w_syn)),
-                     spike_mask=bool(spike_mask_ok))
+                     spike_mask=bool(spike_mask_ok), chain=chain if chain_out is not None else None, chain_out=chain_out)
     out, vT, iT = _AffineNeuron.apply(seq, gamma, bias, v0, i0, addend, cfg, w_mem, w_syn)
+    if chain_out:
+        out._snn_chain = [(0, chain_out[0])]
     if spikes_out:
         out._snn_spike_threshold = spikes_out[0]
         if len(spikes_out) > 1:
@@ -1826,7 +1988,14 @@
 
 
 def assemble_channels(promise: ConcatPromise, xs: List[torch.Tensor]) -> torch.Tensor:
-    return _ConcatAssemble.apply(promise.buf, *xs)
+    whole = _ConcatAssemble.apply(promise.buf, *xs)
+    chains, off = [], 0
+    for x in xs:
+        chains += [(off + o, ch) for o, ch in getattr(x, "_snn_chain", None) or ()]
+        off += x.shape[2]
+    if chains:
+        whole._snn_chain = chains
+    return whole
 
 
 def sum_tensors(xs: List[torch.Tensor], dest: Optional[Dest] = None) -> torch.Tensor:
diff --git a/snn_for_object_detection_amd/generator.py b/snn_for_object_detection_amd/generator.py
--- a/snn_for_object_detection_amd/generator.py
+++ b/snn_for_object_detection_amd/generator.py
@@ -192,7 +192,7 @@
         return True
 
     def forward(self, X: torch.Tensor, state: Optional[ListState] = None, dest=None, promise=None, pre_conv=None,
-                last_only: bool = False):
+                last_only: bool = False, chain_consumer=None):
         out = []
         out_state = []
         state = [None] * len(self.net) if state is None else state
@@ -230,6 +230,14 @@
                 last = k == len(plan) - 1
                 step_dest = branch_dest if last else None
                 step_promise, pending = pending, None
+                step_consumer = None
+                if zero_copy and kind in ("layer", "conv_block") and isinstance(branch[idx + (kind == "conv_block")], BlockGen):
+                    if last:
+                        step_consumer = chain_consumer if self.merge in ("dense", "forward") else None
+                    elif plan[k + 1][0] == "layer" and _is_plain_1x1(branch[plan[k + 1][1]]):
+                        nconv = branch[plan[k + 1][1]]
+                        step_consumer = HF.ChainConsumer(nconv.weight, nconv.forward_precision is None
+                                                         and nconv.backward_precision is None, self.training)
                 if zero_copy and not last:
                     nkind, nidx, _ = plan[k + 1]
                     nxt = branch[nidx]
@@ -267,17 +275,19 @@
                                           and nxt_l.forward_precision is None and nxt_l.backward_precision is None)))
                     Y, new = HF.affine_neuron(Y, neuron, old, bn=layer, params=cell.params, dest=direct,
                                               addend=shortcut, last_only=only_last, spikes_ok=spikes_ok,
-                                              tau=getattr(cell, "tau", None), spike_mask_ok=spikes_ok and to_siblings)
+                                              tau=getattr(cell, "tau", None), spike_mask_ok=spikes_ok and to_siblings,
+                                              chain=chain_consumer if shortcut is not None else None)
                     if isinstance(holder, StateStorage):
                         holder.record(old, Y, new)
                     branch_state[idx + 1] = new
                 elif kind == "conv_block":
                     blk = branch[idx + 1]
                     Y, branch_state[idx + 1] = blk(Y, branch_state[idx + 1], dest=step_dest, promise=step_promise,
-                                                   pre_conv=layer)
+                                                   pre_conv=layer, chain_consumer=step_consumer)
                 elif isinstance(layer, BlockGen):
                     Y, branch_state[idx] = layer(Y, branch_state[idx], dest=step_dest, promise=step_promise,
-                                                 last_only=last_only and last and len(self.net) == 1)
+                                                 last_only=last_only and last and len(self.net) == 1,
+                                                 chain_consumer=step_consumer)
                 elif isinstance(layer, HipConv2d) and pre_conv is not None and k == 0:
                     Y = HF.composed_conv1x1(Y, pre_conv.weight, layer.weight, dest=step_dest,
                                             forward_precision=pre_conv.forward_precision or layer.forward_precision,
diff --git a/snn_for_object_detection_amd/profiler.py b/snn_for_object_detection_amd/profiler.py
--- a/snn_for_object_detection_amd/profiler.py
+++ b/snn_for_object_detection_amd/profiler.py
@@ -69,6 +69,18 @@
             return WGRAD_LABELS[0] + ", mask, spikes", flops, byts
         tile = "32, 4, 1" if cout <= 32 else ("64, 2, 2" if cout <= 64 else "128, 2, 2")
         return f"k_conv_gather<{tile}, false, true>, mask, spikes", flops, byts
+    if name in ("snn_conv1x1_chain_fwd", "snn_conv1x1_chain_wgrad"):
+        fwd = name.endswith("_fwd")
+        n, h, w, cin, cout = a[10:15] if fwd else a[9:14]
+        groups = [tuple(a[2][4 * k:4 * k + 4]) for k in range(cin // 32)]
+        bases = len({g[0] for g in groups})
+        bits = sum(g[2] for g in groups)
+        flops = 2.0 * n * h * w * cout * cin
+        byts = n * h * w * (4.0 * 32 * bases + 4.0 * bits) + 4.0 * (n * h * w * cout + cout * cin)
+        if not fwd:
+            return WGRAD_LABELS[0] + ", chain", flops, byts
+        tile = "32, 4, 1" if cout <= 32 else ("64, 2, 2" if cout <= 64 else "128, 2, 2")
+        return f"k_conv_gather<{tile}, false, true>, chain", flops, byts
     if name in ("snn_conv2d_spikes_fwd", "snn_conv2d_spikes_wgrad"):
         fwd = name.endswith("_fwd")
         n, h, w, cin, ho, wo, cout, kh, kw, stride, pad = a[6:17]
```

After: 7483 (median of 6 runs). No clear change (+1.1%).
